# xmlyqing00/V-FloodNet

Hardware: AMD Instinct MI355X
Metric: segmented frames/sec at 480p (higher is better)
Workload: dtype f32

## Files before the change

include/vfn_hip.h:

```cpp
#ifndef VFN_HIP_H
#define VFN_HIP_H

#ifdef __cplusplus
extern "C" {
#endif

#define VFN_ABI_VERSION 12
enum { VFN_DESC_CONV = 0, VFN_DESC_STEM = 1, VFN_DESC_BANKSCAN = 2, VFN_DESC_MEMREAD = 3, VFN_DESC_BANK = 4, VFN_DESC_WGRAD = 5,
       VFN_DESC_REFRESH_FILTER = 6, VFN_DESC_REFRESH_EPILOGUE = 7, VFN_DESC_GATHER = 8 };
int vfn_abi_version(void);
int vfn_sizeof_desc(int which);

typedef struct vfn_conv_desc {
    const float* in;
    const float* w;
    const float* scale;
    const float* shift;
    const float* res;
    float* out;
    int N, H, W, Cin, in_ld;
    int Ho, Wo, Cout, cout_pad, out_ld, res_ld;
    int KH, KW, stride, pad;
    int relu_in, relu_out;
    int M;
    int ksplit;
    int split_from;
    int res_mod;
    float* partial;
    int* tile_counters;
    int w_packed;
    int in_lp;
    int out_lp_relu;
    void* out_lp;
    const float* mask;
    int mask_ld;
    int mask_after;
    int w_batch_rows;
    int k_rot;
} vfn_conv_desc;

int vfn_conv_cfg_count(void);
int vfn_conv_cfg_tile(int cfg, int* bm, int* bn);
int vfn_conv_cfg_info(int cfg, int* bm, int* bn, int* wm, int* wn, int* dma);
int vfn_conv_cfg_wk(int cfg);
int vfn_conv_cfg_tpb(int cfg);
#define VFN_CONV_SK_WS_FLOATS (16 * 1024 * 1024)
#define VFN_CONV_SK_MAX_TILES 16384
int vfn_conv_cfg_kind(int cfg);
int vfn_conv_cfg_name(int cfg, char* buf, int n);
int vfn_conv2d_nhwc_f32(const vfn_conv_desc* d, int cfg, void* stream);
int vfn_conv2d_nhwc_bf16(const vfn_conv_desc* d, int cfg, void* stream);
int vfn_conv2d_nhwc_bf16x3(const vfn_conv_desc* d, int cfg, void* stream);

int vfn_winograd_tiles(int N, int H, int W);
int vfn_winograd_input_f32(const float* x, int N, int H, int W, int C, int ld_x, int relu, float* V, int rows_pad, void* stream);
int vfn_winograd_output_f32(const float* Mb, int rows_pad, int N, int H, int W, int Cout, const float* scale, const float* shift,
                            const float* res, int res_ld, int res_mod, int relu_out, float* out, int out_ld, void* stream);
int vfn_winograd_output_masked_f32(const float* Mb, int rows_pad, int N, int H, int W, int Cout, const float* res, int res_ld,
                                   const float* mask, int mask_ld, int mask_after, float* out, int out_ld, void* stream);
int vfn_winograd_gemm_f32(const float* V, const float* U, float* Mb, int comps, int rows_pad, int C, int Cout, int cout_pad, int cfg,
                          int wgs, void* stream);
int vfn_conv1x1_persistent_f32(const vfn_conv_desc* d, int cfg, int wgs, void* stream);
int vfn_winograd_input_bf16(const float* x, int N, int H, int W, int C, int ld_x, int relu, void* V, int rows_pad, void* stream);
int vfn_winograd_gemm_bf16(const void* V, const void* U, float* Mb, int comps, int rows_pad, int C, int Cout, int cout_pad, int cfg,
                           int wgs, void* stream);
int vfn_winograd_gy_f32(const float* gy, int N, int H, int W, int C, int ld, float* Z, int rows_pad, void* stream);
int vfn_winograd_dw_f32(const float* dU, int Cout, int Cin, const float* rowscale, float* dw, int accumulate, void* stream);

typedef struct vfn_stem_desc {
    const float* frame;
    const float* mask;
    const float* w;
    const float* scale;
    const float* shift;
    float* out;
    float mean[3];
    float std[3];
    int N, cin;
    int H0, W0;
    int pad_top, pad_left;
    int Hp, Wp;
    int Ho, Wo;
} vfn_stem_desc;

int vfn_stem_conv7x7_f32(const vfn_stem_desc* d, void* stream);
int vfn_maxpool3x3s2_nhwc_f32(const float* in, float* out, int N, int H, int W, int C, void* stream);

int vfn_upsample2x_add_nhwc_f32(const float* s, const float* pm, float* out, int N, int h, int w, int C,
                                int s_bcast, void* stream);
int vfn_upsample2x_add_lp_nhwc_f32(const float* s, const float* pm, float* out, void* out_lp, int lp_relu,
                                   int N, int h, int w, int C, int s_bcast, void* stream);
int vfn_rough_uncertainty_f32(const float* p, float* p_up, float* rough, float* unc, int obj_n, int h, int w,
                              void* stream);
int vfn_local_hpass_f32(const float* r1, const float* rough, float* hs, float* hr, float* hm, int obj_n,
                        int h, int w, int C, void* stream);
int vfn_local_vpass_f32(const float* hs, const float* hr, const float* hm, float* lm,
                        float* conf, int obj_n, int h, int w, int C, void* stream);
int vfn_local_stats_f32(const float* r1, const float* rough, float* lm, float* conf, int obj_n, int h, int w, int C,
                        void* stream);
int vfn_pred2_gather_f32(const float* z, const float* bias, float* out, int N, int h, int w, int ldz, void* stream);
int vfn_final_logits_f32(const float* p_up, const float* unc, const float* conf, const float* q, float* score,
                         int obj_n, int h, int w, int pad_top, int pad_left, int H0, int W0, void* stream);

int vfn_segment_uncertainty_f32(const float* logit, int bs, int obj_n, int n, float* partial, float* out, void* stream);

int vfn_transpose_taps_f32(const float* x, int N, int H, int W, int C, int ld_x, int relu, int k, int stride, int pad, int Ho, int Wo,
                           const float* colscale, float* out, int Mpad, void* stream);

typedef struct vfn_wgrad_desc {
    const float* x;
    const float* gy;
    const float* rowscale;
    float* dw;
    float* partial;
    int N, H, W, Cin, ld_x;
    int Ho, Wo, Cout, ld_g;
    int k, stride, pad;
    int relu;
    int accumulate;
    int ksplit;
    int* tile_counters;
    int batch;
    int reserved;
    long long x_bstride, g_bstride;
} vfn_wgrad_desc;
int vfn_conv_wgrad_f32(const vfn_wgrad_desc* d, void* stream);

int vfn_stem_wgrad_scratch_floats(int C);
int vfn_stem_wgrad_f32(const float* x, const float* g, const float* rowscale, float* dw, float* partial, long long partial_floats,
                       int N, int Hp, int Wp, int C, int Ho, int Wo, int accumulate, void* stream);

typedef struct vfn_refresh_filter {
    const float* src;
    float* dst;
    const float* gamma;
    const float* var;
    float eps;
    int kind;
    int cout, cin, cin_off, cin_total, kh, kw;
    int dst_ld, dst_row0, dst_col0, cout_ld;
    int block0;
    int reserved;
} vfn_refresh_filter;
typedef struct vfn_refresh_epilogue {
    const float* gamma;
    const float* beta;
    const float* mean;
    const float* var;
    float* scale;
    float* shift;
    float eps;
    int C;
} vfn_refresh_epilogue;
int vfn_refresh_elems_per_block(void);
int vfn_refresh_filters_f32(const vfn_refresh_filter* table_dev, int n, int total_blocks, void* stream);
int vfn_refresh_epilogues_f32(const vfn_refresh_epilogue* table_dev, int n, void* stream);
typedef struct vfn_gather_entry {
    const float* src;
    long long dst_offset;
    long long stride[4];
    int shape[4];
    int block0;
    int reserved;
} vfn_gather_entry;
int vfn_gather_strided_f32(const vfn_gather_entry* table_dev, int n, int total_blocks, float* dst, void* stream);
int vfn_dilate2_f32(const float* g, float* out, int N, int Ho, int Wo, int H, int W, int C, void* stream);
int vfn_bn_param_grads_f32(const float* g, const float* y, const float* idn, const float* beta, const float* gamma, int M, int C,
                           float* partial, int nb, float* dgamma, float* dbeta, void* stream);
int vfn_bn_param_grads_acc_f32(const float* g, const float* y, const float* idn, const float* beta, const float* gamma, int M, int C,
                               float* partial, int nb, float* dgamma, float* dbeta, int accumulate, int* counter,
                               void* stream);
int vfn_maxpool3x3s2_backward_f32(const float* x, const float* g, float* gx, int N, int H, int W, int C, const float* add, int relu_mask,
                                  void* stream);
int vfn_softmax_cols_f32(const float* S, int B, int Q, int ld, float scale, float* P, void* stream);
int vfn_softmax_cols_backward_f32(const float* P, const float* dP, int B, int Q, int ld, float scale, float* dS, void* stream);
int vfn_adamw_f32(float* p, const float* g, float* m, float* v, long long n, double lr, double beta1, double beta2, double eps,
                  double weight_decay, int step, void* stream);
int vfn_colsum_f32(const float* x, int M, int C, int ld, float* partial, int nb, float* out, void* stream);
#define VFN_COLSUM_COUNTERS 64
int vfn_colsum_acc_f32(const float* x, int M, int C, int ld, float* partial, int nb, float* out, int accumulate, int* counter,
                       void* stream);
int vfn_upsample2x_add_backward_f32(const float* gm, float* gs, float* gpm, int N, int h, int w, int C, int s_bcast,
                                    void* stream);
int vfn_segment_loss_f32(const float* logit, const int* label, int bs, int obj_n, int n, float lu, float* partial, float* stats,
                         float* grad, void* stream);
int vfn_segment_uncertainty_backward_f32(const float* logit, int bs, int obj_n, int n, const float* g_unc_dev,
                                         const float* g_scores, float* partial, float* stats, float* grad, void* stream);
int vfn_tail_grad_o_f32(const float* G, const float* p_up, const float* unc, const float* conf, const float* q, float* g_o,
                        int obj_n, int h, int w, int pad_top, int pad_left, int H0, int W0, void* stream);
int vfn_tail_split_f32(const float* g_p2, const float* unc, const float* conf, const float* q, float* g_q, float* g_cf, float* g_u,
                       int obj_n, int npix, void* stream);
int vfn_local_stats_backward_f32(const float* g_lm, const float* lm, const float* g_cf, const float* g_u, const float* g_p2,
                                 const float* r1, const float* rough, const float* p_up, float* dA, float* dBv, int* amax,
                                 float* g_r1, float* g_pup, int obj_n, int h, int w, int C, void* stream);

typedef struct vfn_bankscan_desc {
    const float* q;
    const float* bank_k;
    const int* bank_len;
    const float* rowscale;
    float* part;
    long long stride_q, stride_k, stride_rs;
    float scale;
    int ldq, q_per_obj, HW, obj_n, nsplit, mode;
    int precision;
    int* work_counter;
    const void* bank_k_lp;
    float* scores;
    long long stride_scores;
} vfn_bankscan_desc;

typedef struct vfn_memread_desc {
    const float* q;
    const float* qv;
    const float* bank_k;
    const float* bank_v;
    const int* bank_len;
    const float* ml;
    float* o_part;
    int* cnt;
    float* info;
    float* out;
    long long stride_k, stride_v, stride_cnt, stride_info;
    float scale, thres;
    int ldq, ldqv, ld_out, HW, obj_n, nsplit;
    int precision;
    const void* bank_k_lp;
    const void* bank_v_lp;
    const float* scores;
    long long stride_scores;
} vfn_memread_desc;

int vfn_bank_scan(const vfn_bankscan_desc* d, void* stream);
int vfn_bank_scan_finish(const float* part, int nsplit, int HW, int obj_n, int mode, float* ml, int* idx,
                         float* corr, const float* colscale, void* stream);
int vfn_memread_apply(const vfn_memread_desc* d, void* stream);
int vfn_memread_finish(const vfn_memread_desc* d, void* stream);

#define VFN_BANK_MAX_HW 32768
typedef struct vfn_bank_desc {
    float* bank_k;
    float* bank_v;
    float* info;
    float* scratch_k;
    float* scratch_v;
    float* scratch_info;
    const int* bank_len;
    int* bank_len_rw;
    const float* bank_knorm;
    const float* bank_vnorm;
    const int* match_idx;
    const float* match_corr;
    const float* new_k;
    const float* new_knorm;
    const float* new_vnorm;
    int* app_pos;
    int* keep_dst;
    int* plan;
    int* stats;
    long long stride_k, stride_v, stride_info, stride_n, stride_new;
    double class_budget;
    float thres_close, update_rate, new_hit_init;
    int frame_idx, ld_new, voff, HW, obj_n, cap;
    int rm_class;
    int rm_request;
} vfn_bank_desc;

int vfn_bank_refresh_lp(const vfn_bank_desc* d, void* bank_k_lp, void* bank_v_lp, int all_rows, void* stream);

int vfn_row_norms(const float* x, long long stride_obj, int ld, int dim, const int* len_dev, int rows,
                  int obj_n, float* nrm, float* inv , long long stride_n, void* stream);
int vfn_bank_merge(const vfn_bank_desc* d, void* stream);
int vfn_bank_append(const vfn_bank_desc* d, void* stream);
int vfn_bank_remove(const vfn_bank_desc* d, void* stream);
int vfn_bank_refresh_norms(const vfn_bank_desc* d, float* bank_knorm, float* bank_kinv, float* bank_vnorm, void* stream);
int vfn_scatter_mean_f32(const float* src, long long src_s0, long long src_s1, const long long* index,
                         int S, float* out, long long out_s0, long long out_s1, int D, void* stream);
int vfn_scatter_mean_checked_f32(const float* src, long long src_s0, long long src_s1, const long long* index,
                                 long long index_s0, int S, float* out, long long out_s0, long long out_s1, int D,
                                 long long B, int* status, void* stream);

int vfn_resize_bicubic_f32(const float* in, float* out, int C, int Hi, int Wi, int Ho, int Wo, void* stream);
int vfn_resize_nearest_f32(const float* in, float* out, int C, int Hi, int Wi, int Ho, int Wo, void* stream);
int vfn_softmax_objects_f32(const float* score, float* prob, int obj_n, int n, void* stream);
int vfn_resize_argmax_u8(const float* prob, unsigned char* label, int obj_n, int Hi, int Wi, int Ho, int Wo,
                         void* stream);
int vfn_postprocess_pred_u8(const unsigned char* pred_host, int H, int W, unsigned char* out_host);
int vfn_postprocess_pred_device_u8(const unsigned char* pred, unsigned char* out, int* scratch, int H, int W,
                                   void* stream);

int vfn_to_tensor_u8(const unsigned char* src, float* dst, int H, int W, void* stream);
int vfn_overlay_u8(const float* frame, const unsigned char* mask, const unsigned char* palette, int* scratch,
                   unsigned char* out, int H, int W, double alpha, double cscale, void* stream);

int vfn_jpeg_entropy_decode(const unsigned char* data, long long size, short* coef, long long coef_cap,
                            unsigned short* qt, int* info);
int vfn_jpeg_idct_u8(const short* coef, const unsigned short* qt, unsigned char* plane, int blocks_per_row,
                     int block_rows, int pitch, void* stream);
int vfn_jpeg_to_tensor_f32(const unsigned char* y, const unsigned char* cb, const unsigned char* cr, int pitch_y,
                           int pitch_c, int W, int H, int hs, int vs, int ncomp, float* out_f32, unsigned char* out_u8,
                           void* stream);

int vfn_png_sizes(int H, int W, int bpp, long long* work_bytes, long long* out_bytes);
int vfn_png_deflate_u8(const unsigned char* raw, int H, int W, int bpp, void* work, unsigned char* out, int* stats,
                       void* stream);

int vfn_png_unfilter_sizes(int width, int height, int bpp, int* pitch, long long* work_bytes);
int vfn_png_unfilter_u8(const unsigned char* filtered, int width, int height, int bpp, void* work, unsigned char* raw,
                        int* status, void* stream);
int vfn_png_to_tensor_f32(const unsigned char* raw, int pitch, int width, int height, int color_type,
                          const unsigned char* palette, float* out, unsigned char* out_u8, void* stream);

int vfn_ln_stem_f32(const float* x, const float* w, const float* scale, const float* shift, float* out, int N, int H, int W, int Ho,
                    int Wo, int ld, int pad_before, void* stream);
int vfn_ln_dwconv_f32(const float* x, const float* w, const float* scale, const float* shift, float* out, int N, int H, int W, int C,
                      int ld_x, int ld_out, int k, int stride, int pad_before, int Ho, int Wo, int swish_in, void* stream);
int vfn_ln_se_gate_f32(const float* sum_px, float inv_hw, const float* w1, const float* b1, const float* w2, const float* b2,
                       float* gate, int C, int sq, int Cpad, void* stream);
int vfn_ln_scale_cols_f32(const float* w, const float* g, float* out, int rows, int K, void* stream);
int vfn_ln_add_f32(const float* a, const float* b, float* out, long long n, void* stream);
int vfn_ln_head_f32(const float* x, const float* w, float bias, float* out, long long M, int C, int ld, int prob, void* stream);

#ifdef __cplusplus
}
#endif
#endif
```

v-floodnet_amd/_lib.py:

```python
import ctypes as C
import os

import torch

_HERE = os.path.dirname(os.path.abspath(__file__))
LIB_PATH = os.environ.get('VFN_LIB_PATH') or os.path.join(_HERE, 'libvfn_hip.so')

_lib = None

c_fp = C.c_void_p


class ConvDesc(C.Structure):
    _fields_ = [('inp', c_fp), ('w', c_fp), ('scale', c_fp), ('shift', c_fp), ('res', c_fp), ('out', c_fp),
                ('N', C.c_int), ('H', C.c_int), ('W', C.c_int), ('Cin', C.c_int), ('in_ld', C.c_int),
                ('Ho', C.c_int), ('Wo', C.c_int), ('Cout', C.c_int), ('cout_pad', C.c_int),
                ('out_ld', C.c_int), ('res_ld', C.c_int),
                ('KH', C.c_int), ('KW', C.c_int), ('stride', C.c_int), ('pad', C.c_int),
                ('relu_in', C.c_int), ('relu_out', C.c_int), ('M', C.c_int), ('ksplit', C.c_int),
                ('split_from', C.c_int), ('res_mod', C.c_int), ('partial', c_fp), ('tile_counters', c_fp),
                ('w_packed', C.c_int), ('in_lp', C.c_int), ('out_lp_relu', C.c_int), ('out_lp', c_fp), ('mask', c_fp), ('mask_ld', C.c_int), ('mask_after', C.c_int), ('w_batch_rows', C.c_int), ('k_rot', C.c_int)]


class WgradDesc(C.Structure):
    _fields_ = [('x', c_fp), ('gy', c_fp), ('rowscale', c_fp), ('dw', c_fp), ('partial', c_fp),
                ('N', C.c_int), ('H', C.c_int), ('W', C.c_int), ('Cin', C.c_int), ('ld_x', C.c_int),
                ('Ho', C.c_int), ('Wo', C.c_int), ('Cout', C.c_int), ('ld_g', C.c_int),
                ('k', C.c_int), ('stride', C.c_int), ('pad', C.c_int), ('relu', C.c_int), ('accumulate', C.c_int), ('ksplit', C.c_int),
                ('tile_counters', c_fp), ('batch', C.c_int), ('reserved', C.c_int), ('x_bstride', C.c_longlong), ('g_bstride', C.c_longlong)]


class RefreshFilter(C.Structure):
    _fields_ = [('src', c_fp), ('dst', c_fp), ('gamma', c_fp), ('var', c_fp), ('eps', C.c_float), ('kind', C.c_int),
                ('cout', C.c_int), ('cin', C.c_int), ('cin_off', C.c_int), ('cin_total', C.c_int), ('kh', C.c_int), ('kw', C.c_int),
                ('dst_ld', C.c_int), ('dst_row0', C.c_int), ('dst_col0', C.c_int), ('cout_ld', C.c_int), ('block0', C.c_int),
                ('reserved', C.c_int)]


class RefreshEpilogue(C.Structure):
    _fields_ = [('gamma', c_fp), ('beta', c_fp), ('mean', c_fp), ('var', c_fp), ('scale', c_fp), ('shift', c_fp),
                ('eps', C.c_float), ('C', C.c_int)]


class GatherEntry(C.Structure):
    _fields_ = [('src', c_fp), ('dst_offset', C.c_longlong), ('stride', C.c_longlong * 4), ('shape', C.c_int * 4), ('block0', C.c_int),
                ('reserved', C.c_int)]


class StemDesc(C.Structure):
    _fields_ = [('frame', c_fp), ('mask', c_fp), ('w', c_fp), ('scale', c_fp), ('shift', c_fp), ('out', c_fp),
                ('mean', C.c_float * 3), ('std', C.c_float * 3),
                ('N', C.c_int), ('cin', C.c_int), ('H0', C.c_int), ('W0', C.c_int),
                ('pad_top', C.c_int), ('pad_left', C.c_int), ('Hp', C.c_int), ('Wp', C.c_int),
                ('Ho', C.c_int), ('Wo', C.c_int)]


class BankScanDesc(C.Structure):
    _fields_ = [('q', c_fp), ('bank_k', c_fp), ('bank_len', c_fp), ('rowscale', c_fp), ('part', c_fp),
                ('stride_q', C.c_longlong), ('stride_k', C.c_longlong), ('stride_rs', C.c_longlong),
                ('scale', C.c_float),
                ('ldq', C.c_int), ('q_per_obj', C.c_int), ('HW', C.c_int), ('obj_n', C.c_int),
                ('nsplit', C.c_int), ('mode', C.c_int), ('precision', C.c_int), ('work_counter', c_fp), ('bank_k_lp', c_fp), ('scores', c_fp), ('stride_scores', C.c_longlong)]


class MemReadDesc(C.Structure):
    _fields_ = [('q', c_fp), ('qv', c_fp), ('bank_k', c_fp), ('bank_v', c_fp), ('bank_len', c_fp), ('ml', c_fp),
                ('o_part', c_fp), ('cnt', c_fp), ('info', c_fp), ('out', c_fp),
                ('stride_k', C.c_longlong), ('stride_v', C.c_longlong), ('stride_cnt', C.c_longlong),
                ('stride_info', C.c_longlong),
                ('scale', C.c_float), ('thres', C.c_float),
                ('ldq', C.c_int), ('ldqv', C.c_int), ('ld_out', C.c_int), ('HW', C.c_int), ('obj_n', C.c_int),
                ('nsplit', C.c_int), ('precision', C.c_int), ('bank_k_lp', c_fp), ('bank_v_lp', c_fp), ('scores', c_fp), ('stride_scores', C.c_longlong)]


class BankDesc(C.Structure):
    _fields_ = [('bank_k', c_fp), ('bank_v', c_fp), ('info', c_fp),
                ('scratch_k', c_fp), ('scratch_v', c_fp), ('scratch_info', c_fp),
                ('bank_len', c_fp), ('bank_len_rw', c_fp), ('bank_knorm', c_fp), ('bank_vnorm', c_fp),
                ('match_idx', c_fp), ('match_corr', c_fp), ('new_k', c_fp), ('new_knorm', c_fp), ('new_vnorm', c_fp),
                ('app_pos', c_fp), ('keep_dst', c_fp), ('plan', c_fp), ('stats', c_fp),
                ('stride_k', C.c_longlong), ('stride_v', C.c_longlong), ('stride_info', C.c_longlong),
                ('stride_n', C.c_longlong), ('stride_new', C.c_longlong),
                ('class_budget', C.c_double),
                ('thres_close', C.c_float), ('update_rate', C.c_float), ('new_hit_init', C.c_float),
                ('frame_idx', C.c_int), ('ld_new', C.c_int), ('voff', C.c_int), ('HW', C.c_int),
                ('obj_n', C.c_int), ('cap', C.c_int), ('rm_class', C.c_int), ('rm_request', C.c_int)]


ABI_VERSION = 12
DESC_IDS = {0: ConvDesc, 1: StemDesc, 2: BankScanDesc, 3: MemReadDesc, 4: BankDesc, 5: WgradDesc, 6: RefreshFilter, 7: RefreshEpilogue, 8: GatherEntry}


def lib():
    global _lib
    if _lib is None:
        if not os.path.isfile(LIB_PATH):
            raise RuntimeError(
                f'{LIB_PATH} not found: build the HIP kernels first '
                '(python -c "import __graft_entry__ as g; g.build()" or make -C v-floodnet_amd/csrc)')
        L = C.CDLL(LIB_PATH)
        L.vfn_abi_version.restype = C.c_int
        if L.vfn_abi_version() != ABI_VERSION:
            raise RuntimeError(f'{LIB_PATH} has ABI version {L.vfn_abi_version()}, this package expects {ABI_VERSION} '
                               '(descriptor layouts differ): rebuild it (make -C v-floodnet_amd/csrc)')
        L.vfn_sizeof_desc.restype = C.c_int
        for which, cls in DESC_IDS.items():
            if L.vfn_sizeof_desc(which) != C.sizeof(cls):
                raise RuntimeError(f'{LIB_PATH}: sizeof({cls.__name__}) is {L.vfn_sizeof_desc(which)} in the library, '
                                   f'{C.sizeof(cls)} in this binding: rebuild it (make -C v-floodnet_amd/csrc)')
        _declare(L)
        _lib = L
    return _lib


def _declare(L):
    i, f, p = C.c_int, C.c_float, C.c_void_p
    L.vfn_abi_version.restype = i
    L.vfn_conv_cfg_count.restype = i
    L.vfn_conv_cfg_tile.argtypes = [i, C.POINTER(i), C.POINTER(i)]
    L.vfn_conv_cfg_info.argtypes = [i] + [C.POINTER(i)] * 5
    L.vfn_conv_cfg_wk.argtypes = [i]
    L.vfn_conv_cfg_wk.restype = i
    L.vfn_conv_cfg_tpb.argtypes = [i]
    L.vfn_conv_cfg_tpb.restype = i
    L.vfn_conv_cfg_kind.argtypes = [i]
    L.vfn_conv_cfg_name.argtypes = [i, C.c_char_p, i]
    L.vfn_conv_cfg_name.restype = i
    L.vfn_conv_cfg_kind.restype = i
    L.vfn_sizeof_desc.argtypes = [i]
    L.vfn_conv2d_nhwc_f32.argtypes = [C.POINTER(ConvDesc), i, p]
    L.vfn_conv2d_nhwc_bf16.argtypes = [C.POINTER(ConvDesc), i, p]
    L.vfn_conv2d_nhwc_bf16x3.argtypes = [C.POINTER(ConvDesc), i, p]
    L.vfn_stem_conv7x7_f32.argtypes = [C.POINTER(StemDesc), p]
    L.vfn_bank_scan.argtypes = [C.POINTER(BankScanDesc), p]
    L.vfn_memread_apply.argtypes = [C.POINTER(MemReadDesc), p]
    L.vfn_memread_finish.argtypes = [C.POINTER(MemReadDesc), p]
    L.vfn_bank_merge.argtypes = [C.POINTER(BankDesc), p]
    L.vfn_bank_append.argtypes = [C.POINTER(BankDesc), p]
    L.vfn_bank_remove.argtypes = [C.POINTER(BankDesc), p]
    L.vfn_bank_refresh_norms.argtypes = [C.POINTER(BankDesc), p, p, p, p]
    L.vfn_conv_wgrad_f32.argtypes = [C.POINTER(WgradDesc), p]
    L.vfn_bank_refresh_lp.argtypes = [C.POINTER(BankDesc), p, p, i, p]
    L.vfn_stem_wgrad_scratch_floats.argtypes = [i]
    L.vfn_stem_wgrad_scratch_floats.restype = i
    for name, args in SIGNATURES.items():
        fn = getattr(L, name)
        fn.argtypes = args
        fn.restype = i


_i, _f, _p = C.c_int, C.c_float, C.c_void_p
_ll = C.c_longlong
SIGNATURES = {
    'vfn_maxpool3x3s2_nhwc_f32': [_p, _p, _i, _i, _i, _i, _p],
    'vfn_upsample2x_add_nhwc_f32': [_p, _p, _p, _i, _i, _i, _i, _i, _p],
    'vfn_upsample2x_add_lp_nhwc_f32': [_p, _p, _p, _p, _i, _i, _i, _i, _i, _i, _p],
    'vfn_rough_uncertainty_f32': [_p, _p, _p, _p, _i, _i, _i, _p],
    'vfn_transpose_taps_f32': [_p, _i, _i, _i, _i, _i, _i, _i, _i, _i, _i, _i, _p, _p, _i, _p],
    'vfn_dilate2_f32': [_p, _p, _i, _i, _i, _i, _i, _i, _p],
    'vfn_bn_param_grads_f32': [_p, _p, _p, _p, _p, _i, _i, _p, _i, _p, _p, _p],
    'vfn_bn_param_grads_acc_f32': [_p, _p, _p, _p, _p, _i, _i, _p, _i, _p, _p, _i, _p, _p],
    'vfn_maxpool3x3s2_backward_f32': [_p, _p, _p, _i, _i, _i, _i, _p, _i, _p],
    'vfn_softmax_cols_f32': [_p, _i, _i, _i, _f, _p, _p],
    'vfn_softmax_cols_backward_f32': [_p, _p, _i, _i, _i, _f, _p, _p],
    'vfn_adamw_f32': [_p, _p, _p, _p, _ll, C.c_double, C.c_double, C.c_double, C.c_double, C.c_double, _i, _p],
    'vfn_colsum_f32': [_p, _i, _i, _i, _p, _i, _p, _p],
    'vfn_colsum_acc_f32': [_p, _i, _i, _i, _p, _i, _p, _i, _p, _p],
    'vfn_upsample2x_add_backward_f32': [_p, _p, _p, _i, _i, _i, _i, _i, _p],
    'vfn_tail_grad_o_f32': [_p, _p, _p, _p, _p, _p, _i, _i, _i, _i, _i, _i, _i, _p],
    'vfn_segment_loss_f32': [_p, _p, _i, _i, _i, _f, _p, _p, _p, _p],
    'vfn_segment_uncertainty_backward_f32': [_p, _i, _i, _i, _p, _p, _p, _p, _p, _p],
    'vfn_tail_split_f32': [_p, _p, _p, _p, _p, _p, _p, _i, _i, _p],
    'vfn_local_stats_backward_f32': [_p] * 13 + [_i, _i, _i, _i, _p],
    'vfn_local_hpass_f32': [_p, _p, _p, _p, _p, _i, _i, _i, _i, _p],
    'vfn_local_vpass_f32': [_p, _p, _p, _p, _p, _i, _i, _i, _i, _p],
    'vfn_local_stats_f32': [_p, _p, _p, _p, _i, _i, _i, _i, _p],
    'vfn_pred2_gather_f32': [_p, _p, _p, _i, _i, _i, _i, _p],
    'vfn_final_logits_f32': [_p, _p, _p, _p, _p, _i, _i, _i, _i, _i, _i, _i, _p],
    'vfn_bank_scan_finish': [_p, _i, _i, _i, _i, _p, _p, _p, _p, _p],
    'vfn_row_norms': [_p, _ll, _i, _i, _p, _i, _i, _p, _p, _ll, _p],
    'vfn_scatter_mean_f32': [_p, _ll, _ll, _p, _i, _p, _ll, _ll, _i, _p],
    'vfn_winograd_tiles': [_i, _i, _i],
    'vfn_winograd_input_f32': [_p, _i, _i, _i, _i, _i, _i, _p, _i, _p],
    'vfn_winograd_output_f32': [_p, _i, _i, _i, _i, _i, _p, _p, _p, _i, _i, _i, _p, _i, _p],
    'vfn_winograd_gy_f32': [_p, _i, _i, _i, _i, _i, _p, _i, _p],
    'vfn_winograd_gemm_f32': [_p, _p, _p, _i, _i, _i, _i, _i, _i, _i, _p],
    'vfn_conv1x1_persistent_f32': [_p, _i, _i, _p],
    'vfn_winograd_input_bf16': [_p, _i, _i, _i, _i, _i, _i, _p, _i, _p],
    'vfn_winograd_gemm_bf16': [_p, _p, _p, _i, _i, _i, _i, _i, _i, _i, _p],
    'vfn_winograd_dw_f32': [_p, _i, _i, _p, _p, _i, _p],
    'vfn_winograd_output_masked_f32': [_p, _i, _i, _i, _i, _i, _p, _i, _p, _i, _i, _p, _i, _p],
    'vfn_scatter_mean_checked_f32': [_p, _ll, _ll, _p, _ll, _i, _p, _ll, _ll, _i, _ll, _p, _p],
    'vfn_resize_bicubic_f32': [_p, _p, _i, _i, _i, _i, _i, _p],
    'vfn_resize_nearest_f32': [_p, _p, _i, _i, _i, _i, _i, _p],
    'vfn_softmax_objects_f32': [_p, _p, _i, _i, _p],
    'vfn_resize_argmax_u8': [_p, _p, _i, _i, _i, _i, _i, _p],
    'vfn_postprocess_pred_u8': [_p, _i, _i, _p],
    'vfn_postprocess_pred_device_u8': [_p, _p, _p, _i, _i, _p],
    'vfn_to_tensor_u8': [_p, _p, _i, _i, _p],
    'vfn_overlay_u8': [_p, _p, _p, _p, _p, _i, _i, C.c_double, C.c_double, _p],
    'vfn_segment_uncertainty_f32': [_p, _i, _i, _i, _p, _p, _p],
    'vfn_jpeg_entropy_decode': [_p, _ll, _p, _ll, _p, _p],
    'vfn_jpeg_idct_u8': [_p, _p, _p, _i, _i, _i, _p],
    'vfn_jpeg_to_tensor_f32': [_p, _p, _p, _i, _i, _i, _i, _i, _i, _i, _p, _p, _p],
    'vfn_png_sizes': [_i, _i, _i, C.POINTER(_ll), C.POINTER(_ll)],
    'vfn_png_deflate_u8': [_p, _i, _i, _i, _p, _p, _p, _p],
    'vfn_png_unfilter_sizes': [_i, _i, _i, C.POINTER(_i), C.POINTER(_ll)],
    'vfn_png_unfilter_u8': [_p, _i, _i, _i, _p, _p, _p, _p],
    'vfn_png_to_tensor_f32': [_p, _i, _i, _i, _i, _p, _p, _p, _p],
    'vfn_refresh_elems_per_block': [],
    'vfn_refresh_filters_f32': [_p, _i, _i, _p],
    'vfn_refresh_epilogues_f32': [_p, _i, _p],
    'vfn_gather_strided_f32': [_p, _i, _i, _p, _p],
    'vfn_ln_stem_f32': [_p, _p, _p, _p, _p, _i, _i, _i, _i, _i, _i, _i, _p],
    'vfn_ln_dwconv_f32': [_p, _p, _p, _p, _p, _i, _i, _i, _i, _i, _i, _i, _i, _i, _i, _i, _i, _p],
    'vfn_ln_se_gate_f32': [_p, _f, _p, _p, _p, _p, _p, _i, _i, _i, _p],
    'vfn_ln_scale_cols_f32': [_p, _p, _p, _i, _i, _p],
    'vfn_ln_add_f32': [_p, _p, _p, _ll, _p],
    'vfn_ln_head_f32': [_p, _p, _f, _p, _ll, _i, _i, _i, _p],
    'vfn_stem_wgrad_f32': [_p, _p, _p, _p, _p, _ll, _i, _i, _i, _i, _i, _i, _i, _p],
}
ALL_SYMBOLS = sorted(list(SIGNATURES) + [
    'vfn_abi_version', 'vfn_sizeof_desc', 'vfn_conv_cfg_count', 'vfn_conv_cfg_tile', 'vfn_conv_cfg_info', 'vfn_conv_cfg_wk', 'vfn_conv_cfg_tpb', 'vfn_conv_cfg_kind', 'vfn_conv_cfg_name', 'vfn_conv2d_nhwc_f32', 'vfn_conv2d_nhwc_bf16', 'vfn_conv2d_nhwc_bf16x3',
    'vfn_stem_conv7x7_f32',
    'vfn_bank_scan', 'vfn_memread_apply', 'vfn_memread_finish', 'vfn_bank_merge', 'vfn_bank_append', 'vfn_bank_remove', 'vfn_bank_refresh_norms', 'vfn_bank_refresh_lp', 'vfn_conv_wgrad_f32',
    'vfn_stem_wgrad_scratch_floats'])


def check(status, what):
    if status != 0:
        raise RuntimeError(f'HIP kernel launcher {what} failed with status {status}')


def ptr(t):
    if t is None:
        return None
    return C.c_void_p(t.data_ptr())


_raw_stream = getattr(torch._C, '_cuda_getCurrentRawStream', None)


def stream():
    if _raw_stream is not None:
        return C.c_void_p(_raw_stream(torch.cuda.current_device()))
    return C.c_void_p(torch.cuda.current_stream().cuda_stream)


def require_gpu(t, what='tensor'):
    if not t.is_cuda:
        raise RuntimeError(f'{what} must live on the GPU: the V-FloodNet hot path has no CPU fallback')


PROBES = []


def independent_stream(device, beside=(), tries=12, priority=0):
    device = torch.device(device)
    cur = torch.cuda.current_stream(device)
    others = [cur] + [s_ for s_ in beside if s_ is not None]
    big, small = torch.zeros(16 * 1024 * 1024, device=device), torch.zeros(16, device=device)

    def overlaps(cand, ref):
        torch.cuda.synchronize(device)
        ref_end, cand_end = torch.cuda.Event(), torch.cuda.Event()
        with torch.cuda.stream(ref):
            for _ in range(64):
                big.add_(1.0)
            ref_end.record()
        with torch.cuda.stream(cand):
            small.add_(1.0)
            cand_end.record()
        cand_end.synchronize()
        ok = not ref_end.query()
        torch.cuda.synchronize(device)
        return ok

    cand = None
    for n_ in range(tries):
        cand = torch.cuda.Stream(device=device, priority=priority)
        if all(overlaps(cand, o_) for o_ in others):
            PROBES.append((True, n_ + 1))
            return cand
    PROBES.append((False, tries))
    import warnings
    warnings.warn('vfloodnet_amd: no stream with a hardware queue of its own found; side-stream work will run in order with the frame loop')
    return cand
```

v-floodnet_amd/csrc/abi.hip:

```cpp
#include "common.h"
#include "../../include/vfn_hip.h"
extern "C" int vfn_abi_version(void) { return VFN_ABI_VERSION; }

extern "C" int vfn_sizeof_desc(int which) {
    switch (which) {
        case VFN_DESC_CONV: return (int)sizeof(vfn_conv_desc);
        case VFN_DESC_STEM: return (int)sizeof(vfn_stem_desc);
        case VFN_DESC_BANKSCAN: return (int)sizeof(vfn_bankscan_desc);
        case VFN_DESC_MEMREAD: return (int)sizeof(vfn_memread_desc);
        case VFN_DESC_BANK: return (int)sizeof(vfn_bank_desc);
        case VFN_DESC_WGRAD: return (int)sizeof(vfn_wgrad_desc);
        case VFN_DESC_REFRESH_FILTER: return (int)sizeof(vfn_refresh_filter);
        case VFN_DESC_REFRESH_EPILOGUE: return (int)sizeof(vfn_refresh_epilogue);
        case VFN_DESC_GATHER: return (int)sizeof(vfn_gather_entry);
    }
    return -1;
}
```

v-floodnet_amd/csrc/bank.hip:

```cpp
#include "common.h"
#include "../../include/vfn_hip.h"

namespace {

constexpr int DK = 128, DV = 512;

__device__ __forceinline__ float block_reduce_sum(float v, float* red) {
    v = wave_sum(v);
    const int lane = threadIdx.x & 63, w = threadIdx.x >> 6;
    __syncthreads();
    if (lane == 0) red[w] = v;
    __syncthreads();
    float t = 0.f;
    for (int i = 0; i < (int)(blockDim.x >> 6); ++i) t += red[i];
    return t;
}
__device__ __forceinline__ float block_reduce_min(float v, float* red) {
    v = wave_min(v);
    const int lane = threadIdx.x & 63, w = threadIdx.x >> 6;
    __syncthreads();
    if (lane == 0) red[w] = v;
    __syncthreads();
    float t = INFINITY;
    for (int i = 0; i < (int)(blockDim.x >> 6); ++i) t = fminf(t, red[i]);
    return t;
}
__device__ __forceinline__ int block_reduce_sum_i(int v, int* red) {
    v = wave_sum_i(v);
    const int lane = threadIdx.x & 63, w = threadIdx.x >> 6;
    __syncthreads();
    if (lane == 0) red[w] = v;
    __syncthreads();
    int t = 0;
    for (int i = 0; i < (int)(blockDim.x >> 6); ++i) t += red[i];
    return t;
}

__device__ __forceinline__ int block_excl_scan(int flag, int* red, int* total) {
    const int lane = threadIdx.x & 63, w = threadIdx.x >> 6;
    const unsigned long long m = __ballot(flag);
    const int within = __popcll(m & ((1ull << lane) - 1ull));
    __syncthreads();
    if (lane == 0) red[w] = __popcll(m);
    __syncthreads();
    int base = 0, tot = 0;
    for (int i = 0; i < (int)(blockDim.x >> 6); ++i) { if (i < w) base += red[i]; tot += red[i]; }
    *total = tot;
    return base + within;
}

__global__ void row_norms_kernel(const float* __restrict__ x, long long stride_obj, int ld, int dim,
                                 const int* __restrict__ len_dev, int rows_fixed,
                                 float* __restrict__ nrm, float* __restrict__ inv, long long stride_n) {
    const int obj = blockIdx.y;
    const int rows = len_dev ? len_dev[obj] : rows_fixed;
    const int lane = threadIdx.x & 63;
    const int wpb = blockDim.x >> 6;
    for (int r = blockIdx.x * wpb + (threadIdx.x >> 6); r < rows; r += gridDim.x * wpb) {
        const float* src = x + (size_t)obj * stride_obj + (size_t)r * ld;
        float s = 0.f;
        for (int d = lane * 4; d < dim; d += 256) {
            const f32x4 v = *reinterpret_cast<const f32x4*>(src + d);
            s += v.x * v.x + v.y * v.y + v.z * v.z + v.w * v.w;
        }
        s = wave_sum(s);
        if (lane == 0) {
            const float n = sqrtf(s);
            nrm[(size_t)obj * stride_n + r] = n;
            if (inv) inv[(size_t)obj * stride_n + r] = 1.f / fmaxf(n, 1e-12f);
        }
    }
}

__global__ __launch_bounds__(256)
void bank_merge_kernel(const vfn_bank_desc p) {
    extern __shared__ __attribute__((aligned(16))) char smem[];
    __shared__ int s_any;
    const int obj = blockIdx.y, hw = blockIdx.x, tid = threadIdx.x;
    const int* idx = p.match_idx + (size_t)obj * p.HW;
    const float* corr = p.match_corr + (size_t)obj * p.HW;
    if (!(corr[hw] > p.thres_close)) return;
    const int tgt = idx[hw];
    if (tid == 0) s_any = 0;
    __syncthreads();
    int found = 0;
    for (int j = tid; j < hw; j += 256) found |= (idx[j] == tgt && corr[j] > p.thres_close);
    if (found) s_any = 1;
    __syncthreads();
    if (s_any) return;
    unsigned* s_bits = reinterpret_cast<unsigned*>(smem);
    const int nwords = (p.HW + 31) >> 5;
    for (int w = tid; w < nwords; w += 256) s_bits[w] = 0u;
    __syncthreads();
    for (int j = hw + tid; j < p.HW; j += 256)
        if (idx[j] == tgt && corr[j] > p.thres_close) atomicOr(&s_bits[j >> 5], 1u << (j & 31));
    __syncthreads();

    const float* nk = p.new_k + (size_t)obj * p.stride_new;
    const float* nkn = p.new_knorm + (size_t)obj * p.HW;
    const float* nvn = p.new_vnorm + (size_t)obj * p.HW;
    float ak = 0.f, av0 = 0.f, av1 = 0.f;
    int cnt = 0;
    for (int w = hw >> 5; w < nwords; ++w) {
        unsigned bits = s_bits[w];
        while (bits) {
            const int j = (w << 5) + __ffs(bits) - 1;
            bits &= bits - 1;
            const float* row = nk + (size_t)j * p.ld_new;
            const float dk = fmaxf(nkn[j], 1e-12f), dv = fmaxf(nvn[j], 1e-12f);
            if (tid < DK) ak += row[tid] / dk;
            av0 += row[p.voff + tid] / dv;
            av1 += row[p.voff + 256 + tid] / dv;
            ++cnt;
        }
    }
    const float c = (float)(cnt < 1 ? 1 : cnt);
    const float r = p.update_rate;
    float* K = p.bank_k + (size_t)obj * p.stride_k + (size_t)tgt * DK;
    float* V = p.bank_v + (size_t)obj * p.stride_v + (size_t)tgt * DV;
    const float magk = p.bank_knorm[(size_t)obj * p.stride_n + tgt];
    const float magv = p.bank_vnorm[(size_t)obj * p.stride_n + tgt];
    const float dk = fmaxf(magk, 1e-12f), dv = fmaxf(magv, 1e-12f);
    if (tid < DK) K[tid] = magk * ((1.f - r) * (K[tid] / dk) + r * (ak / c));
    V[tid] = magv * ((1.f - r) * (V[tid] / dv) + r * (av0 / c));
    V[256 + tid] = magv * ((1.f - r) * (V[256 + tid] / dv) + r * (av1 / c));
}

__global__ __launch_bounds__(1024)
void bank_plan_kernel(const vfn_bank_desc p) {
    __shared__ float redf[16];
    __shared__ int redi[16];
    __shared__ int s_carry;
    const int obj = blockIdx.x, tid = threadIdx.x;
    const float* corr = p.match_corr + (size_t)obj * p.HW;
    int* pos = p.app_pos + (size_t)obj * p.HW;
    int* plan = p.plan + obj * 4;
    const int B = p.bank_len[obj];
    const bool remove_only = p.rm_class >= 0;
    if (remove_only && obj != p.rm_class) {
        if (tid == 0) { plan[0] = 0; plan[1] = 0; plan[2] = B; plan[3] = 0; }
        return;
    }

    int carry = 0;
    for (int base = 0; base < (remove_only ? 0 : p.HW); base += 1024) {
        const int j = base + tid;
        const int f = (j < p.HW) && (corr[j] <= p.thres_close);
        int tot;
        const int off = block_excl_scan(f, redi, &tot);
        if (j < p.HW) pos[j] = f ? carry + off : -1;
        carry += tot;
        __syncthreads();
    }
    const int n_app = remove_only ? p.rm_request : carry;

    int evict = 0, kept = B;
    if (remove_only || (double)p.class_budget < (double)B + (double)n_app) {
        evict = 1;
        const float* info = p.info + (size_t)obj * p.stride_info;
        int* dst = p.keep_dst + (size_t)obj * p.stride_n;
        float mn = INFINITY;
        int has_nan = 0;
        for (int b = tid; b < B; b += 1024) {
            const float l = info[(size_t)b * 2 + 1] / ((float)p.frame_idx - info[(size_t)b * 2]);
            has_nan |= (l != l);
            mn = fminf(mn, l);
        }
        mn = block_reduce_min(mn, redf);
        has_nan = block_reduce_sum_i(has_nan, redi);
        if (has_nan || (B > 0 && !(fabsf(mn) < INFINITY))) {
            if (tid == 0) { plan[0] = 0; plan[1] = 0; plan[2] = B; plan[3] = 0; p.stats[obj * 4 + 3] = has_nan ? -1 : -2; }
            return;
        }
        int thr = (int)mn + 1;
        for (int it = 0; it < 100000; ++it) {
            int cnt = 0;
            float mn2 = INFINITY;
            for (int b = tid; b < B; b += 1024) {
                const float l = info[(size_t)b * 2 + 1] / ((float)p.frame_idx - info[(size_t)b * 2]);
                if (l > (float)thr) { ++cnt; mn2 = fminf(mn2, l); }
            }
            kept = block_reduce_sum_i(cnt, redi);
            const double balance = ((double)p.class_budget - (double)kept) - (double)n_app;
            if (balance >= 0.0 || kept == 0) break;
            mn2 = block_reduce_min(mn2, redf);
            thr = (int)mn2 + 1;
        }
        int c2 = 0;
        for (int base = 0; base < B; base += 1024) {
            const int b = base + tid;
            int f = 0;
            if (b < B) {
                const float l = info[(size_t)b * 2 + 1] / ((float)p.frame_idx - info[(size_t)b * 2]);
                f = l > (float)thr;
            }
            int tot;
            const int off = block_excl_scan(f, redi, &tot);
            if (b < B) dst[b] = f ? c2 + off : -1;
            c2 += tot;
            __syncthreads();
        }
        kept = c2;
    }
    if (tid == 0) {
        plan[0] = remove_only ? 0 : n_app; plan[1] = evict; plan[2] = kept; plan[3] = B - kept;
        (void)s_carry;
    }
}

__global__ void bank_compact_kernel(const vfn_bank_desc p, int phase) {
    const int obj = blockIdx.y;
    const int* plan = p.plan + obj * 4;
    if (!plan[1]) return;
    const int B = p.bank_len[obj];
    const int* dst = p.keep_dst + (size_t)obj * p.stride_n;
    float* K = p.bank_k + (size_t)obj * p.stride_k;
    float* V = p.bank_v + (size_t)obj * p.stride_v;
    float* I = p.info + (size_t)obj * p.stride_info;
    float* Ks = p.scratch_k + (size_t)obj * p.stride_k;
    float* Vs = p.scratch_v + (size_t)obj * p.stride_v;
    float* Is = p.scratch_info + (size_t)obj * p.stride_info;
    const int lane = threadIdx.x & 63, wpb = blockDim.x >> 6;
    for (int b = blockIdx.x * wpb + (threadIdx.x >> 6); b < B; b += gridDim.x * wpb) {
        const int d = dst[b];
        if (d < 0 || d == b) continue;
        const float* sk = phase == 0 ? K + (size_t)b * DK : Ks + (size_t)d * DK;
        const float* sv = phase == 0 ? V + (size_t)b * DV : Vs + (size_t)d * DV;
        const float* si = phase == 0 ? I + (size_t)b * 2 : Is + (size_t)d * 2;
        float* dk = phase == 0 ? Ks + (size_t)d * DK : K + (size_t)d * DK;
        float* dv = phase == 0 ? Vs + (size_t)d * DV : V + (size_t)d * DV;
        float* di = phase == 0 ? Is + (size_t)d * 2 : I + (size_t)d * 2;
        if (lane < 32) *reinterpret_cast<f32x4*>(dk + lane * 4) = *reinterpret_cast<const f32x4*>(sk + lane * 4);
        *reinterpret_cast<f32x4*>(dv + lane * 4) = *reinterpret_cast<const f32x4*>(sv + lane * 4);
        *reinterpret_cast<f32x4*>(dv + 256 + lane * 4) = *reinterpret_cast<const f32x4*>(sv + 256 + lane * 4);
        if (lane == 0) { di[0] = si[0]; di[1] = si[1]; }
    }
}

__global__ void bank_append_kernel(const vfn_bank_desc p) {
    const int obj = blockIdx.y;
    const int* plan = p.plan + obj * 4;
    const int base = plan[2];
    const int* pos = p.app_pos + (size_t)obj * p.HW;
    float* K = p.bank_k + (size_t)obj * p.stride_k;
    float* V = p.bank_v + (size_t)obj * p.stride_v;
    float* I = p.info + (size_t)obj * p.stride_info;
    const float* nk = p.new_k + (size_t)obj * p.stride_new;
    const int lane = threadIdx.x & 63, wpb = blockDim.x >> 6;
    for (int j = blockIdx.x * wpb + (threadIdx.x >> 6); j < p.HW; j += gridDim.x * wpb) {
        const int q = pos[j];
        if (q < 0) continue;
        const int row = base + q;
        if (row >= p.cap) continue;
        const float* src = nk + (size_t)j * p.ld_new;
        if (lane < 32) *reinterpret_cast<f32x4*>(K + (size_t)row * DK + lane * 4) = *reinterpret_cast<const f32x4*>(src + lane * 4);
        *reinterpret_cast<f32x4*>(V + (size_t)row * DV + lane * 4) = *reinterpret_cast<const f32x4*>(src + p.voff + lane * 4);
        *reinterpret_cast<f32x4*>(V + (size_t)row * DV + 256 + lane * 4) = *reinterpret_cast<const f32x4*>(src + p.voff + 256 + lane * 4);
        if (lane == 0) { I[(size_t)row * 2] = (float)p.frame_idx; I[(size_t)row * 2 + 1] = p.new_hit_init; }
    }
}

__global__ void bank_finalize_kernel(const vfn_bank_desc p) {
    const int obj = blockIdx.y;
    const int* plan = p.plan + obj * 4;
    int newlen = plan[2] + plan[0];
    if (newlen > p.cap) newlen = p.cap;
    float* I = p.info + (size_t)obj * p.stride_info;
    if (p.rm_class < 0)
        for (int b = blockIdx.x * blockDim.x + threadIdx.x; b < newlen; b += gridDim.x * blockDim.x)
            I[(size_t)b * 2 + 1] = fminf(fmaxf(I[(size_t)b * 2 + 1], 0.f), 1e5f);
    if (blockIdx.x == 0 && threadIdx.x == 0) {
        int* st = p.stats + obj * 4;
        st[0] = newlen;
        if (newlen > st[1]) st[1] = newlen;
        st[2] += plan[3];
        if (st[3] >= 0 && p.rm_class < 0) st[3] = plan[0];
    }
}

__global__ void bank_commit_len_kernel(const vfn_bank_desc p) {
    const int obj = threadIdx.x;
    if (obj < p.obj_n) p.bank_len_rw[obj] = p.stats[obj * 4];
}

__global__ void bank_refresh_norms_kernel(const vfn_bank_desc p, float* __restrict__ knorm, float* __restrict__ kinv,
                                          float* __restrict__ vnorm) {
    const int obj = blockIdx.y;
    const int* plan = p.plan + obj * 4;
    const bool all = plan[1] != 0;
    const int newlen = p.stats[obj * 4];
    const int base = plan[2];
    const int items = all ? newlen : p.HW;
    const int* idx = p.match_idx + (size_t)obj * p.HW;
    const float* corr = p.match_corr + (size_t)obj * p.HW;
    const int* pos = p.app_pos + (size_t)obj * p.HW;
    const float* K = p.bank_k + (size_t)obj * p.stride_k;
    const float* V = p.bank_v + (size_t)obj * p.stride_v;
    const int lane = threadIdx.x & 63, wpb = blockDim.x >> 6;
    for (int it = blockIdx.x * wpb + (threadIdx.x >> 6); it < items; it += gridDim.x * wpb) {
        int row = it;
        if (!all) row = (corr[it] > p.thres_close) ? idx[it] : base + pos[it];
        if (row < 0 || row >= newlen) continue;
        float sk = 0.f, sv = 0.f;
        for (int d = lane * 4; d < DK; d += 256) {
            const f32x4 v = *reinterpret_cast<const f32x4*>(K + (size_t)row * DK + d);
            sk += v.x * v.x + v.y * v.y + v.z * v.z + v.w * v.w;
        }
        for (int d = lane * 4; d < DV; d += 256) {
            const f32x4 v = *reinterpret_cast<const f32x4*>(V + (size_t)row * DV + d);
            sv += v.x * v.x + v.y * v.y + v.z * v.z + v.w * v.w;
        }
        sk = wave_sum(sk);
        sv = wave_sum(sv);
        if (lane == 0) {
            const float nk = sqrtf(sk);
            knorm[(size_t)obj * p.stride_n + row] = nk;
            kinv[(size_t)obj * p.stride_n + row] = 1.f / fmaxf(nk, 1e-12f);
            vnorm[(size_t)obj * p.stride_n + row] = sqrtf(sv);
        }
    }
}

typedef __bf16 bf16x4_t __attribute__((ext_vector_type(4)));
typedef __bf16 bf16x2_t __attribute__((ext_vector_type(2)));
typedef __bf16 bf16x8_t __attribute__((ext_vector_type(8)));
__global__ void bank_refresh_lp_kernel(const vfn_bank_desc p, char* __restrict__ klp, char* __restrict__ vlp, int all_rows) {
    const int obj = blockIdx.y;
    bool all = all_rows != 0;
    int newlen, base = 0;
    if (all) newlen = p.bank_len[obj];
    else {
        const int* plan = p.plan + obj * 4;
        all = plan[1] != 0;
        newlen = p.stats[obj * 4];
        base = plan[2];
    }
    const int* idx = p.match_idx + (size_t)obj * p.HW;
    const float* corr = p.match_corr + (size_t)obj * p.HW;
    const int* pos = p.app_pos + (size_t)obj * p.HW;
    const float* K = p.bank_k + (size_t)obj * p.stride_k;
    const float* V = p.bank_v + (size_t)obj * p.stride_v;
    char* KL = klp + (size_t)obj * p.stride_k * 4;
    char* VL = vlp + (size_t)obj * p.stride_v * 4;
    const int lane = threadIdx.x & 63, wpb = blockDim.x >> 6;
    auto split_key_row = [&](int row) {
        const float2 v = *reinterpret_cast<const float2*>(K + (size_t)row * DK + 2 * lane);
        bf16x2_t h, l;
        h[0] = (__bf16)v.x; h[1] = (__bf16)v.y;
        l[0] = (__bf16)(v.x - (float)h[0]); l[1] = (__bf16)(v.y - (float)h[1]);
        char* dst = KL + (size_t)row * (DK * 4);
        *reinterpret_cast<bf16x2_t*>(dst + 4 * lane) = h;
        *reinterpret_cast<bf16x2_t*>(dst + DK * 2 + 4 * lane) = l;
    };
    if (all) {
        const int nblk = (newlen + 7) >> 3;
        for (int blk = blockIdx.x * wpb + (threadIdx.x >> 6); blk < nblk; blk += gridDim.x * wpb) {
#pragma unroll
            for (int r = 0; r < 8; ++r)
                if (blk * 8 + r < newlen) split_key_row(blk * 8 + r);
            char* dst = VL + (size_t)blk * (8 * DV * 4);
            for (int c = lane; c < DV; c += 64) {
                bf16x8_t h, l;
#pragma unroll
                for (int r = 0; r < 8; ++r) {
                    const int row = blk * 8 + r;
                    const float x = row < newlen ? V[(size_t)row * DV + c] : 0.f;
                    h[r] = (__bf16)x;
                    l[r] = (__bf16)(x - (float)h[r]);
                }
                *reinterpret_cast<bf16x8_t*>(dst + c * 16) = h;
                *reinterpret_cast<bf16x8_t*>(dst + DV * 16 + c * 16) = l;
            }
        }
        return;
    }
    for (int it = blockIdx.x * wpb + (threadIdx.x >> 6); it < p.HW; it += gridDim.x * wpb) {
        const int row = (corr[it] > p.thres_close) ? idx[it] : base + pos[it];
        if (row < 0 || row >= newlen) continue;
        split_key_row(row);
        char* dst = VL + (size_t)(row >> 3) * (8 * DV * 4) + (row & 7) * 2;
        for (int c = lane; c < DV; c += 64) {
            const float x = V[(size_t)row * DV + c];
            const __bf16 h = (__bf16)x;
            *reinterpret_cast<__bf16*>(dst + c * 16) = h;
            *reinterpret_cast<__bf16*>(dst + DV * 16 + c * 16) = (__bf16)(x - (float)h);
        }
    }
}

__global__ __launch_bounds__(256)
void scatter_mean_kernel(const float* __restrict__ src, long long src_s0, long long src_s1,
                         const long long* __restrict__ index, long long index_s0, int S, float* __restrict__ out,
                         long long out_s0, long long out_s1, int D, long long B, int* __restrict__ status) {
    __shared__ int s_any;
    const int s = blockIdx.x, tid = threadIdx.x;
    const long long tgt = index[s];
    if (status) {
        if (index_s0 != 0) {
            int bad = 0;
            for (int d = tid; d < D; d += 256) bad |= (index[d * index_s0 + s] != tgt);
            if (bad) atomicOr(status, 2);
        }
        if (tgt < 0 || tgt >= B) {
            if (tid == 0) atomicOr(status, 1);
            return;
        }
    }
    if (tid == 0) s_any = 0;
    __syncthreads();
    int found = 0;
    for (int j = tid; j < s; j += 256) found |= (index[j] == tgt);
    if (found) s_any = 1;
    __syncthreads();
    if (s_any) return;
    for (int d = tid; d < D; d += 256) {
        float acc = out[d * out_s0 + tgt * out_s1];
        int cnt = 0;
        for (int j = s; j < S; ++j)
            if (index[j] == tgt) { acc += src[d * src_s0 + j * src_s1]; ++cnt; }
        out[d * out_s0 + tgt * out_s1] = acc / (float)(cnt < 1 ? 1 : cnt);
    }
}

}

extern "C" int vfn_row_norms(const float* x, long long stride_obj, int ld, int dim, const int* len_dev, int rows,
                             int obj_n, float* nrm, float* inv, long long stride_n, void* stream) {
    if (!x || !nrm || dim % 4 || ld % 4 || obj_n < 1) return VFN_ERR_ARG;
    const int blocks = len_dev ? 1024 : (cdiv(rows, 4) < 1024 ? (cdiv(rows, 4) > 0 ? cdiv(rows, 4) : 1) : 1024);
    hipLaunchKernelGGL(row_norms_kernel, dim3(blocks, obj_n), dim3(256), 0, (hipStream_t)stream,
                       x, stride_obj, ld, dim, len_dev, rows, nrm, inv, stride_n);
    return vfn_check_launch();
}

static int bank_desc_ok(const vfn_bank_desc* d) {
    return d && d->bank_k && d->bank_v && d->info && d->bank_len && d->HW > 0 && d->HW <= VFN_BANK_MAX_HW && d->obj_n > 0;
}

extern "C" int vfn_bank_merge(const vfn_bank_desc* d, void* stream) {
    if (!bank_desc_ok(d) || d->rm_class >= 0) return VFN_ERR_ARG;
    if (!d->match_idx || !d->match_corr || !d->new_k || !d->new_knorm || !d->new_vnorm || !d->bank_knorm || !d->bank_vnorm)
        return VFN_ERR_ARG;
    hipLaunchKernelGGL(bank_merge_kernel, dim3(d->HW, d->obj_n), dim3(256), (size_t)((d->HW + 31) / 32) * 4, (hipStream_t)stream, *d);
    return vfn_check_launch();
}

extern "C" int vfn_bank_append(const vfn_bank_desc* d, void* stream) {
    if (!bank_desc_ok(d) || d->rm_class >= 0) return VFN_ERR_ARG;
    if (!d->match_corr || !d->app_pos || !d->plan || !d->keep_dst || !d->new_k || !d->stats || !d->bank_len_rw ||
        !d->scratch_k || !d->scratch_v || !d->scratch_info)
        return VFN_ERR_ARG;
    hipStream_t s = (hipStream_t)stream;
    hipLaunchKernelGGL(bank_plan_kernel, dim3(d->obj_n), dim3(1024), 0, s, *d);
    hipLaunchKernelGGL(bank_compact_kernel, dim3(1024, d->obj_n), dim3(256), 0, s, *d, 0);
    hipLaunchKernelGGL(bank_compact_kernel, dim3(1024, d->obj_n), dim3(256), 0, s, *d, 1);
    hipLaunchKernelGGL(bank_append_kernel, dim3(cdiv(d->HW, 4), d->obj_n), dim3(256), 0, s, *d);
    hipLaunchKernelGGL(bank_finalize_kernel, dim3(256, d->obj_n), dim3(256), 0, s, *d);
    hipLaunchKernelGGL(bank_commit_len_kernel, dim3(1), dim3(64), 0, s, *d);
    return vfn_check_launch();
}

extern "C" int vfn_bank_remove(const vfn_bank_desc* d, void* stream) {
    if (!bank_desc_ok(d) || d->rm_class < 0 || d->rm_class >= d->obj_n || d->rm_request < 0) return VFN_ERR_ARG;
    if (!d->app_pos || !d->plan || !d->keep_dst || !d->stats || !d->bank_len_rw || !d->scratch_k || !d->scratch_v ||
        !d->scratch_info || !d->match_corr)
        return VFN_ERR_ARG;
    hipStream_t s = (hipStream_t)stream;
    hipLaunchKernelGGL(bank_plan_kernel, dim3(d->obj_n), dim3(1024), 0, s, *d);
    hipLaunchKernelGGL(bank_compact_kernel, dim3(1024, d->obj_n), dim3(256), 0, s, *d, 0);
    hipLaunchKernelGGL(bank_compact_kernel, dim3(1024, d->obj_n), dim3(256), 0, s, *d, 1);
    hipLaunchKernelGGL(bank_finalize_kernel, dim3(256, d->obj_n), dim3(256), 0, s, *d);
    hipLaunchKernelGGL(bank_commit_len_kernel, dim3(1), dim3(64), 0, s, *d);
    return vfn_check_launch();
}

extern "C" int vfn_scatter_mean_f32(const float* src, long long src_s0, long long src_s1, const long long* index,
                                    int S, float* out, long long out_s0, long long out_s1, int D, void* stream) {
    if (!src || !index || !out || S < 0 || D < 1) return VFN_ERR_ARG;
    if (S == 0) return VFN_OK;
    hipLaunchKernelGGL(scatter_mean_kernel, dim3(S), dim3(256), 0, (hipStream_t)stream,
                       src, src_s0, src_s1, index, 0LL, S, out, out_s0, out_s1, D, 0LL, (int*)nullptr);
    return vfn_check_launch();
}

extern "C" int vfn_scatter_mean_checked_f32(const float* src, long long src_s0, long long src_s1, const long long* index,
                                            long long index_s0, int S, float* out, long long out_s0, long long out_s1, int D,
                                            long long B, int* status, void* stream) {
    if (!src || !index || !out || !status || S < 0 || D < 1 || B < 1) return VFN_ERR_ARG;
    if (S == 0) return VFN_OK;
    hipLaunchKernelGGL(scatter_mean_kernel, dim3(S), dim3(256), 0, (hipStream_t)stream,
                       src, src_s0, src_s1, index, index_s0, S, out, out_s0, out_s1, D, B, status);
    return vfn_check_launch();
}

extern "C" int vfn_bank_refresh_norms(const vfn_bank_desc* d, float* bank_knorm, float* bank_kinv, float* bank_vnorm,
                                      void* stream) {
    if (!bank_desc_ok(d) || !d->plan || !d->stats || !d->match_idx || !d->match_corr || !d->app_pos) return VFN_ERR_ARG;
    if (!bank_knorm || !bank_kinv || !bank_vnorm) return VFN_ERR_ARG;
    hipLaunchKernelGGL(bank_refresh_norms_kernel, dim3(1024, d->obj_n), dim3(256), 0, (hipStream_t)stream, *d,
                       bank_knorm, bank_kinv, bank_vnorm);
    return vfn_check_launch();
}

extern "C" int vfn_bank_refresh_lp(const vfn_bank_desc* d, void* bank_k_lp, void* bank_v_lp, int all_rows, void* stream) {
    if (!bank_desc_ok(d) || !bank_k_lp || !bank_v_lp) return VFN_ERR_ARG;
    if (!all_rows && (!d->plan || !d->stats || !d->match_idx || !d->match_corr || !d->app_pos)) return VFN_ERR_ARG;
    hipLaunchKernelGGL(bank_refresh_lp_kernel, dim3(all_rows ? 4096 : 1024, d->obj_n), dim3(256), 0, (hipStream_t)stream, *d,
                       (char*)bank_k_lp, (char*)bank_v_lp, all_rows);
    return vfn_check_launch();
}
```

v-floodnet_amd/csrc/memory_read.hip:

```cpp
#include "common.h"
#include "../../include/vfn_hip.h"
#include <type_traits>
#include <cstdlib>

namespace {

constexpr int DK = 128, DV = 512;
constexpr int CH = 64;

__device__ __forceinline__ int swz(int row, int chunk) { return row * DK + ((chunk ^ (row & 15)) << 2); }

__device__ __forceinline__ int swz64(int row, int chunk) { return row * CH + ((chunk ^ (row & 15)) << 2); }

struct ChunkRegs { f32x4 v[8]; };
__device__ __forceinline__ void chunk_load(ChunkRegs& R, const float* src, int valid, int tid) {
    const int c = tid & 31;
#pragma unroll
    for (int j = 0; j < 8; ++j) {
        const int r = (tid >> 5) + 8 * j;
        const int rr = r < valid ? r : 0;
        R.v[j] = *reinterpret_cast<const f32x4*>(src + (size_t)rr * DK + c * 4);
        if (r >= valid) R.v[j] = f32x4{0.f, 0.f, 0.f, 0.f};
    }
}
__device__ __forceinline__ void chunk_store(const ChunkRegs& R, float* dst, int tid) {
    const int c = tid & 31;
#pragma unroll
    for (int j = 0; j < 8; ++j) {
        const int r = (tid >> 5) + 8 * j;
        *reinterpret_cast<f32x4*>(dst + swz(r, c)) = R.v[j];
    }
}

__device__ __forceinline__ void chunk_load_async(float* sK, const float* src, int valid, int wave, int lane) {
#pragma unroll
    for (int j = 0; j < 8; ++j) {
        const int r = (wave * 8 + j) * 2 + (lane >> 5);
        const int pc = lane & 31;
        const int rr = min(r, valid - 1);
        const float* g = src + (size_t)rr * DK + ((pc ^ (r & 15)) << 2);
        __builtin_amdgcn_global_load_lds(g, sK + (wave * 8 + j) * 2 * DK, 16, 0, 0);
    }
}

__device__ __forceinline__ void stage_rows(float* dst, const float* src, size_t ld, int rows, int valid, int tid) {
    const int c = tid & 31;
    for (int r = tid >> 5; r < rows; r += 8) {
        f32x4 v = {0.f, 0.f, 0.f, 0.f};
        if (r < valid) v = *reinterpret_cast<const f32x4*>(src + (size_t)r * ld + c * 4);
        *reinterpret_cast<f32x4*>(dst + swz(r, c)) = v;
    }
}

__device__ __forceinline__ void score_tile(const float* sK, const float* sQ, int wr, int wq, int li, int lh, f32x16& acc) {
#pragma unroll
    for (int r = 0; r < 16; ++r) acc[r] = 0.f;
    const int ra = wr * 32 + li, rq = wq * 32 + li;
    f32x4 a[2], b[2];
    a[0] = *reinterpret_cast<const f32x4*>(sK + swz(ra, lh));
    b[0] = *reinterpret_cast<const f32x4*>(sQ + swz(rq, lh));
#pragma unroll
    for (int kk = 0; kk < 16; ++kk) {
        const int cur = kk & 1;
        if (kk + 1 < 16) {
            a[cur ^ 1] = *reinterpret_cast<const f32x4*>(sK + swz(ra, 2 * (kk + 1) + lh));
            b[cur ^ 1] = *reinterpret_cast<const f32x4*>(sQ + swz(rq, 2 * (kk + 1) + lh));
        }
#pragma unroll
        for (int t = 0; t < 4; ++t)
            acc = __builtin_amdgcn_mfma_f32_32x32x2f32(a[cur][t], b[cur][t], acc, 0, 0, 0);
    }
}

typedef __attribute__((ext_vector_type(2))) float f32x2;
typedef unsigned u32x4 __attribute__((ext_vector_type(4)));
typedef unsigned u32x2 __attribute__((ext_vector_type(2)));
typedef __attribute__((ext_vector_type(4))) __bf16 bf16x4;
typedef __attribute__((ext_vector_type(8))) __bf16 bf16x8;

__device__ __forceinline__ bf16x8 cvt8(const f32x4& a, const f32x4& b) {
    bf16x8 r;
#pragma unroll
    for (int e = 0; e < 4; ++e) { r[e] = (__bf16)a[e]; r[4 + e] = (__bf16)b[e]; }
    return r;
}
__device__ __forceinline__ void split8(const f32x4& a, const f32x4& b, bf16x8& h, bf16x8& l) {
#pragma unroll
    for (int e = 0; e < 4; ++e) {
        const __bf16 x = (__bf16)a[e], y = (__bf16)b[e];
        h[e] = x; h[4 + e] = y;
        l[e] = (__bf16)(a[e] - (float)x); l[4 + e] = (__bf16)(b[e] - (float)y);
    }
}
__device__ __forceinline__ int swzk(int row, int half, int chunk) { return row * 512 + half * 256 + ((chunk ^ (row & 15)) << 4); }
__device__ __forceinline__ int swzq(int row, int chunk) { return row * 256 + ((chunk ^ (row & 15)) << 4); }

template <int NT, bool X3>
__device__ __forceinline__ void convert_chunk_inplace(float* sK, int tid) {
    constexpr int TPR = NT / CH;
    constexpr int F4 = 32 / TPR;
    const int r = tid / TPR, part = tid % TPR;
    f32x4 v[F4];
#pragma unroll
    for (int j = 0; j < F4; ++j) v[j] = *reinterpret_cast<const f32x4*>(sK + swz(r, part * F4 + j));
    __syncthreads();
    char* base = reinterpret_cast<char*>(sK);
#pragma unroll
    for (int j = 0; j < F4; j += 2) {
        bf16x8 h, l;
        split8(v[j], v[j + 1], h, l);
        const int chunk = (part * F4 + j) >> 1;
        *reinterpret_cast<bf16x8*>(base + swzk(r, 0, chunk)) = h;
        if constexpr (X3) *reinterpret_cast<bf16x8*>(base + swzk(r, 1, chunk)) = l;
    }
    __syncthreads();
}

template <bool X3>
__device__ __forceinline__ void mfma_lp(f32x16& acc, const bf16x8& ah, const bf16x8& al, const bf16x8& bh, const bf16x8& bl) {
    if constexpr (X3) {
        acc = __builtin_amdgcn_mfma_f32_32x32x16_bf16(al, bh, acc, 0, 0, 0);
        acc = __builtin_amdgcn_mfma_f32_32x32x16_bf16(ah, bl, acc, 0, 0, 0);
    }
    acc = __builtin_amdgcn_mfma_f32_32x32x16_bf16(ah, bh, acc, 0, 0, 0);
}

__device__ __forceinline__ float fast_exp(float x) { return __expf(x); }

__device__ __forceinline__ void chunk_range(int B, int nsplit, int split, int& c_lo, int& c_hi) {
    const int nchunks = (B + CH - 1) / CH;
    const int per = (nchunks + nsplit - 1) / nsplit;
    c_lo = split * per;
    c_hi = min(nchunks, c_lo + per);
}

constexpr int QTS = 128;

#ifdef VFN_CENSUS
__device__ unsigned long long vfn_census_buf[4096 * 4];
#endif

template <int MODE, int PREC = 0>
__global__ __launch_bounds__(256, 2)
void bank_scan_kernel(const vfn_bankscan_desc p) {
#ifdef VFN_CENSUS
    const unsigned long long census_t0 = __builtin_amdgcn_s_memrealtime();
#endif
    extern __shared__ __attribute__((aligned(16))) char smem[];
    float* sKb = reinterpret_cast<float*>(smem);
    __shared__ int s_item;

    const int tid = threadIdx.x, lane = tid & 63, wave = tid >> 6;
    const int li = lane & 31, lh = lane >> 5;
    const int qtiles = (p.HW + QTS - 1) / QTS;
    const int total = p.nsplit * qtiles * p.obj_n;
  for (;;) {
    if (tid == 0) s_item = atomicAdd(p.work_counter, 1);
    __syncthreads();
    const int item = s_item;
    __syncthreads();
    if (item >= total) break;
    const int obj = item % p.obj_n;
    const int qt = (item / p.obj_n) % qtiles;
    const int split = item / (p.obj_n * qtiles);
    const int q0 = qt * QTS + wave * 32;
    const int B = p.bank_len[obj];
    const bool lp_image = PREC != 0 && p.bank_k_lp != nullptr;
    const float* K = (lp_image ? reinterpret_cast<const float*>(p.bank_k_lp) : p.bank_k) + (size_t)obj * p.stride_k;
    const float* Q = p.q + (size_t)(p.q_per_obj ? obj : 0) * p.stride_q;

    int c_lo, c_hi;
    chunk_range(B, p.nsplit, split, c_lo, c_hi);
    if (c_lo < c_hi) chunk_load_async(sKb, K + (size_t)c_lo * CH * DK, min(CH, B - c_lo * CH), wave, lane);

    f32x4 qf[PREC == 0 ? 16 : 1];
    bf16x8 qh[PREC == 0 ? 1 : 8], ql[PREC == 2 ? 8 : 1];
    {
        const int q = min(q0 + li, p.HW - 1);
        if constexpr (PREC == 0) {
            const float* qrow = Q + (size_t)q * p.ldq + 4 * lh;
#pragma unroll
            for (int kk = 0; kk < 16; ++kk) qf[kk] = *reinterpret_cast<const f32x4*>(qrow + 8 * kk);
        } else {
            const float* qrow = Q + (size_t)q * p.ldq + 8 * lh;
#pragma unroll
            for (int g = 0; g < 8; ++g) {
                const f32x4 x0 = *reinterpret_cast<const f32x4*>(qrow + 16 * g);
                const f32x4 x1 = *reinterpret_cast<const f32x4*>(qrow + 16 * g + 4);
                if constexpr (PREC == 2) split8(x0, x1, qh[g], ql[g]);
                else qh[g] = cvt8(x0, x1);
            }
        }
    }

    float run_m = -INFINITY, run_l = 0.f;
    int run_i = 0x7fffffff;
    __syncthreads();

    for (int c = c_lo; c < c_hi; ++c) {
        const int b0 = c * CH;
        const float* sK = sKb + ((c - c_lo) & 1) * CH * DK;
#ifndef VFN_ABLATE_KLOAD
        if (c + 1 < c_hi)
            chunk_load_async(sKb + ((c + 1 - c_lo) & 1) * CH * DK, K + (size_t)(b0 + CH) * DK, min(CH, B - b0 - CH), wave, lane);
#endif
        f32x4 scv[MODE == 1 ? 2 : 1][MODE == 1 ? 4 : 1];
        if constexpr (MODE == 1) {
            const float* rs = p.rowscale + (size_t)obj * p.stride_rs;
#pragma unroll
            for (int i = 0; i < 2; ++i)
#pragma unroll
                for (int g = 0; g < 4; ++g) scv[i][g] = *reinterpret_cast<const f32x4*>(rs + b0 + 32 * i + 4 * lh + 8 * g);
        }
        f32x16 acc[2];
#pragma unroll
        for (int i = 0; i < 2; ++i)
#pragma unroll
            for (int r = 0; r < 16; ++r) acc[i][r] = 0.f;
        if constexpr (PREC == 0) {
            f32x4 a[2][2];
            a[0][0] = *reinterpret_cast<const f32x4*>(sK + swz(li, lh));
            a[0][1] = *reinterpret_cast<const f32x4*>(sK + swz(32 + li, lh));
#pragma unroll
            for (int kk = 0; kk < 16; ++kk) {
                const int cur = kk & 1;
                if (kk + 1 < 16) {
                    a[cur ^ 1][0] = *reinterpret_cast<const f32x4*>(sK + swz(li, 2 * (kk + 1) + lh));
                    a[cur ^ 1][1] = *reinterpret_cast<const f32x4*>(sK + swz(32 + li, 2 * (kk + 1) + lh));
                }
#pragma unroll
                for (int t = 0; t < 4; ++t) {
                    acc[0] = __builtin_amdgcn_mfma_f32_32x32x2f32(a[cur][0][t], qf[kk][t], acc[0], 0, 0, 0);
                    acc[1] = __builtin_amdgcn_mfma_f32_32x32x2f32(a[cur][1][t], qf[kk][t], acc[1], 0, 0, 0);
                }
            }
        } else if (PREC == 2 || lp_image) {
            if (!lp_image) convert_chunk_inplace<256, true>(const_cast<float*>(sK), tid);
            const char* kb = reinterpret_cast<const char*>(sK);
#pragma unroll
            for (int g = 0; g < 8; ++g) {
#pragma unroll
                for (int i = 0; i < 2; ++i) {
                    const bf16x8 ah = *reinterpret_cast<const bf16x8*>(kb + swzk(32 * i + li, 0, 2 * g + lh));
                    bf16x8 al = ah;
                    if constexpr (PREC == 2) al = *reinterpret_cast<const bf16x8*>(kb + swzk(32 * i + li, 1, 2 * g + lh));
                    mfma_lp<PREC == 2>(acc[i], ah, al, qh[g], ql[PREC == 2 ? g : 0]);
                }
            }
        } else {
#pragma unroll
            for (int g = 0; g < 8; ++g) {
#pragma unroll
                for (int i = 0; i < 2; ++i) {
                    const f32x4 x0 = *reinterpret_cast<const f32x4*>(sK + swz(32 * i + li, 4 * g + 2 * lh));
                    const f32x4 x1 = *reinterpret_cast<const f32x4*>(sK + swz(32 * i + li, 4 * g + 2 * lh + 1));
                    const bf16x8 ah = cvt8(x0, x1);
                    mfma_lp<false>(acc[i], ah, ah, qh[g], ql[0]);
                }
            }
        }
        if (MODE == 0 && p.scores) {
            float* tile = p.scores + (size_t)obj * p.stride_scores + ((size_t)c * qtiles + qt) * (CH * QTS);
#pragma unroll
            for (int i = 0; i < 2; ++i)
#pragma unroll
                for (int g = 0; g < 4; ++g) {
                    const f32x4 v = {acc[i][4 * g], acc[i][4 * g + 1], acc[i][4 * g + 2], acc[i][4 * g + 3]};
                    __builtin_nontemporal_store(v, reinterpret_cast<f32x4*>(tile + ((((i * 4 + g) * 2 + lh) * QTS) + wave * 32 + li) * 4));
                }
        }
#ifdef VFN_ABLATE_SOFTMAX
        if (true) { run_m = fmaxf(run_m, acc[0][0] + acc[1][5]); } else
#endif
        if (MODE == 0) {
            if (b0 + CH <= B) {
                float mx = acc[0][0];
#pragma unroll
                for (int i = 0; i < 2; ++i)
#pragma unroll
                    for (int r = 0; r < 16; ++r) mx = fmaxf(mx, acc[i][r]);
                const float mn = fmaxf(run_m, mx * p.scale);
                float sum = 0.f;
#pragma unroll
                for (int i = 0; i < 2; ++i)
#pragma unroll
                    for (int r = 0; r < 16; ++r) sum += fast_exp(acc[i][r] * p.scale - mn);
                run_l = run_l * expf(run_m - mn) + sum;
                run_m = mn;
            } else {
                float mx = -INFINITY;
#pragma unroll
                for (int i = 0; i < 2; ++i)
#pragma unroll
                    for (int r = 0; r < 16; ++r) {
                        const int row = b0 + 32 * i + 4 * lh + (r & 3) + 8 * (r >> 2);
                        const float s_ = acc[i][r] * p.scale;
                        acc[i][r] = s_;
                        if (row < B) mx = fmaxf(mx, s_);
                    }
                const float mn = fmaxf(run_m, mx);
                if (mn > -INFINITY) {
                    float sum = 0.f;
#pragma unroll
                    for (int i = 0; i < 2; ++i)
#pragma unroll
                        for (int r = 0; r < 16; ++r) {
                            const int row = b0 + 32 * i + 4 * lh + (r & 3) + 8 * (r >> 2);
                            if (row < B) sum += fast_exp(acc[i][r] - mn);
                        }
                    run_l = run_l * expf(run_m - mn) + sum;
                    run_m = mn;
                }
            }
        } else {
#pragma unroll
            for (int i = 0; i < 2; ++i)
#pragma unroll
                for (int g = 0; g < 4; ++g) {
                    const int row0 = b0 + 32 * i + 4 * lh + 8 * g;
                    const f32x4 sc = scv[MODE == 1 ? i : 0][MODE == 1 ? g : 0];
#pragma unroll
                    for (int j = 0; j < 4; ++j) {
                        const int row = row0 + j;
                        if (row < B) {
                            const float s_ = acc[i][4 * g + j] * sc[j];
                            if (s_ > run_m) { run_m = s_; run_i = row; }
                        }
                    }
                }
        }
        __syncthreads();
    }

    {
        const float om = __shfl_xor(run_m, 32, 64);
        if (MODE == 0) {
            const float ol = __shfl_xor(run_l, 32, 64);
            const float mn = fmaxf(run_m, om);
            float l = 0.f;
            if (mn > -INFINITY) l = run_l * expf(run_m - mn) + ol * expf(om - mn);
            run_m = mn; run_l = l;
        } else {
            const int oi = __shfl_xor(run_i, 32, 64);
            if (om > run_m || (om == run_m && oi < run_i)) { run_m = om; run_i = oi; }
        }
    }
#ifdef VFN_CENSUS
    if (threadIdx.x == 0) {
        const int lin = blockIdx.y * gridDim.x + blockIdx.x;
        if (lin < 4096) {
            unsigned hw_id, xcc;
            asm volatile("s_getreg_b32 %0, hwreg(HW_REG_HW_ID)" : "=s"(hw_id));
            asm volatile("s_getreg_b32 %0, hwreg(HW_REG_XCC_ID)" : "=s"(xcc));
            vfn_census_buf[lin * 4] = census_t0; vfn_census_buf[lin * 4 + 1] = __builtin_amdgcn_s_memrealtime();
            vfn_census_buf[lin * 4 + 2] = hw_id; vfn_census_buf[lin * 4 + 3] = xcc;
        }
    }
#endif
    const int q = q0 + li;
    if (lh == 0 && q < p.HW) {
        float* dst = p.part + (((size_t)obj * p.nsplit + split) * p.HW + q) * 2;
        dst[0] = run_m;
        dst[1] = (MODE == 0) ? run_l : __int_as_float(run_i);
    }
  }
}

constexpr size_t SCAN_PIPE_LDS = 2 * (size_t)CH * DK * 2 + 2 * CH * sizeof(float);
constexpr unsigned SCAN_PIPE_SC0 = 2 * CH * DK * 2;

template <int MODE>
__global__ __launch_bounds__(256, 2)
void bank_scan_pipe_kernel(const vfn_bankscan_desc p) {
    extern __shared__ __attribute__((aligned(16))) char smem[];
    __shared__ int s_item;

    const int tid = threadIdx.x, lane = tid & 63, wave = tid >> 6;
    const int li = lane & 31, lh = lane >> 5;
    const int qtiles = (p.HW + QTS - 1) / QTS;
    const int total = p.nsplit * qtiles * p.obj_n;
    const int krow = tid >> 2, kc4 = (tid & 3) * 4;
    const unsigned klane_off = (unsigned)krow * 512u + (unsigned)kc4 * 16u;
  for (;;) {
    if (tid == 0) s_item = atomicAdd(p.work_counter, 1);
    __syncthreads();
    const int item = s_item;
    __syncthreads();
    if (item >= total) break;
    const int obj = item % p.obj_n;
    const int qt = (item / p.obj_n) % qtiles;
    const int split = item / (p.obj_n * qtiles);
    const int q0 = qt * QTS + wave * 32;
    const int B = p.bank_len[obj];
    const char* Kimg = reinterpret_cast<const char*>(p.bank_k_lp) + (size_t)obj * p.stride_k * 4;
    const float* Q = p.q + (size_t)(p.q_per_obj ? obj : 0) * p.stride_q;

    int c_lo, c_hi;
    chunk_range(B, p.nsplit, split, c_lo, c_hi);

    u32x4 kst[2][4];
    f32x4 sst[2];
    const float* rs = MODE == 1 ? p.rowscale + (size_t)obj * p.stride_rs : nullptr;
    auto load_k = [&](int c, auto SET_) {
        constexpr int set = decltype(SET_)::value;
        const int b0 = c * CH;
        const __amdgpu_buffer_rsrc_t r = __builtin_amdgcn_make_buffer_rsrc(const_cast<char*>(Kimg + (size_t)b0 * 512), 0, min(CH, B - b0) * 512, 0x00020000);
#pragma unroll
        for (int j = 0; j < 4; ++j) kst[set][j] = __builtin_amdgcn_raw_buffer_load_b128(r, klane_off, 16 * j, 0);
        if constexpr (MODE == 1) { if (tid < 16) sst[set] = *reinterpret_cast<const f32x4*>(rs + b0 + 4 * tid); }
    };
    auto store_k = [&](int buf, auto SET_) {
        constexpr int set = decltype(SET_)::value;
        char* d = smem + buf * (CH * DK * 2);
#pragma unroll
        for (int j = 0; j < 4; ++j) *reinterpret_cast<u32x4*>(d + swzq(krow, kc4 + j)) = kst[set][j];
        if constexpr (MODE == 1) { if (tid < 16) *reinterpret_cast<f32x4*>(smem + SCAN_PIPE_SC0 + buf * (CH * 4) + tid * 16) = sst[set]; }
    };
    using Z0 = std::integral_constant<int, 0>; using Z1 = std::integral_constant<int, 1>;
    if (c_lo < c_hi) load_k(c_lo, Z0{});
    if (c_lo + 1 < c_hi) load_k(c_lo + 1, Z1{});

    bf16x8 qh[8];
    {
        const int q = min(q0 + li, p.HW - 1);
        const float* qrow = Q + (size_t)q * p.ldq + 8 * lh;
#pragma unroll
        for (int g = 0; g < 8; ++g) {
            const f32x4 x0 = *reinterpret_cast<const f32x4*>(qrow + 16 * g);
            const f32x4 x1 = *reinterpret_cast<const f32x4*>(qrow + 16 * g + 4);
            qh[g] = cvt8(x0, x1);
        }
    }

    float run_m = -INFINITY, run_l = 0.f;
    int run_i = 0x7fffffff;
    if (c_lo < c_hi) store_k(0, Z0{});
    __syncthreads();

    auto body = [&](auto PAR_, int c) {
        constexpr int PAR = decltype(PAR_)::value;
        const int b0 = c * CH;
        const char* kb = smem + PAR * (CH * DK * 2);
        if (c + 2 < c_hi) load_k(c + 2, PAR_);
        f32x4 scv[MODE == 1 ? 2 : 1][MODE == 1 ? 4 : 1];
        if constexpr (MODE == 1) {
            const float* sS = reinterpret_cast<const float*>(smem + SCAN_PIPE_SC0 + PAR * (CH * 4));
#pragma unroll
            for (int i = 0; i < 2; ++i)
#pragma unroll
                for (int g = 0; g < 4; ++g) scv[i][g] = *reinterpret_cast<const f32x4*>(sS + 32 * i + 4 * lh + 8 * g);
        }
        f32x16 acc[2];
#pragma unroll
        for (int i = 0; i < 2; ++i)
#pragma unroll
            for (int r = 0; r < 16; ++r) acc[i][r] = 0.f;
#pragma unroll
        for (int g = 0; g < 8; ++g) {
#pragma unroll
            for (int i = 0; i < 2; ++i) {
                const bf16x8 ah = *reinterpret_cast<const bf16x8*>(kb + swzq(32 * i + li, 2 * g + lh));
                acc[i] = __builtin_amdgcn_mfma_f32_32x32x16_bf16(ah, qh[g], acc[i], 0, 0, 0);
            }
        }
        if (MODE == 0) {
            if (b0 + CH <= B) {
                float mx = acc[0][0];
#pragma unroll
                for (int i = 0; i < 2; ++i)
#pragma unroll
                    for (int r = 0; r < 16; ++r) mx = fmaxf(mx, acc[i][r]);
                const float mn = fmaxf(run_m, mx * p.scale);
                float sum = 0.f;
#pragma unroll
                for (int i = 0; i < 2; ++i)
#pragma unroll
                    for (int r = 0; r < 16; ++r) sum += fast_exp(acc[i][r] * p.scale - mn);
                run_l = run_l * expf(run_m - mn) + sum;
                run_m = mn;
            } else {
                float mx = -INFINITY;
#pragma unroll
                for (int i = 0; i < 2; ++i)
#pragma unroll
                    for (int r = 0; r < 16; ++r) {
                        const int row = b0 + 32 * i + 4 * lh + (r & 3) + 8 * (r >> 2);
                        const float s_ = acc[i][r] * p.scale;
                        acc[i][r] = s_;
                        if (row < B) mx = fmaxf(mx, s_);
                    }
                const float mn = fmaxf(run_m, mx);
                if (mn > -INFINITY) {
                    float sum = 0.f;
#pragma unroll
                    for (int i = 0; i < 2; ++i)
#pragma unroll
                        for (int r = 0; r < 16; ++r) {
                            const int row = b0 + 32 * i + 4 * lh + (r & 3) + 8 * (r >> 2);
                            if (row < B) sum += fast_exp(acc[i][r] - mn);
                        }
                    run_l = run_l * expf(run_m - mn) + sum;
                    run_m = mn;
                }
            }
        } else {
#pragma unroll
            for (int i = 0; i < 2; ++i)
#pragma unroll
                for (int g = 0; g < 4; ++g) {
                    const int row0 = b0 + 32 * i + 4 * lh + 8 * g;
                    const f32x4 sc = scv[MODE == 1 ? i : 0][MODE == 1 ? g : 0];
#pragma unroll
                    for (int j = 0; j < 4; ++j) {
                        const int row = row0 + j;
                        if (row < B) {
                            const float s_ = acc[i][4 * g + j] * sc[j];
                            if (s_ > run_m) { run_m = s_; run_i = row; }
                        }
                    }
                }
        }
        if (c + 1 < c_hi) store_k(PAR ^ 1, std::integral_constant<int, PAR ^ 1>{});
        __syncthreads();
    };
    for (int c = c_lo; c < c_hi; c += 2) {
        body(std::integral_constant<int, 0>{}, c);
        if (c + 1 < c_hi) body(std::integral_constant<int, 1>{}, c + 1);
    }

    {
        const float om = __shfl_xor(run_m, 32, 64);
        if (MODE == 0) {
            const float ol = __shfl_xor(run_l, 32, 64);
            const float mn = fmaxf(run_m, om);
            float l = 0.f;
            if (mn > -INFINITY) l = run_l * expf(run_m - mn) + ol * expf(om - mn);
            run_m = mn; run_l = l;
        } else {
            const int oi = __shfl_xor(run_i, 32, 64);
            if (om > run_m || (om == run_m && oi < run_i)) { run_m = om; run_i = oi; }
        }
    }
    const int q = q0 + li;
    if (lh == 0 && q < p.HW) {
        float* dst = p.part + (((size_t)obj * p.nsplit + split) * p.HW + q) * 2;
        dst[0] = run_m;
        dst[1] = (MODE == 0) ? run_l : __int_as_float(run_i);
    }
  }
}

template <int MODE>
__global__ void bank_scan_finish_kernel(const float* __restrict__ part, int nsplit, int HW, int obj_n,
                                        float* __restrict__ ml, int* __restrict__ idx, float* __restrict__ corr,
                                        const float* __restrict__ colscale) {
    const int t = blockIdx.x * blockDim.x + threadIdx.x;
    const int i = min(t >> 3, obj_n * HW - 1), j = t & 7;
    const bool live = (t >> 3) < obj_n * HW;
    const int obj = i / HW, q = i - obj * HW;
    float m = -INFINITY, x = (MODE == 0) ? 0.f : __int_as_float(0x7fffffff);
    auto fold = [&](float om, float ox) {
        if (MODE == 0) {
            const float mn = fmaxf(m, om);
            if (mn > -INFINITY) x = x * expf(m - mn) + ox * expf(om - mn);
            m = mn;
        } else {
            const int i0 = __float_as_int(x), i1 = __float_as_int(ox);
            if (om > m || (om == m && i1 < i0)) { m = om; x = ox; }
        }
    };
    for (int s = j; s < nsplit; s += 8) {
        const float* src = part + (((size_t)obj * nsplit + s) * HW + q) * 2;
        fold(src[0], src[1]);
    }
    const int base = (threadIdx.x & 63) & ~7;
#pragma unroll
    for (int o = 1; o < 8; ++o) {
        const float om = __shfl(m, base + o, 64), ox = __shfl(x, base + o, 64);
        if (j == 0) fold(om, ox);
    }
    if (j != 0 || !live) return;
    if (MODE == 0) { ml[(size_t)i * 2] = m; ml[(size_t)i * 2 + 1] = x; }
    else { idx[i] = __float_as_int(x); corr[i] = m * colscale[i]; }
}

__device__ __forceinline__ int softmax_hits(f32x16& acc, float scale, float qm, float qinv, float thres, int nvalid, int rloc) {
    int cnt = 0;
#ifdef VFN_ABLATE_SOFTMAX
    for (int r = 0; r < 16; ++r) acc[r] *= qinv;
    return cnt;
#endif
    const float sm = -qm;
    if (nvalid >= CH) {
#pragma unroll
        for (int r = 0; r < 16; ++r) acc[r] = fast_exp(fmaf(acc[r], scale, sm)) * qinv;
    } else {
#pragma unroll
        for (int r = 0; r < 16; ++r) {
            const int rr = rloc + (r & 3) + 8 * (r >> 2);
            const float pv = fast_exp(fmaf(acc[r], scale, sm)) * qinv;
            acc[r] = rr < nvalid ? pv : 0.f;
        }
    }
#pragma unroll
    for (int r = 0; r < 16; ++r) {
        const unsigned long long hit = __ballot(acc[r] > thres);
        const int rlo = (r & 3) + 8 * (r >> 2);
        const int c_lo = __popcll(hit & 0xffffffffull), c_hi = __popcll(hit >> 32);
        asm volatile("v_writelane_b32 %0, %1, %2" : "+v"(cnt) : "s"(c_lo), "n"(rlo));
        asm volatile("v_writelane_b32 %0, %1, %2" : "+v"(cnt) : "s"(c_hi), "n"(rlo + 4));
    }
    return cnt;
}

__device__ int vfn_apply_linear_order = 0;
__device__ __forceinline__ void apply_item(const vfn_memread_desc& p, int& split, int& qt, int& obj) {
    const int qtiles = (int)gridDim.x / p.nsplit;
    if (vfn_apply_linear_order) { split = blockIdx.x % p.nsplit; qt = blockIdx.x / p.nsplit; obj = blockIdx.y; return; }
    const int total = (int)(gridDim.x * gridDim.y);
    const int id = (int)(blockIdx.y * gridDim.x + blockIdx.x);
    const int q = total >> 3, r = total & 7;
    const int xcd = id & 7, slot = id >> 3;
    const int L = (xcd < r ? xcd * (q + 1) : r * (q + 1) + (xcd - r) * q) + slot;
    const int pair = L / qtiles;
    qt = L - pair * qtiles;
    obj = pair / p.nsplit;
    split = pair - obj * p.nsplit;
}

__device__ __forceinline__ int swzp(int row, int chunk) { return row * 128 + ((chunk ^ ((row >> 1) & 7)) << 4); }

constexpr int QTW = 128;

__device__ __forceinline__ void chunk_load_async8(float* sK, const float* src, int valid, int wave, int lane) {
#pragma unroll
    for (int j = 0; j < 4; ++j) {
        const int r = (wave * 4 + j) * 2 + (lane >> 5);
        const int pc = lane & 31;
        const int rr = min(r, valid - 1);
        const float* g = src + (size_t)rr * DK + ((pc ^ (r & 15)) << 2);
        __builtin_amdgcn_global_load_lds(g, sK + (wave * 4 + j) * 2 * DK, 16, 0, 0);
    }
}

template <bool X3>
__global__ __launch_bounds__(512, 1)
void memread_apply_lpw_kernel(const vfn_memread_desc p) {
    extern __shared__ __attribute__((aligned(16))) char smem[];
    char* sQh = smem;
    char* sQl = sQh + QTW * DK * 2;
    float* sK = reinterpret_cast<float*>(sQh + (X3 ? 2 : 1) * QTW * DK * 2);
    char* sPh = reinterpret_cast<char*>(sK + CH * DK);
    char* sPl = sPh + QTW * CH * 2;

    const int tid = threadIdx.x, lane = tid & 63, wave = tid >> 6;
    const int li = lane & 31, lh = lane >> 5;
    const int wr = wave >> 2, wq = wave & 3;
    int split, qt, obj;
    apply_item(p, split, qt, obj);
    const int q0 = qt * QTW;
    const int B = p.bank_len[obj];
    const float* K = p.bank_k + (size_t)obj * p.stride_k;
    const float* V = p.bank_v + (size_t)obj * p.stride_v;

    {
        const int c = tid & 31;
        for (int r = tid >> 5; r < QTW; r += 16) {
            f32x4 v = {0.f, 0.f, 0.f, 0.f};
            if (q0 + r < p.HW) v = *reinterpret_cast<const f32x4*>(p.q + (size_t)(q0 + r) * p.ldq + c * 4);
            bf16x4 h, l;
#pragma unroll
            for (int e = 0; e < 4; ++e) { h[e] = (__bf16)v[e]; l[e] = (__bf16)(v[e] - (float)h[e]); }
            const int off = swzq(r, c >> 1) + (c & 1) * 8;
            *reinterpret_cast<bf16x4*>(sQh + off) = h;
            if constexpr (X3) *reinterpret_cast<bf16x4*>(sQl + off) = l;
        }
    }

    int c_lo, c_hi;
    chunk_range(B, p.nsplit, split, c_lo, c_hi);

    f32x16 o[4][2];
#pragma unroll
    for (int a = 0; a < 4; ++a)
#pragma unroll
        for (int b = 0; b < 2; ++b)
#pragma unroll
            for (int r = 0; r < 16; ++r) o[a][b][r] = 0.f;

    const float* vcol = V + wave * 64 + li * 2;
    const unsigned vlane_off = (unsigned)((8 * lh) * DV + wave * 64 + li * 2) * 4u;

    if (c_lo < c_hi) chunk_load_async8(sK, K + (size_t)c_lo * CH * DK, min(CH, B - c_lo * CH), wave, lane);
    __syncthreads();

    const int qcol = wq * 32 + li;
    const bool qok = (q0 + qcol) < p.HW;
    float qm = 1e30f, qinv = 0.f;
    if (qok) {
        qm = p.ml[((size_t)obj * p.HW + q0 + qcol) * 2];
        qinv = 1.f / p.ml[((size_t)obj * p.HW + q0 + qcol) * 2 + 1];
    }

    for (int c = c_lo; c < c_hi; ++c) {
        const int b0 = c * CH;
        const bool more = c + 1 < c_hi;

        f32x2 raw[8];
        const __amdgpu_buffer_rsrc_t vrsrc = __builtin_amdgcn_make_buffer_rsrc(
            const_cast<float*>(V + (size_t)b0 * DV), 0, min(CH, B - b0) * DV * 4, 0x00020000);
        auto load_raw = [&](int st) {
#pragma unroll
            for (int j = 0; j < 8; ++j)
                raw[j] = __builtin_bit_cast(f32x2, __builtin_amdgcn_raw_buffer_load_b64(vrsrc, vlane_off + (unsigned)((16 * st + j) * DV * 4), 0, 0));
        };
        load_raw(0);

        f32x16 acc;
#pragma unroll
        for (int r = 0; r < 16; ++r) acc[r] = 0.f;
        {
            const int ra = wr * 32 + li, rq = wq * 32 + li;
#pragma unroll
            for (int g = 0; g < 8; ++g) {
                const f32x4 x0 = *reinterpret_cast<const f32x4*>(sK + swz(ra, 4 * g + 2 * lh));
                const f32x4 x1 = *reinterpret_cast<const f32x4*>(sK + swz(ra, 4 * g + 2 * lh + 1));
                const bf16x8 bh = *reinterpret_cast<const bf16x8*>(sQh + swzq(rq, 2 * g + lh));
                bf16x8 bl = bh;
                if constexpr (X3) bl = *reinterpret_cast<const bf16x8*>(sQl + swzq(rq, 2 * g + lh));
                bf16x8 ah, al;
                if constexpr (X3) split8(x0, x1, ah, al);
                else { ah = cvt8(x0, x1); al = ah; }
                mfma_lp<X3>(acc, ah, al, bh, bl);
            }
        }

        const int rloc = wr * 32 + 4 * lh;
        const int mycnt = softmax_hits(acc, p.scale, qm, qinv, p.thres, B - b0, rloc);
#pragma unroll
        for (int g = 0; g < 4; ++g) {
            const int brow = rloc + 8 * g;
            bf16x4 h, l;
#pragma unroll
            for (int e = 0; e < 4; ++e) { h[e] = (__bf16)acc[4 * g + e]; l[e] = (__bf16)(acc[4 * g + e] - (float)h[e]); }
            const int off = swzp(qcol, brow >> 3) + ((brow >> 2) & 1) * 8;
            *reinterpret_cast<bf16x4*>(sPh + off) = h;
            if constexpr (X3) *reinterpret_cast<bf16x4*>(sPl + off) = l;
        }
        if (p.cnt && lh == 0 && mycnt > 0) {
            const int row = b0 + wr * 32 + li;
            if (row < B) atomicAdd(p.cnt + (size_t)obj * p.stride_cnt + row, mycnt);
        }
        __syncthreads();
        if (more) chunk_load_async8(sK, K + (size_t)(b0 + CH) * DK, min(CH, B - b0 - CH), wave, lane);

#pragma unroll
        for (int st = 0; st < CH / 16; ++st) {
            bf16x8 vh[2], vl[2];
#pragma unroll
            for (int tc = 0; tc < 2; ++tc)
#pragma unroll
                for (int j = 0; j < 8; ++j) {
                    const float x = raw[j][tc];
                    const __bf16 hx = (__bf16)x;
                    vh[tc][j] = hx;
                    if constexpr (X3) vl[tc][j] = (__bf16)(x - (float)hx); else vl[tc][j] = hx;
                }
            if (st + 1 < CH / 16) load_raw(st + 1);
#pragma unroll
            for (int tq = 0; tq < 4; ++tq) {
                const bf16x8 ph = *reinterpret_cast<const bf16x8*>(sPh + swzp(tq * 32 + li, 2 * st + lh));
                bf16x8 pl = ph;
                if constexpr (X3) pl = *reinterpret_cast<const bf16x8*>(sPl + swzp(tq * 32 + li, 2 * st + lh));
#pragma unroll
                for (int tc = 0; tc < 2; ++tc) mfma_lp<X3>(o[tq][tc], ph, pl, vh[tc], vl[tc]);
            }
        }
        __syncthreads();
    }

    float* dst = p.o_part + ((size_t)obj * p.nsplit + split) * p.HW * DV;
#pragma unroll
    for (int tq = 0; tq < 4; ++tq)
#pragma unroll
        for (int r = 0; r < 16; ++r) {
            const int q = q0 + tq * 32 + (r & 3) + 8 * (r >> 2) + 4 * lh;
            if (q < p.HW) {
                const f32x2 v = {o[tq][0][r], o[tq][1][r]};
                *reinterpret_cast<f32x2*>(dst + (size_t)q * DV + wave * 64 + li * 2) = v;
            }
        }
}


constexpr unsigned VBLK = 8 * DV * 4;

template <bool X3>
__global__ __launch_bounds__(512, 1)
void memread_apply_shw_kernel(const vfn_memread_desc p) {
    extern __shared__ __attribute__((aligned(16))) char smem[];
    char* sQh = smem;
    char* sQl = sQh + QTW * DK * 2;
    float* sK = reinterpret_cast<float*>(sQh + (X3 ? 2 : 1) * QTW * DK * 2);
    char* sPh = reinterpret_cast<char*>(sK + CH * DK);
    char* sPl = sPh + QTW * CH * 2;

    const int tid = threadIdx.x, lane = tid & 63, wave = tid >> 6;
    const int li = lane & 31, lh = lane >> 5;
    const int wr = wave >> 2, wq = wave & 3;
    const int qhalf = wave >> 2, cq = wave & 3;
    int split, qt, obj;
    apply_item(p, split, qt, obj);
    const int q0 = qt * QTW;
    const int B = p.bank_len[obj];
    const float* K = reinterpret_cast<const float*>(p.bank_k_lp) + (size_t)obj * p.stride_k;
    const char* V = reinterpret_cast<const char*>(p.bank_v_lp) + (size_t)obj * p.stride_v * 4;

    {
        const int c = tid & 31;
        for (int r = tid >> 5; r < QTW; r += 16) {
            f32x4 v = {0.f, 0.f, 0.f, 0.f};
            if (q0 + r < p.HW) v = *reinterpret_cast<const f32x4*>(p.q + (size_t)(q0 + r) * p.ldq + c * 4);
            bf16x4 h, l;
#pragma unroll
            for (int e = 0; e < 4; ++e) { h[e] = (__bf16)v[e]; l[e] = (__bf16)(v[e] - (float)h[e]); }
            const int off = swzq(r, c >> 1) + (c & 1) * 8;
            *reinterpret_cast<bf16x4*>(sQh + off) = h;
            if constexpr (X3) *reinterpret_cast<bf16x4*>(sQl + off) = l;
        }
    }

    int c_lo, c_hi;
    chunk_range(B, p.nsplit, split, c_lo, c_hi);

    f32x16 o[2][4];
#pragma unroll
    for (int a = 0; a < 2; ++a)
#pragma unroll
        for (int b = 0; b < 4; ++b)
#pragma unroll
            for (int r = 0; r < 16; ++r) o[a][b][r] = 0.f;

    const unsigned vlane_off = (unsigned)lh * VBLK + (unsigned)(cq * 128 + li) * 16u;

    if (c_lo < c_hi) chunk_load_async8(sK, K + (size_t)c_lo * CH * DK, min(CH, B - c_lo * CH), wave, lane);
    __syncthreads();

    const int qcol = wq * 32 + li;
    const bool qok = (q0 + qcol) < p.HW;
    float qm = 1e30f, qinv = 0.f;
    if (qok) {
        qm = p.ml[((size_t)obj * p.HW + q0 + qcol) * 2];
        qinv = 1.f / p.ml[((size_t)obj * p.HW + q0 + qcol) * 2 + 1];
    }

    for (int c = c_lo; c < c_hi; ++c) {
        const int b0 = c * CH;
        const bool more = c + 1 < c_hi;
        const int live = min(CH, B - b0);
        const __amdgpu_buffer_rsrc_t vrsrc = __builtin_amdgcn_make_buffer_rsrc(
            const_cast<char*>(V + (size_t)(b0 >> 3) * VBLK), 0, ((live + 7) >> 3) * VBLK, 0x00020000);

        constexpr int NSLOT = X3 ? 2 : 3;
        u32x4 vop[NSLOT][8];
        auto load_v = [&](int st, u32x4 (&dst)[8]) {
#pragma unroll
            for (int tc = 0; tc < 4; ++tc) {
#ifdef VFN_ABLATE_V
                dst[2 * tc] = u32x4{(unsigned)lane, (unsigned)st, 0x3f803f80u, 0x3f803f80u};
                dst[2 * tc + 1] = u32x4{0x3f803f80u, (unsigned)tc, 0u, 0u};
#else
                dst[2 * tc] = __builtin_amdgcn_raw_buffer_load_b128(vrsrc, vlane_off, 2 * st * VBLK + tc * 512, 0);
                if constexpr (X3) dst[2 * tc + 1] = __builtin_amdgcn_raw_buffer_load_b128(vrsrc, vlane_off, 2 * st * VBLK + DV * 16 + tc * 512, 0);
#endif
            }
        };
        if constexpr (X3) load_v(0, vop[0]);
        else {
#pragma unroll
            for (int st = 0; st < 3; ++st) load_v(st, vop[st]);
        }

        f32x16 acc;
#pragma unroll
        for (int r = 0; r < 16; ++r) acc[r] = 0.f;
        {
            const int ra = wr * 32 + li, rq = wq * 32 + li;
            const char* kb = reinterpret_cast<const char*>(sK);
#pragma unroll
            for (int g = 0; g < 8; ++g) {
                const bf16x8 ah = *reinterpret_cast<const bf16x8*>(kb + swzk(ra, 0, 2 * g + lh));
                bf16x8 al = ah;
                if constexpr (X3) al = *reinterpret_cast<const bf16x8*>(kb + swzk(ra, 1, 2 * g + lh));
                const bf16x8 bh = *reinterpret_cast<const bf16x8*>(sQh + swzq(rq, 2 * g + lh));
                bf16x8 bl = bh;
                if constexpr (X3) bl = *reinterpret_cast<const bf16x8*>(sQl + swzq(rq, 2 * g + lh));
                mfma_lp<X3>(acc, ah, al, bh, bl);
            }
        }

        const int rloc = wr * 32 + 4 * lh;
        const int mycnt = softmax_hits(acc, p.scale, qm, qinv, p.thres, B - b0, rloc);
#pragma unroll
        for (int g = 0; g < 4; ++g) {
            const int brow = rloc + 8 * g;
            bf16x4 h, l;
#pragma unroll
            for (int e = 0; e < 4; ++e) { h[e] = (__bf16)acc[4 * g + e]; l[e] = (__bf16)(acc[4 * g + e] - (float)h[e]); }
            const int off = swzp(qcol, brow >> 3) + ((brow >> 2) & 1) * 8;
            *reinterpret_cast<bf16x4*>(sPh + off) = h;
            if constexpr (X3) *reinterpret_cast<bf16x4*>(sPl + off) = l;
        }
        if (p.cnt && lh == 0 && mycnt > 0) {
            const int row = b0 + wr * 32 + li;
            if (row < B) atomicAdd(p.cnt + (size_t)obj * p.stride_cnt + row, mycnt);
        }
        __syncthreads();
        if (more) chunk_load_async8(sK, K + (size_t)(b0 + CH) * DK, min(CH, B - b0 - CH), wave, lane);

#pragma unroll
        for (int st = 0; st < CH / 16; ++st) {
            if constexpr (X3) { if (st + 1 < CH / 16) load_v(st + 1, vop[(st + 1) & 1]); }
            const u32x4 (&vv)[8] = vop[X3 ? (st & 1) : st % 3];
#pragma unroll
            for (int tq = 0; tq < 2; ++tq) {
                const int prow = qhalf * 64 + tq * 32 + li;
                const bf16x8 ph = *reinterpret_cast<const bf16x8*>(sPh + swzp(prow, 2 * st + lh));
                bf16x8 pl = ph;
                if constexpr (X3) pl = *reinterpret_cast<const bf16x8*>(sPl + swzp(prow, 2 * st + lh));
#pragma unroll
                for (int tc = 0; tc < 4; ++tc) {
                    const bf16x8 vh = __builtin_bit_cast(bf16x8, vv[2 * tc]);
                    const bf16x8 vl = X3 ? __builtin_bit_cast(bf16x8, vv[2 * tc + 1]) : vh;
                    mfma_lp<X3>(o[tq][tc], ph, pl, vh, vl);
                }
            }
            if constexpr (!X3) {
                if (st == 0) { __builtin_amdgcn_sched_barrier(0); load_v(3, vop[0]); }
            }
        }
        __syncthreads();
    }

    float* dst = p.o_part + ((size_t)obj * p.nsplit + split) * p.HW * DV;
#pragma unroll
    for (int tq = 0; tq < 2; ++tq)
#pragma unroll
        for (int r = 0; r < 16; ++r) {
            const int q = q0 + qhalf * 64 + tq * 32 + (r & 3) + 8 * (r >> 2) + 4 * lh;
            if (q < p.HW) {
#pragma unroll
                for (int tc = 0; tc < 4; ++tc) dst[(size_t)q * DV + cq * 128 + tc * 32 + li] = o[tq][tc][r];
            }
        }
}

constexpr size_t APPLY_PIPE_LDS = (size_t)QTW * DK * 2 + 2 * (size_t)CH * DK * 2 + 2 * (size_t)QTW * CH * 2;
constexpr unsigned PIPE_K0 = QTW * DK * 2;
constexpr unsigned PIPE_P0 = PIPE_K0 + 2 * CH * DK * 2;
constexpr unsigned PIPE_KB = CH * DK * 2, PIPE_PB = QTW * CH * 2;

__global__ __launch_bounds__(512, 1)
void memread_apply_pipe_kernel(const vfn_memread_desc p) {
    extern __shared__ __attribute__((aligned(16))) char smem[];
    char* sQh = smem;

    const int tid = threadIdx.x, lane = tid & 63, wave = tid >> 6;
    const int li = lane & 31, lh = lane >> 5;
    const int wr = wave >> 2, wq = wave & 3;
#ifdef PIPE_2X4
    constexpr int TQN = 2, TCN = 4;
    const int qbase = (wave >> 2) * 64, cbase = (wave & 3) * 128;
#else
    constexpr int TQN = 4, TCN = 2;
    const int qbase = 0, cbase = wave * 64;
#endif
    int split, qt, obj;
    apply_item(p, split, qt, obj);
    const int q0 = qt * QTW;
    const int B = p.bank_len[obj];
    const char* Kimg = reinterpret_cast<const char*>(p.bank_k_lp) + (size_t)obj * p.stride_k * 4;
    const char* V = reinterpret_cast<const char*>(p.bank_v_lp) + (size_t)obj * p.stride_v * 4;

    {
        const int c = tid & 31;
        for (int r = tid >> 5; r < QTW; r += 16) {
            f32x4 v = {0.f, 0.f, 0.f, 0.f};
            if (q0 + r < p.HW) v = *reinterpret_cast<const f32x4*>(p.q + (size_t)(q0 + r) * p.ldq + c * 4);
            const bf16x4 h = {(__bf16)v[0], (__bf16)v[1], (__bf16)v[2], (__bf16)v[3]};
            *reinterpret_cast<bf16x4*>(sQh + swzq(r, c >> 1) + (c & 1) * 8) = h;
        }
    }

    int c_lo, c_hi;
    chunk_range(B, p.nsplit, split, c_lo, c_hi);
    const int n = c_hi - c_lo;

    f32x16 o[TQN][TCN];
#pragma unroll
    for (int a = 0; a < TQN; ++a)
#pragma unroll
        for (int b = 0; b < TCN; ++b)
#pragma unroll
            for (int r = 0; r < 16; ++r) o[a][b][r] = 0.f;

    const int qcol = wq * 32 + li;
    const bool qok = (q0 + qcol) < p.HW;
    float qm = 1e30f, qinv = 0.f;
    if (qok) {
        qm = p.ml[((size_t)obj * p.HW + q0 + qcol) * 2];
        qinv = 1.f / p.ml[((size_t)obj * p.HW + q0 + qcol) * 2 + 1];
    }
    const float sm = -qm;
    const int rloc = wr * 32 + 4 * lh;

    if (n > 0) {
        const unsigned vlane_off = (unsigned)lh * VBLK + (unsigned)(cbase + li) * 16u;
        const int krow = tid >> 3, kc2 = (tid & 7) * 2;
        const unsigned klane_off = (unsigned)krow * 512u + (unsigned)kc2 * 16u;
        unsigned bK = PIPE_K0 + (unsigned)swzq(wr * 32 + li, lh);
        unsigned bQ = (unsigned)swzq(wq * 32 + li, lh);
        unsigned bR = PIPE_P0 + (unsigned)swzp(qbase + li, lh);
        unsigned bW = PIPE_P0 + (unsigned)swzp(qcol, 4 * wr) + 8u * lh;
        unsigned bS = PIPE_K0 + (unsigned)swzq(krow, kc2);
        const unsigned bS1 = (unsigned)(swzq(krow, kc2 + 1) - swzq(krow, kc2));
        auto lds = [&](unsigned a) { return smem + a; };
        u32x4 vop[4][TCN];
        u32x4 kreg[2];
        f32x16 acc;
        int mycnt = 0;

        auto vres = [&](int c) {
            const int b0 = c * CH;
            return __builtin_amdgcn_make_buffer_rsrc(const_cast<char*>(V + (size_t)(b0 >> 3) * VBLK), 0, ((min(CH, B - b0) + 7) >> 3) * (int)VBLK, 0x00020000);
        };
        auto kres = [&](int c) {
            const int b0 = c * CH;
            return __builtin_amdgcn_make_buffer_rsrc(const_cast<char*>(Kimg + (size_t)b0 * 512), 0, min(CH, B - b0) * 512, 0x00020000);
        };
        auto load_v = [&](const __amdgpu_buffer_rsrc_t& r, int st, auto SLOT_) {
            constexpr int slot = decltype(SLOT_)::value;
#ifdef PIPE_ABLATE_V
            for (int tc = 0; tc < TCN; ++tc) vop[slot][tc] = u32x4{0x3f803f80u + (unsigned)st, 0x3f803f80u, 0x3f803f80u + (unsigned)tc, 0x3f803f80u};
#else
#pragma unroll
            for (int tc = 0; tc < TCN; ++tc) vop[slot][tc] = __builtin_amdgcn_raw_buffer_load_b128(r, vlane_off, 2 * st * (int)VBLK + tc * 512, 0);
#endif
        };
        auto load_k = [&](int c) {
            const __amdgpu_buffer_rsrc_t r = kres(c);
            kreg[0] = __builtin_amdgcn_raw_buffer_load_b128(r, klane_off, 0, 0);
            kreg[1] = __builtin_amdgcn_raw_buffer_load_b128(r, klane_off, 16, 0);
        };
        auto store_k = [&](int buf) {
            const unsigned a = bS + buf * PIPE_KB;
            *reinterpret_cast<u32x4*>(lds(a)) = kreg[0];
            *reinterpret_cast<u32x4*>(lds(a + bS1)) = kreg[1];
        };
        auto score = [&](int buf) {
            const unsigned ak = bK + buf * PIPE_KB;
#pragma unroll
            for (int r = 0; r < 16; ++r) acc[r] = 0.f;
            bf16x8 fa[2], fb[2];
            fa[0] = *reinterpret_cast<const bf16x8*>(lds(ak));
            fb[0] = *reinterpret_cast<const bf16x8*>(lds(bQ));
#pragma unroll
            for (int g = 0; g < 8; ++g) {
                if (g + 1 < 8) {
                    fa[(g + 1) & 1] = *reinterpret_cast<const bf16x8*>(lds(ak ^ (32u * (g + 1))));
                    fb[(g + 1) & 1] = *reinterpret_cast<const bf16x8*>(lds(bQ ^ (32u * (g + 1))));
                }
                acc = __builtin_amdgcn_mfma_f32_32x32x16_bf16(fa[g & 1], fb[g & 1], acc, 0, 0, 0);
                __builtin_amdgcn_sched_group_barrier(0x100, 2, 0);
                __builtin_amdgcn_sched_group_barrier(0x8, 1, 0);
            }
        };
        auto softmax_quarter = [&](auto G_, int pbuf) {
            constexpr int g = decltype(G_)::value;
            float pv[4];
#pragma unroll
            for (int e = 0; e < 4; ++e) pv[e] = fast_exp(fmaf(acc[4 * g + e], p.scale, sm)) * qinv;
#ifndef PIPE_NO_HITS
#pragma unroll
            for (int e = 0; e < 4; ++e) {
                const unsigned long long hit = __ballot(pv[e] > p.thres);
                const int h_lo = __popcll(hit & 0xffffffffull), h_hi = __popcll(hit >> 32);
                asm volatile("v_writelane_b32 %0, %1, %2" : "+v"(mycnt) : "s"(h_lo), "n"(e + 8 * g));
                asm volatile("v_writelane_b32 %0, %1, %2" : "+v"(mycnt) : "s"(h_hi), "n"(e + 8 * g + 4));
            }
#endif
            const bf16x4 h = {(__bf16)pv[0], (__bf16)pv[1], (__bf16)pv[2], (__bf16)pv[3]};
            *reinterpret_cast<bf16x4*>(lds((bW + pbuf * PIPE_PB) ^ (16u * g))) = h;
        };
        auto zero_dead_rows = [&](int pbuf, int nvalid) {
#pragma unroll
            for (int g = 0; g < 4; ++g)
#pragma unroll
                for (int e = 0; e < 4; ++e)
                    if (rloc + 8 * g + e >= nvalid) *reinterpret_cast<unsigned short*>(lds(((bW + pbuf * PIPE_PB) ^ (16u * g)) + e * 2)) = 0;
        };
        auto add_hits = [&](int c) {
            if (p.cnt && lh == 0 && mycnt > 0) {
                const int row = c * CH + wr * 32 + li;
                if (row < B) atomicAdd(p.cnt + (size_t)obj * p.stride_cnt + row, mycnt);
            }
            mycnt = 0;
        };
        auto pv_step = [&](auto ST_, auto SLOT_, int pbuf) {
            constexpr int st = decltype(ST_)::value, slot = decltype(SLOT_)::value;
            const unsigned ar = (bR + pbuf * PIPE_PB) ^ (32u * st);
#pragma unroll
            for (int tq = 0; tq < TQN; ++tq) {
                const bf16x8 ph = *reinterpret_cast<const bf16x8*>(lds(ar + tq * 4096));
#ifdef PIPE_SETPRIO
                __builtin_amdgcn_s_setprio(1);
#endif
#pragma unroll
                for (int tc = 0; tc < TCN; ++tc)
                    o[tq][tc] = __builtin_amdgcn_mfma_f32_32x32x16_bf16(ph, __builtin_bit_cast(bf16x8, vop[slot][tc]), o[tq][tc], 0, 0, 0);
#ifdef PIPE_SETPRIO
                __builtin_amdgcn_s_setprio(0);
#endif
            }
        };
        using I0 = std::integral_constant<int, 0>; using I1 = std::integral_constant<int, 1>;
        using I2 = std::integral_constant<int, 2>; using I3 = std::integral_constant<int, 3>;
        auto opaque = [&]() {
            asm volatile("" : "+v"(bK), "+v"(bQ), "+v"(bR), "+v"(bW), "+v"(bS));
        };

        {
            const __amdgpu_buffer_rsrc_t vr = vres(c_lo);
            load_k(c_lo);
            load_v(vr, 0, I0{}); load_v(vr, 1, I1{}); load_v(vr, 2, I2{}); load_v(vr, 3, I3{});
            store_k(0);
            if (n > 1) load_k(c_lo + 1);
            __syncthreads();
            score(0);
            softmax_quarter(I0{}, 0); softmax_quarter(I1{}, 0); softmax_quarter(I2{}, 0); softmax_quarter(I3{}, 0);
            if (B - c_lo * CH < CH) zero_dead_rows(0, B - c_lo * CH);
            add_hits(c_lo);
            if (n > 1) store_k(1);
            __syncthreads();
        }

        auto iter = [&](auto NEXT_, auto KNEXT_, int i) {
            constexpr bool NEXT = decltype(NEXT_)::value, KNEXT = decltype(KNEXT_)::value;
            const int c = c_lo + i;
            const int pc = i & 1, pn = pc ^ 1;
            opaque();
            if constexpr (KNEXT) load_k(c + 2);
            const __amdgpu_buffer_rsrc_t vr1 = vres(NEXT ? c + 1 : c);
#ifdef PIPE_NO_SCHEDBAR
#define PIPE_SB()
#else
#define PIPE_SB() __builtin_amdgcn_sched_barrier(0)
#endif
#ifdef PIPE_SCORE_LATE
            pv_step(I0{}, I0{}, pc);
            if constexpr (NEXT) { load_v(vr1, 0, I0{}); score(pn); }
            PIPE_SB();
            pv_step(I1{}, I1{}, pc);
            if constexpr (NEXT) { load_v(vr1, 1, I1{}); softmax_quarter(I0{}, pn); }
            PIPE_SB();
            pv_step(I2{}, I2{}, pc);
            if constexpr (NEXT) { load_v(vr1, 2, I2{}); softmax_quarter(I1{}, pn); }
            PIPE_SB();
            pv_step(I3{}, I3{}, pc);
            if constexpr (NEXT) { load_v(vr1, 3, I3{}); softmax_quarter(I2{}, pn); softmax_quarter(I3{}, pn); }
#else
            if constexpr (NEXT) score(pn);
            pv_step(I0{}, I0{}, pc);
            if constexpr (NEXT) { load_v(vr1, 0, I0{}); softmax_quarter(I0{}, pn); }
            PIPE_SB();
            pv_step(I1{}, I1{}, pc);
            if constexpr (NEXT) { load_v(vr1, 1, I1{}); softmax_quarter(I1{}, pn); }
            PIPE_SB();
            pv_step(I2{}, I2{}, pc);
            if constexpr (NEXT) { load_v(vr1, 2, I2{}); softmax_quarter(I2{}, pn); }
            PIPE_SB();
            pv_step(I3{}, I3{}, pc);
            if constexpr (NEXT) { load_v(vr1, 3, I3{}); softmax_quarter(I3{}, pn); }
#endif
            if constexpr (NEXT) {
                if (B - (c + 1) * CH < CH) zero_dead_rows(pn, B - (c + 1) * CH);
                add_hits(c + 1);
            }
            if constexpr (KNEXT) store_k(pc);
            __syncthreads();
        };
        const std::true_type T{};
        const std::false_type F{};
        int i = 0;
        for (; i + 2 < n; ++i) iter(T, T, i);
        if (i + 1 < n) { iter(T, F, i); ++i; }
        iter(F, F, i);
    }

    float* dst = p.o_part + ((size_t)obj * p.nsplit + split) * p.HW * DV;
#pragma unroll
    for (int tq = 0; tq < TQN; ++tq)
#pragma unroll
        for (int r = 0; r < 16; ++r) {
            const int q = q0 + qbase + tq * 32 + (r & 3) + 8 * (r >> 2) + 4 * lh;
            if (q < p.HW) {
#pragma unroll
                for (int tc = 0; tc < TCN; ++tc) dst[(size_t)q * DV + cbase + tc * 32 + li] = o[tq][tc][r];
            }
        }
}

#ifdef VFN_CENSUS
#define PH_DECL unsigned long long ph_t = __builtin_amdgcn_s_memtime(), ph_acc[5] = {0, 0, 0, 0, 0}
#define PH_MARK(k) do { const unsigned long long t_ = __builtin_amdgcn_s_memtime(); ph_acc[k] += t_ - ph_t; ph_t = t_; } while (0)
#else
#define PH_DECL
#define PH_MARK(k)
#endif
__global__ __launch_bounds__(512, 1)
void memread_apply_wide_kernel(const vfn_memread_desc p) {
    extern __shared__ __attribute__((aligned(16))) char smem[];
    float* sQ = reinterpret_cast<float*>(smem);
    float* sK = sQ + QTW * DK;
    float* sP = sK + CH * DK;

    const int tid = threadIdx.x, lane = tid & 63, wave = tid >> 6;
    const int li = lane & 31, lh = lane >> 5;
    const int wr = wave >> 2, wq = wave & 3;
    int split, qt, obj;
    apply_item(p, split, qt, obj);
    const int q0 = qt * QTW;
    const int B = p.bank_len[obj];
    const float* K = p.bank_k + (size_t)obj * p.stride_k;
    const float* V = p.bank_v + (size_t)obj * p.stride_v;

    {
        const int c = tid & 31;
        for (int r = tid >> 5; r < QTW; r += 16) {
            f32x4 v = {0.f, 0.f, 0.f, 0.f};
            if (q0 + r < p.HW) v = *reinterpret_cast<const f32x4*>(p.q + (size_t)(q0 + r) * p.ldq + c * 4);
            *reinterpret_cast<f32x4*>(sQ + swz(r, c)) = v;
        }
    }

    int c_lo, c_hi;
    chunk_range(B, p.nsplit, split, c_lo, c_hi);

    f32x16 o[4][2];
#pragma unroll
    for (int a = 0; a < 4; ++a)
#pragma unroll
        for (int b = 0; b < 2; ++b)
#pragma unroll
            for (int r = 0; r < 16; ++r) o[a][b][r] = 0.f;

    const float* vcol = V + wave * 64 + li * 2;
    const unsigned vlane_off = (unsigned)((4 * lh) * DV + wave * 64 + li * 2) * 4u;

    if (c_lo < c_hi) chunk_load_async8(sK, K + (size_t)c_lo * CH * DK, min(CH, B - c_lo * CH), wave, lane);
    __syncthreads();

    const int qcol = wq * 32 + li;
    const bool qok = (q0 + qcol) < p.HW;
    float qm = 1e30f, qinv = 0.f;
    if (qok) {
        qm = p.ml[((size_t)obj * p.HW + q0 + qcol) * 2];
        qinv = 1.f / p.ml[((size_t)obj * p.HW + q0 + qcol) * 2 + 1];
    }

    PH_DECL;
    for (int c = c_lo; c < c_hi; ++c) {
        const int b0 = c * CH;
        const bool more = c + 1 < c_hi;

        f32x16 acc;
        score_tile(sK, sQ, wr, wq, li, lh, acc);
        PH_MARK(0);

        const int rloc = wr * 32 + 4 * lh;
        const int mycnt = softmax_hits(acc, p.scale, qm, qinv, p.thres, B - b0, rloc);
#pragma unroll
        for (int g = 0; g < 4; ++g) {
            const int brow = rloc + 8 * g;
            const f32x4 v = {acc[4 * g], acc[4 * g + 1], acc[4 * g + 2], acc[4 * g + 3]};
            *reinterpret_cast<f32x4*>(sP + swz64(qcol, brow >> 2)) = v;
        }
        if (p.cnt && lh == 0 && mycnt > 0) {
            const int row = b0 + wr * 32 + li;
            if (row < B) atomicAdd(p.cnt + (size_t)obj * p.stride_cnt + row, mycnt);
        }
        PH_MARK(1);
        __syncthreads();
        PH_MARK(2);
        if (more) chunk_load_async8(sK, K + (size_t)(b0 + CH) * DK, min(CH, B - b0 - CH), wave, lane);

        f32x2 vb[3][4];
        const __amdgpu_buffer_rsrc_t vrsrc = __builtin_amdgcn_make_buffer_rsrc(
            const_cast<float*>(V + (size_t)b0 * DV), 0, min(CH, B - b0) * DV * 4, 0x00020000);
        auto load_v = [&](int kk, int slot) {
#pragma unroll
            for (int t = 0; t < 4; ++t)
                vb[slot][t] = __builtin_bit_cast(f32x2, __builtin_amdgcn_raw_buffer_load_b64(vrsrc, vlane_off + (unsigned)((8 * kk + t) * DV * 4), 0, 0));
        };
        load_v(0, 0);
        load_v(1, 1);
        __builtin_amdgcn_sched_barrier(0);
#pragma unroll
        for (int kk = 0; kk < CH / 8; ++kk) {
            const int cur = kk % 3;
            if (kk + 2 < CH / 8) load_v(kk + 2, (kk + 2) % 3);
            __builtin_amdgcn_sched_barrier(0);
            const int lc = 2 * kk + lh;
            f32x4 a[4];
#pragma unroll
            for (int tq = 0; tq < 4; ++tq) a[tq] = *reinterpret_cast<const f32x4*>(sP + swz64(tq * 32 + li, lc));
#pragma unroll
            for (int t = 0; t < 4; ++t)
#pragma unroll
                for (int tq = 0; tq < 4; ++tq) {
                    o[tq][0] = __builtin_amdgcn_mfma_f32_32x32x2f32(a[tq][t], vb[cur][t][0], o[tq][0], 0, 0, 0);
                    o[tq][1] = __builtin_amdgcn_mfma_f32_32x32x2f32(a[tq][t], vb[cur][t][1], o[tq][1], 0, 0, 0);
                }
        }
        PH_MARK(3);
        __syncthreads();
        PH_MARK(4);
    }
#ifdef VFN_CENSUS
    if ((threadIdx.x & 63) == 0) {
        const int lin = (blockIdx.y * gridDim.x + blockIdx.x) * 8 + (threadIdx.x >> 6);
        if (lin < 2048) {
            for (int k = 0; k < 5; ++k) vfn_census_buf[lin * 8 + k] = ph_acc[k];
            vfn_census_buf[lin * 8 + 5] = c_hi - c_lo;
        }
    }
#endif

    float* dst = p.o_part + ((size_t)obj * p.nsplit + split) * p.HW * DV;
#pragma unroll
    for (int tq = 0; tq < 4; ++tq)
#pragma unroll
        for (int r = 0; r < 16; ++r) {
            const int q = q0 + tq * 32 + (r & 3) + 8 * (r >> 2) + 4 * lh;
            if (q < p.HW) {
                const f32x2 v = {o[tq][0][r], o[tq][1][r]};
                *reinterpret_cast<f32x2*>(dst + (size_t)q * DV + wave * 64 + li * 2) = v;
            }
        }
}

__global__ __launch_bounds__(512, 1)
void memread_apply_ss_kernel(const vfn_memread_desc p) {
    extern __shared__ __attribute__((aligned(16))) char smem[];
    float* sP = reinterpret_cast<float*>(smem);

    const int tid = threadIdx.x, lane = tid & 63, wave = tid >> 6;
    const int li = lane & 31, lh = lane >> 5;
    const int wr = wave >> 2, wq = wave & 3;
    int split, qt, obj;
    apply_item(p, split, qt, obj);
    const int q0 = qt * QTW;
    const int qtiles = (p.HW + QTW - 1) / QTW;
    const int B = p.bank_len[obj];
    const float* V = p.bank_v + (size_t)obj * p.stride_v;
    const float* S = p.scores + (size_t)obj * p.stride_scores;

    int c_lo, c_hi;
    chunk_range(B, p.nsplit, split, c_lo, c_hi);

    f32x16 o[4][2];
#pragma unroll
    for (int a = 0; a < 4; ++a)
#pragma unroll
        for (int b = 0; b < 2; ++b)
#pragma unroll
            for (int r = 0; r < 16; ++r) o[a][b][r] = 0.f;

    const float* vcol = V + wave * 64 + li * 2;
    const unsigned vlane_off = (unsigned)((4 * lh) * DV + wave * 64 + li * 2) * 4u;
    const unsigned slane_off = (unsigned)(((wr * 4) * 2 + lh) * QTW + wq * 32 + li) * 16u;
    f32x4 sv[4];
    auto load_scores = [&](int c) {
        const char* tile = reinterpret_cast<const char*>(S + ((size_t)c * qtiles + qt) * (CH * QTW));
#pragma unroll
        for (int g = 0; g < 4; ++g) sv[g] = __builtin_nontemporal_load(reinterpret_cast<const f32x4*>(tile + slane_off + g * (2 * QTW * 16)));
    };
    const int qcol = wq * 32 + li;
    const bool qok = (q0 + qcol) < p.HW;
    float qm = 1e30f, qinv = 0.f;
    if (qok) {
        qm = p.ml[((size_t)obj * p.HW + q0 + qcol) * 2];
        qinv = 1.f / p.ml[((size_t)obj * p.HW + q0 + qcol) * 2 + 1];
    }
    const int rloc = wr * 32 + 4 * lh;
    auto softmax_to = [&](int c, float* sPb) {
        f32x16 acc;
#pragma unroll
        for (int r = 0; r < 16; ++r) acc[r] = sv[r >> 2][r & 3];
        const int b0 = c * CH;
        const int mycnt = softmax_hits(acc, p.scale, qm, qinv, p.thres, B - b0, rloc);
#pragma unroll
        for (int g = 0; g < 4; ++g) {
            const int brow = rloc + 8 * g;
            const f32x4 v = {acc[4 * g], acc[4 * g + 1], acc[4 * g + 2], acc[4 * g + 3]};
            *reinterpret_cast<f32x4*>(sPb + swz64(qcol, brow >> 2)) = v;
        }
        if (p.cnt && lh == 0 && mycnt > 0) {
            const int row = b0 + wr * 32 + li;
            if (row < B) atomicAdd(p.cnt + (size_t)obj * p.stride_cnt + row, mycnt);
        }
    };

    f32x2 vb[4][4];
    auto chunk_rsrc = [&](int c) {
        const int rows = c < c_hi ? min(CH, B - c * CH) : 0;
        return __builtin_amdgcn_make_buffer_rsrc(const_cast<float*>(V + (size_t)min(c, max(c_hi - 1, 0)) * CH * DV), 0, rows * DV * 4, 0x00020000);
    };
    auto load_v = [&](const __amdgpu_buffer_rsrc_t& rs, int kk, int slot) {
#pragma unroll
        for (int t = 0; t < 4; ++t)
            vb[slot][t] = __builtin_bit_cast(f32x2, __builtin_amdgcn_raw_buffer_load_b64(rs, vlane_off + (unsigned)((8 * kk + t) * DV * 4), 0, 0));
    };
    if (c_lo < c_hi) {
        const __amdgpu_buffer_rsrc_t rs0 = chunk_rsrc(c_lo);
        load_v(rs0, 0, 0);
        load_v(rs0, 1, 1);
        load_scores(c_lo);
        softmax_to(c_lo, sP);
        if (c_lo + 1 < c_hi) load_scores(c_lo + 1);
    }
    __syncthreads();

    for (int c = c_lo; c < c_hi; ++c) {
        const int b0 = c * CH;
        const int buf = (c - c_lo) & 1;
        const float* sPc = sP + buf * (QTW * CH);
        float* sPn = sP + (buf ^ 1) * (QTW * CH);
        const bool nxt = c + 1 < c_hi;

        const __amdgpu_buffer_rsrc_t vrsrc = chunk_rsrc(c), vrsrc_n = chunk_rsrc(c + 1);
        f32x4 a[2][4];
#pragma unroll
        for (int tq = 0; tq < 4; ++tq) a[0][tq] = *reinterpret_cast<const f32x4*>(sPc + swz64(tq * 32 + li, lh));
        __builtin_amdgcn_sched_barrier(0);
#pragma unroll
        for (int kk = 0; kk < CH / 8; ++kk) {
            const int cur = kk % 4;
            if (kk + 2 < CH / 8) load_v(vrsrc, kk + 2, (kk + 2) % 4);
            else load_v(vrsrc_n, kk + 2 - CH / 8, (kk + 2) % 4);
            if (kk + 1 < CH / 8) {
#pragma unroll
                for (int tq = 0; tq < 4; ++tq)
                    a[(kk + 1) & 1][tq] = *reinterpret_cast<const f32x4*>(sPc + swz64(tq * 32 + li, 2 * (kk + 1) + lh));
            }
            __builtin_amdgcn_sched_barrier(0);
#pragma unroll
            for (int t = 0; t < 4; ++t)
#pragma unroll
                for (int tq = 0; tq < 4; ++tq) {
                    o[tq][0] = __builtin_amdgcn_mfma_f32_32x32x2f32(a[kk & 1][tq][t], vb[cur][t][0], o[tq][0], 0, 0, 0);
                    o[tq][1] = __builtin_amdgcn_mfma_f32_32x32x2f32(a[kk & 1][tq][t], vb[cur][t][1], o[tq][1], 0, 0, 0);
                }
            if (kk == 2 && nxt) {
                softmax_to(c + 1, sPn);
                if (c + 2 < c_hi) load_scores(c + 2);
            }
        }
        __syncthreads();
    }

    float* dst = p.o_part + ((size_t)obj * p.nsplit + split) * p.HW * DV;
#pragma unroll
    for (int tq = 0; tq < 4; ++tq)
#pragma unroll
        for (int r = 0; r < 16; ++r) {
            const int q = q0 + tq * 32 + (r & 3) + 8 * (r >> 2) + 4 * lh;
            if (q < p.HW) {
                const f32x2 v = {o[tq][0][r], o[tq][1][r]};
                *reinterpret_cast<f32x2*>(dst + (size_t)q * DV + wave * 64 + li * 2) = v;
            }
        }
}

__global__ void memread_finish_kernel(const vfn_memread_desc p) {
    const int obj = blockIdx.y;
    const size_t total = (size_t)p.HW * (DV / 4);
    for (size_t i = blockIdx.x * (size_t)blockDim.x + threadIdx.x; i < total; i += (size_t)gridDim.x * blockDim.x) {
        const int c4 = i % (DV / 4);
        const int q = i / (DV / 4);
        f32x4 s = {0.f, 0.f, 0.f, 0.f};
        for (int sp = 0; sp < p.nsplit; ++sp)
            s += *reinterpret_cast<const f32x4*>(p.o_part + (((size_t)obj * p.nsplit + sp) * p.HW + q) * DV + c4 * 4);
        float* o = p.out + ((size_t)obj * p.HW + q) * p.ld_out;
        *reinterpret_cast<f32x4*>(o + c4 * 4) = s;
        if (p.qv) *reinterpret_cast<f32x4*>(o + DV + c4 * 4) = *reinterpret_cast<const f32x4*>(p.qv + (size_t)q * p.ldqv + c4 * 4);
    }
    if (p.cnt) {
        const int B = p.bank_len[obj];
        int* cnt = p.cnt + (size_t)obj * p.stride_cnt;
        float* info = p.info + (size_t)obj * p.stride_info;
        for (int b = blockIdx.x * blockDim.x + threadIdx.x; b < B; b += gridDim.x * blockDim.x) {
            info[(size_t)b * 2 + 1] += logf((float)cnt[b] + 1.f);
            cnt[b] = 0;
        }
    }
}

constexpr size_t SCAN_LDS = (size_t)(2 * CH * DK) * sizeof(float);

bool scores_fit(long long stride_scores, long long stride_k, int HW) {
    const long long cap = stride_k / DK;
    return stride_scores >= ((cap + CH - 1) / CH) * (long long)((HW + 127) / 128) * 8192;
}

template <typename K>
void allow_lds(K kern, size_t bytes) {
    hipFuncSetAttribute(reinterpret_cast<const void*>(kern), hipFuncAttributeMaxDynamicSharedMemorySize, (int)bytes);
}

}

extern "C" int vfn_bank_scan(const vfn_bankscan_desc* d, void* stream) {
    if (!d || !d->q || !d->bank_k || !d->bank_len || !d->part) return VFN_ERR_ARG;
    if (d->nsplit < 1 || d->HW < 1 || d->obj_n < 1 || d->ldq % 4) return VFN_ERR_ARG;
    if (d->mode == 1 && (!d->rowscale || d->stride_rs % 4)) return VFN_ERR_ARG;
    if (d->precision < 0 || d->precision > 2) return VFN_ERR_ARG;
    if (d->scores && (d->mode != 0 || !scores_fit(d->stride_scores, d->stride_k, d->HW))) return VFN_ERR_ARG;
    static bool once = false;
    if (!once) {
        allow_lds(bank_scan_kernel<0, 0>, SCAN_LDS); allow_lds(bank_scan_kernel<1, 0>, SCAN_LDS);
        allow_lds(bank_scan_kernel<0, 1>, SCAN_LDS); allow_lds(bank_scan_kernel<1, 1>, SCAN_LDS);
        allow_lds(bank_scan_kernel<0, 2>, SCAN_LDS); allow_lds(bank_scan_kernel<1, 2>, SCAN_LDS);
        once = true;
    }
    if (!d->work_counter) return VFN_ERR_ARG;
    const int items = cdiv(d->HW, QTS) * d->nsplit * d->obj_n;
    const dim3 grid(items < 512 ? items : 512);
    hipStream_t s = (hipStream_t)stream;
    if (hipMemsetAsync(d->work_counter, 0, sizeof(int), s) != hipSuccess) return VFN_ERR_LAUNCH;
    if (d->precision == 1 && d->bank_k_lp) {
        const char* ep = getenv("VFN_SCAN_PIPE");
        if (!(ep && atoi(ep) == 0)) {
            static int wgs = 0;
            if (!wgs) { const char* ew = getenv("VFN_SCAN_WGS"); wgs = ew ? atoi(ew) : 768; if (wgs < 1) wgs = 768; }
            const dim3 gridp(items < wgs ? items : wgs);
            if (d->mode == 0) hipLaunchKernelGGL((bank_scan_pipe_kernel<0>), gridp, dim3(256), SCAN_PIPE_LDS, s, *d);
            else hipLaunchKernelGGL((bank_scan_pipe_kernel<1>), gridp, dim3(256), SCAN_PIPE_LDS, s, *d);
            return vfn_check_launch();
        }
    }
    switch (d->mode * 3 + d->precision) {
        case 0: hipLaunchKernelGGL((bank_scan_kernel<0, 0>), grid, dim3(256), SCAN_LDS, s, *d); break;
        case 1: hipLaunchKernelGGL((bank_scan_kernel<0, 1>), grid, dim3(256), SCAN_LDS, s, *d); break;
        case 2: hipLaunchKernelGGL((bank_scan_kernel<0, 2>), grid, dim3(256), SCAN_LDS, s, *d); break;
        case 3: hipLaunchKernelGGL((bank_scan_kernel<1, 0>), grid, dim3(256), SCAN_LDS, s, *d); break;
        case 4: hipLaunchKernelGGL((bank_scan_kernel<1, 1>), grid, dim3(256), SCAN_LDS, s, *d); break;
        case 5: hipLaunchKernelGGL((bank_scan_kernel<1, 2>), grid, dim3(256), SCAN_LDS, s, *d); break;
        default: return VFN_ERR_ARG;
    }
    return vfn_check_launch();
}

extern "C" int vfn_bank_scan_finish(const float* part, int nsplit, int HW, int obj_n, int mode, float* ml, int* idx,
                                    float* corr, const float* colscale, void* stream) {
    if (!part) return VFN_ERR_ARG;
    const int total = obj_n * HW;
    if (mode == 0) {
        if (!ml) return VFN_ERR_ARG;
        hipLaunchKernelGGL(bank_scan_finish_kernel<0>, dim3(cdiv(total * 8, 256)), dim3(256), 0, (hipStream_t)stream,
                           part, nsplit, HW, obj_n, ml, idx, corr, colscale);
    } else {
        if (!idx || !corr || !colscale) return VFN_ERR_ARG;
        hipLaunchKernelGGL(bank_scan_finish_kernel<1>, dim3(cdiv(total * 8, 256)), dim3(256), 0, (hipStream_t)stream,
                           part, nsplit, HW, obj_n, ml, idx, corr, colscale);
    }
    return vfn_check_launch();
}

extern "C" int vfn_memread_apply(const vfn_memread_desc* d, void* stream) {
    if (!d || !d->q || !d->bank_k || !d->bank_v || !d->bank_len || !d->ml || !d->o_part) return VFN_ERR_ARG;
    if (d->nsplit < 1 || d->ldq % 4) return VFN_ERR_ARG;
    if (d->precision < 0 || d->precision > 2) return VFN_ERR_ARG;
    if (d->scores && !scores_fit(d->stride_scores, d->stride_k, d->HW)) return VFN_ERR_ARG;
    {
        static bool once_x = false;
        if (!once_x) {
            const char* e = getenv("VFN_APPLY_XCD");
            const int lin = (e && atoi(e) == 0) ? 1 : 0;
            if (lin && hipMemcpyToSymbol(HIP_SYMBOL(vfn_apply_linear_order), &lin, sizeof(int)) != hipSuccess) return VFN_ERR_LAUNCH;
            once_x = true;
        }
    }
    if (d->precision == 0) {
        static bool once_f = false;
        constexpr size_t LDS_WF = (size_t)(QTW * DK + CH * DK + QTW * CH) * sizeof(float);
        if (!once_f) { allow_lds(memread_apply_wide_kernel, LDS_WF); once_f = true; }
        const dim3 gridw(cdiv(d->HW, QTW) * d->nsplit, d->obj_n);
        if (d->scores) hipLaunchKernelGGL(memread_apply_ss_kernel, gridw, dim3(512), (size_t)2 * QTW * CH * sizeof(float), (hipStream_t)stream, *d);
        else hipLaunchKernelGGL(memread_apply_wide_kernel, gridw, dim3(512), LDS_WF, (hipStream_t)stream, *d);
        return vfn_check_launch();
    }
    {
        static bool once_w = false;
        constexpr size_t LDS_W1 = (size_t)QTW * DK * 2 + (size_t)CH * DK * 4 + 2 * (size_t)QTW * CH * 2;
        constexpr size_t LDS_W2 = LDS_W1 + (size_t)QTW * DK * 2;
        if (!once_w) { allow_lds(memread_apply_lpw_kernel<false>, LDS_W1); allow_lds(memread_apply_lpw_kernel<true>, LDS_W2); once_w = true; }
        const dim3 gridw(cdiv(d->HW, QTW) * d->nsplit, d->obj_n);
        static int img_bf16 = 1;
        if (d->bank_k_lp && d->bank_v_lp && (d->precision == 2 || img_bf16)) {
            static bool once_s = false;
            if (!once_s) {
                allow_lds(memread_apply_shw_kernel<true>, LDS_W2);
                allow_lds(memread_apply_shw_kernel<false>, LDS_W1);
                const char* e = getenv("VFN_APPLY_IMG_BF16");
                if (e) img_bf16 = atoi(e);
                once_s = true;
            }
            static bool once_p = false;
            if (!once_p) { allow_lds(memread_apply_pipe_kernel, APPLY_PIPE_LDS); once_p = true; }
            const char* ep = getenv("VFN_APPLY_PIPE");
            const bool pipe = !(ep && atoi(ep) == 0);
            if (d->precision == 2) hipLaunchKernelGGL(memread_apply_shw_kernel<true>, gridw, dim3(512), LDS_W2, (hipStream_t)stream, *d);
            else if (img_bf16 && pipe) hipLaunchKernelGGL(memread_apply_pipe_kernel, gridw, dim3(512), APPLY_PIPE_LDS, (hipStream_t)stream, *d);
            else if (img_bf16) hipLaunchKernelGGL(memread_apply_shw_kernel<false>, gridw, dim3(512), LDS_W1, (hipStream_t)stream, *d);
            if (d->precision == 2 || img_bf16) return vfn_check_launch();
        }
        if (d->precision == 1) hipLaunchKernelGGL(memread_apply_lpw_kernel<false>, gridw, dim3(512), LDS_W1, (hipStream_t)stream, *d);
        else hipLaunchKernelGGL(memread_apply_lpw_kernel<true>, gridw, dim3(512), LDS_W2, (hipStream_t)stream, *d);
        return vfn_check_launch();
    }
}

extern "C" int vfn_memread_finish(const vfn_memread_desc* d, void* stream) {
    if (!d || !d->o_part || !d->out || !d->bank_len) return VFN_ERR_ARG;
    if (d->cnt && !d->info) return VFN_ERR_ARG;
    if (d->ld_out % 4 || d->ldqv % 4) return VFN_ERR_ARG;
    const dim3 grid(1024, d->obj_n);
    hipLaunchKernelGGL(memread_finish_kernel, grid, dim3(256), 0, (hipStream_t)stream, *d);
    return vfn_check_launch();
}

#ifdef VFN_CENSUS
extern "C" int vfn_debug_census(unsigned long long* host_out) {
    return hipMemcpyFromSymbol(host_out, HIP_SYMBOL(vfn_census_buf), sizeof(unsigned long long) * 4096 * 4) == hipSuccess ? 0 : 1;
}
#endif
```

v-floodnet_amd/feature_bank.py:

```python
import numpy as np
import torch

from . import _lib, ops
from ._lib import ptr, stream, check, BankDesc, BankScanDesc

DK, DV = 128, 512
MAX_SPLIT = 20
MAX_SPLIT_SCAN = 256
QT, QT_SCAN, CH = 64, 128, 64
MAX_HW = 32768


def pick_scan_slices(hw, obj_n, b_upper, target_items=1536, min_chunks=8):
    nchunks = max(1, (b_upper + CH - 1) // CH)
    qtiles = (hw + QT_SCAN - 1) // QT_SCAN
    import os
    if os.environ.get('VFN_NSPLIT_SCAN'):
        return max(1, min(int(os.environ['VFN_NSPLIT_SCAN']), nchunks, MAX_SPLIT_SCAN))
    want = max(1, target_items // (qtiles * obj_n))
    return max(1, min(want, nchunks // min_chunks if nchunks >= min_chunks else 1, MAX_SPLIT_SCAN))


def pick_nsplit(hw, obj_n, b_upper, qt=QT, max_split=MAX_SPLIT):
    nchunks = max(1, (b_upper + CH - 1) // CH)
    qtiles = (hw + qt - 1) // qt
    import os
    env = 'VFN_NSPLIT' if qt == QT else 'VFN_NSPLIT_SCAN'
    if os.environ.get(env):
        return min(int(os.environ[env]), nchunks, max_split)
    best, best_eff = 1, -1.0
    for s in range(1, max(1, min(nchunks // 3, max_split)) + 1):
        blocks = qtiles * obj_n * s
        eff = blocks / (((blocks + 255) // 256) * 256)
        if eff >= best_eff:
            best, best_eff = s, eff
    return best


class FeatureBank:
    def __init__(self, obj_n, memory_budget, device, update_rate=0.1, thres_close=0.95, precision=None):
        self.obj_n = obj_n
        self.update_rate = update_rate
        self.thres_close = thres_close
        self.device = torch.device(device)
        import os
        self.precision = precision or os.environ.get('VFN_PRECISION', 'fp32')
        if self.precision not in ops.MODES:
            raise ValueError(f'precision must be one of {sorted(ops.MODES)}, got {self.precision!r}')

        self._graph_kv = None
        self.peak_n = np.zeros(obj_n)
        self.replace_n = np.zeros(obj_n)

        self.class_budget = memory_budget // obj_n
        if obj_n == 2:
            self.class_budget = 0.8 * self.class_budget

        self._cap = 0
        self._hw = 0
        self._len_host = None
        self._len_upper = None
        self._n_updates = 0
        self._hist = {}
        self._dirty = False
        self._kbuf = self._vbuf = self._ibuf = None
        self._scratch = None
        self._norms_valid = self._lp_valid = False
        self._klp = self._vlp = None

    def _require_gpu(self):
        if self.device.type != 'cuda':
            raise RuntimeError('FeatureBank lives in GPU memory (HIP kernels only, no CPU fallback); '
                               f'got device {self.device}')
        _lib.lib()

    def _alloc(self, hw, n_init):
        self._require_gpu()
        dev = self.device
        o = self.obj_n
        cap = (int(max(self.class_budget, n_init)) + 2 * hw + 2 * CH + 63) // 64 * 64
        self._cap, self._hw = cap, hw
        self._kbuf = torch.empty(o, cap, DK, device=dev)
        self._vbuf = torch.empty(o, cap, DV, device=dev)
        self._ibuf = torch.zeros(o, cap, 2, device=dev)
        self._len_dev = torch.zeros(o, dtype=torch.int32, device=dev)
        self._stats = torch.zeros(o, 4, dtype=torch.int32, device=dev)
        self._knorm = torch.empty(o, cap, device=dev)
        self._vnorm = torch.empty(o, cap, device=dev)
        self._kinv = torch.empty(o, cap, device=dev)
        self._cnt = torch.zeros(o, cap, dtype=torch.int32, device=dev)
        self._keep_dst = torch.empty(o, cap, dtype=torch.int32, device=dev)
        self._plan = torch.zeros(o, 4, dtype=torch.int32, device=dev)
        self._new = torch.empty(o, hw, DK + DV, device=dev)
        self._nknorm = torch.empty(o, hw, device=dev)
        self._nvnorm = torch.empty(o, hw, device=dev)
        self._nkinv = torch.empty(o, hw, device=dev)
        self._midx = torch.empty(o, hw, dtype=torch.int32, device=dev)
        self._mcorr = torch.empty(o, hw, device=dev)
        self._app_pos = torch.empty(o, hw, dtype=torch.int32, device=dev)
        self._part = torch.empty(o, MAX_SPLIT_SCAN, hw, 2, device=dev)
        self._work = torch.zeros(4, dtype=torch.int32, device=dev)
        self._stats_pinned = torch.zeros(o, 4, dtype=torch.int32).pin_memory()
        self._scratch = None
        self._klp = self._vlp = None
        self._norms_valid = self._lp_valid = False

    def _ensure_scratch(self):
        if self._scratch is None:
            self._scratch = (torch.empty_like(self._kbuf), torch.empty_like(self._vbuf), torch.empty_like(self._ibuf))
        return self._scratch

    def _bank_desc(self):
        o, cap = self.obj_n, self._cap
        bd = BankDesc()
        bd.bank_k, bd.bank_v, bd.info = ptr(self._kbuf), ptr(self._vbuf), ptr(self._ibuf)
        bd.bank_len, bd.bank_len_rw = ptr(self._len_dev), ptr(self._len_dev)
        bd.stride_k, bd.stride_v, bd.stride_info, bd.stride_n = cap * DK, cap * DV, cap * 2, cap
        bd.HW, bd.obj_n, bd.cap = self._hw, o, cap
        return bd

    def lp_image(self):
        import os
        if os.environ.get('VFN_LP_IMAGE', '1') == '0' or self._kbuf is None:
            return None, None
        if self._klp is None:
            o, cap = self.obj_n, self._cap
            self._klp = torch.zeros(o * cap * DK * 2 + CH * DK * 2, dtype=torch.int16, device=self.device)
            self._vlp = torch.zeros(o * cap * DV * 2 + CH * DV * 2, dtype=torch.int16, device=self.device)
            self._lp_valid = False
        if not self._lp_valid:
            bd = self._bank_desc()
            check(_lib.lib().vfn_bank_refresh_lp(_lib.C.byref(bd), ptr(self._klp), ptr(self._vlp), 1, stream()),
                  'vfn_bank_refresh_lp')
            self._lp_valid = True
        return self._klp, self._vlp

    def _sync_len(self):
        if self._dirty:
            self._stats_pinned.copy_(self._stats, non_blocking=True)
            torch.cuda.current_stream().synchronize()
            self.absorb_stats(self._stats_pinned)
        return self._len_host

    def absorb_stats(self, stats_host, in_flight=0):
        st = stats_host.numpy()
        self._len_host = [int(st[i, 0]) for i in range(self.obj_n)]
        self._len_upper = [min(n + in_flight * self._hw, self._cap) for n in self._len_host]
        self._hist[self._n_updates - in_flight] = list(self._len_host)
        for k in [k for k in self._hist if k < self._n_updates - 2]:
            del self._hist[k]
        for i in range(self.obj_n):
            self.peak_n[i] = max(self.peak_n[i], float(st[i, 1]))
            self.replace_n[i] = float(st[i, 2])
        self._dirty = in_flight > 0
        for i in range(self.obj_n):
            if st[i, 3] < 0:
                code = int(st[i, 3])
                self._stats[i, 3] = 0
                if code == -1:
                    raise ValueError('cannot convert float NaN to integer (FeatureBank.remove: an entry born at '
                                     f'frame_idx with no hits, object {i})')
                raise OverflowError(f'cannot convert float infinity to integer (FeatureBank.remove, object {i})')

    def stats_device(self):
        return self._stats

    def len_upper(self):
        u = self._n_updates
        if u == 0 and 0 in self._hist:
            return max(self._hist[0])
        prev = self._hist.get(u - 1)
        if prev is not None:
            return min(max(prev) + self._hw, self._cap)
        return max(self._len_upper)

    @property
    def keys(self):
        if self._kbuf is None:
            return None
        n = self._sync_len()
        self._norms_valid = self._lp_valid = False
        return [self._kbuf[i, :n[i]].t() for i in range(self.obj_n)]

    @keys.setter
    def keys(self, value):
        if value is None:
            self._kbuf = None
            return
        raise AttributeError('assign through init_bank()/append(): the bank lives in pre-allocated device slabs')

    @property
    def values(self):
        if self._vbuf is None:
            return None
        n = self._sync_len()
        self._norms_valid = self._lp_valid = False
        return [self._vbuf[i, :n[i]].t() for i in range(self.obj_n)]

    @values.setter
    def values(self, value):
        if value is None:
            self._vbuf = None
            return
        raise AttributeError('assign through init_bank()/append(): the bank lives in pre-allocated device slabs')

    @property
    def info(self):
        if self._ibuf is None:
            return [None for _ in range(self.obj_n)]
        n = self._sync_len()
        return [self._ibuf[i, :n[i]] for i in range(self.obj_n)]

    @torch.no_grad()
    def _write_columns(self, keys, values, start, frame_idx, hit_init):
        for i in range(self.obj_n):
            n = keys[i].shape[1]
            s = start[i]
            self._kbuf[i, s:s + n].copy_(keys[i].t())
            self._vbuf[i, s:s + n].copy_(values[i].t())
            self._ibuf[i, s:s + n, 0] = float(frame_idx)
            self._ibuf[i, s:s + n, 1] = float(hit_init)

    def init_bank(self, keys, values, frame_idx=0):
        self._require_gpu()
        hw = keys[0].shape[1]
        n_init = max(k.shape[1] for k in keys)
        self._alloc(hw, n_init)
        self._write_columns(keys, values, [0] * self.obj_n, frame_idx, 0.0)
        lens = [int(k.shape[1]) for k in keys]
        self._set_lengths(lens)
        self._graph_kv = (list(keys), list(values)) if any(getattr(t_, 'requires_grad', False) for t_ in list(keys) + list(values)) else None

    def _set_lengths(self, lens):
        self._len_host = list(lens)
        self._len_upper = list(lens)
        self._n_updates = 0
        self._hist = {0: list(lens)}
        for i in range(self.obj_n):
            self.peak_n[i] = max(self.peak_n[i], lens[i])
        st = torch.zeros(self.obj_n, 4, dtype=torch.int32, pin_memory=True)
        for i in range(self.obj_n):
            st[i, 0] = lens[i]
            st[i, 1] = int(self.peak_n[i])
            st[i, 2] = int(self.replace_n[i])
        self._stats.copy_(st, non_blocking=True)
        ln = torch.empty(len(lens), dtype=torch.int32, pin_memory=True)
        for i, v in enumerate(lens):
            ln[i] = v
        self._len_dev.copy_(ln, non_blocking=True)
        self._dirty = False

    def append(self, keys, values, frame_idx=0):
        if self._kbuf is None:
            return self.init_bank(keys, values, frame_idx)
        lens = self._sync_len()
        need = max(lens[i] + keys[i].shape[1] for i in range(self.obj_n))
        if need > self._cap:
            self._grow(need)
        self._write_columns(keys, values, lens, frame_idx, 20.0)
        self._graph_kv = None
        self._norms_valid = self._lp_valid = False
        self._set_lengths([lens[i] + int(keys[i].shape[1]) for i in range(self.obj_n)])

    def _grow(self, need):
        cap = (int(need * 1.5) + self._hw + 63) // 64 * 64
        lens = self._len_host
        for name in ('_kbuf', '_vbuf', '_ibuf', '_knorm', '_vnorm', '_kinv', '_cnt', '_keep_dst'):
            old = getattr(self, name)
            new = torch.zeros(old.shape[0], cap, *old.shape[2:], dtype=old.dtype, device=old.device)
            new[:, :self._cap] = old
            setattr(self, name, new)
        self._cap = cap
        self._scratch = None
        self._klp = self._vlp = None
        self._lp_valid = False
        del lens

    def _stage_new(self, prev_key, prev_value):
        hw = prev_key[0].shape[1]
        k0 = prev_key[0]
        ld = DK + DV
        ok = k0.is_cuda and k0.dtype == torch.float32 and k0.stride() == (1, ld) and hw == self._hw
        if ok:
            base = k0.data_ptr()
            for i in range(self.obj_n):
                k, v = prev_key[i], prev_value[i]
                if (k.stride() != (1, ld) or v.stride() != (1, ld) or k.shape != (DK, hw) or v.shape != (DV, hw)
                        or k.data_ptr() != base + i * hw * ld * 4 or v.data_ptr() != k.data_ptr() + DK * 4):
                    ok = False
                    break
        if ok:
            return k0, ld
        for i in range(self.obj_n):
            self._new[i, :, :DK].copy_(prev_key[i].t())
            self._new[i, :, DK:].copy_(prev_value[i].t())
        return self._new, ld

    def update(self, prev_key, prev_value, frame_idx, update_rate=-1):
        self._require_gpu()
        self._graph_kv = None
        if update_rate == -1:
            update_rate = self.update_rate
        hw = prev_key[0].shape[1]
        if hw != self._hw:
            raise RuntimeError(f'feature count changed ({hw} vs {self._hw}): one bank serves one frame size')
        if hw > MAX_HW:
            raise RuntimeError(f'{hw} features per frame exceed the bank kernels\' limit of {MAX_HW} (VFN_BANK_MAX_HW)')
        L = _lib.lib()
        o, cap = self.obj_n, self._cap
        new, ld = self._stage_new(prev_key, prev_value)
        s = stream()

        if not self._norms_valid:
            ops.row_norms(self._kbuf, cap * DK, DK, DK, self._len_dev, 0, o, self._knorm, self._kinv, cap)
            ops.row_norms(self._vbuf, cap * DV, DV, DV, self._len_dev, 0, o, self._vnorm, None, cap)
        ops.row_norms(new, hw * ld, ld, DK, None, hw, o, self._nknorm, self._nkinv, hw)
        check(L.vfn_row_norms(_lib.C.c_void_p(new.data_ptr() + DK * 4), hw * ld, ld, DV, None, hw, o,
                              ptr(self._nvnorm), None, hw, s), 'vfn_row_norms')

        b_up = self.len_upper()
        nsplit = pick_scan_slices(hw, o, b_up)
        d = BankScanDesc()
        d.q, d.bank_k, d.bank_len, d.rowscale, d.part = ptr(new), ptr(self._kbuf), ptr(self._len_dev), ptr(self._kinv), ptr(self._part)
        d.stride_q, d.stride_k, d.stride_rs = hw * ld, cap * DK, cap
        d.scale = 1.0
        d.ldq, d.q_per_obj, d.HW, d.obj_n, d.nsplit, d.mode = ld, 1, hw, o, nsplit, 1
        d.precision = ops.MODES[self.precision]
        d.work_counter = ptr(self._work)
        if d.precision:
            klp, _ = self.lp_image()
            d.bank_k_lp = ptr(klp) if klp is not None else None
        check(L.vfn_bank_scan(_lib.C.byref(d), s), 'vfn_bank_scan')
        check(L.vfn_bank_scan_finish(ptr(self._part), nsplit, hw, o, 1, None, ptr(self._midx), ptr(self._mcorr),
                                     ptr(self._nkinv), s), 'vfn_bank_scan_finish')

        may_evict = self.class_budget < b_up + hw
        if may_evict:
            sk, sv, si = self._ensure_scratch()
        else:
            sk, sv, si = self._kbuf, self._vbuf, self._ibuf
        bd = BankDesc()
        bd.bank_k, bd.bank_v, bd.info = ptr(self._kbuf), ptr(self._vbuf), ptr(self._ibuf)
        bd.scratch_k, bd.scratch_v, bd.scratch_info = ptr(sk), ptr(sv), ptr(si)
        bd.bank_len, bd.bank_len_rw = ptr(self._len_dev), ptr(self._len_dev)
        bd.bank_knorm, bd.bank_vnorm = ptr(self._knorm), ptr(self._vnorm)
        bd.match_idx, bd.match_corr = ptr(self._midx), ptr(self._mcorr)
        bd.new_k, bd.new_knorm, bd.new_vnorm = ptr(new), ptr(self._nknorm), ptr(self._nvnorm)
        bd.app_pos, bd.keep_dst, bd.plan, bd.stats = ptr(self._app_pos), ptr(self._keep_dst), ptr(self._plan), ptr(self._stats)
        bd.stride_k, bd.stride_v, bd.stride_info, bd.stride_n, bd.stride_new = cap * DK, cap * DV, cap * 2, cap, hw * ld
        bd.class_budget = float(self.class_budget)
        bd.thres_close, bd.update_rate, bd.new_hit_init = float(self.thres_close), float(update_rate), 0.0
        bd.frame_idx, bd.ld_new, bd.voff, bd.HW, bd.obj_n, bd.cap = int(frame_idx), ld, DK, hw, o, cap
        bd.rm_class, bd.rm_request = -1, 0
        check(L.vfn_bank_merge(_lib.C.byref(bd), s), 'vfn_bank_merge')
        check(L.vfn_bank_append(_lib.C.byref(bd), s), 'vfn_bank_append')
        check(L.vfn_bank_refresh_norms(_lib.C.byref(bd), ptr(self._knorm), ptr(self._kinv), ptr(self._vnorm), s),
              'vfn_bank_refresh_norms')
        self._norms_valid = True
        if self._klp is not None and self._lp_valid:
            check(L.vfn_bank_refresh_lp(_lib.C.byref(bd), ptr(self._klp), ptr(self._vlp), 0, s), 'vfn_bank_refresh_lp')

        self._dirty = True
        self._len_upper = [min(n + hw, cap) for n in self._len_upper]
        self._n_updates += 1

    def remove(self, class_idx, request_n, frame_idx):
        self._require_gpu()
        self._graph_kv = None
        L = _lib.lib()
        o, cap, hw = self.obj_n, self._cap, self._hw
        self._sync_len()
        sk, sv, si = self._ensure_scratch()
        bd = BankDesc()
        bd.bank_k, bd.bank_v, bd.info = ptr(self._kbuf), ptr(self._vbuf), ptr(self._ibuf)
        bd.scratch_k, bd.scratch_v, bd.scratch_info = ptr(sk), ptr(sv), ptr(si)
        bd.bank_len, bd.bank_len_rw = ptr(self._len_dev), ptr(self._len_dev)
        bd.match_corr = ptr(self._mcorr)
        bd.app_pos, bd.keep_dst, bd.plan, bd.stats = ptr(self._app_pos), ptr(self._keep_dst), ptr(self._plan), ptr(self._stats)
        bd.stride_k, bd.stride_v, bd.stride_info, bd.stride_n, bd.stride_new = cap * DK, cap * DV, cap * 2, cap, 0
        bd.class_budget = float(self.class_budget)
        bd.thres_close, bd.update_rate, bd.new_hit_init = float(self.thres_close), float(self.update_rate), 0.0
        bd.frame_idx, bd.ld_new, bd.voff, bd.HW, bd.obj_n, bd.cap = int(frame_idx), DK + DV, DK, hw, o, cap
        bd.rm_class, bd.rm_request = int(class_idx), int(request_n)
        check(L.vfn_bank_remove(_lib.C.byref(bd), stream()), 'vfn_bank_remove')
        self._norms_valid = self._lp_valid = False
        self._dirty = True
        n = self._sync_len()
        return (self.class_budget - n[class_idx]) - request_n

    def state_dict(self, device='cpu'):
        if self._kbuf is None:
            raise RuntimeError('FeatureBank.state_dict: the bank is empty (init_bank first)')
        n = self._sync_len()
        dev = torch.device(device)
        take = lambda t: t.detach().to(dev, copy=True)
        return dict(version=1, obj_n=self.obj_n, hw=self._hw, dk=DK, dv=DV, class_budget=float(self.class_budget),
                    update_rate=float(self.update_rate), thres_close=float(self.thres_close), precision=self.precision,
                    lens=[int(x) for x in n], n_updates=int(self._n_updates),
                    hist={int(k): [int(x) for x in v] for k, v in self._hist.items()},
                    peak_n=[float(x) for x in self.peak_n], replace_n=[float(x) for x in self.replace_n],
                    keys=[take(self._kbuf[i, :n[i]]) for i in range(self.obj_n)],
                    values=[take(self._vbuf[i, :n[i]]) for i in range(self.obj_n)],
                    info=[take(self._ibuf[i, :n[i]]) for i in range(self.obj_n)])

    @torch.no_grad()
    def load_state_dict(self, sd):
        if sd.get('version') != 1:
            raise ValueError(f'FeatureBank.load_state_dict: unknown snapshot version {sd.get("version")!r}')
        if sd['obj_n'] != self.obj_n or sd['dk'] != DK or sd['dv'] != DV:
            raise ValueError(f'FeatureBank.load_state_dict: snapshot of {sd["obj_n"]} objects with {sd["dk"]} / {sd["dv"]} channels, '
                             f'bank of {self.obj_n} with {DK} / {DV}')
        lens = [int(x) for x in sd['lens']]
        for i in range(self.obj_n):
            k, v, inf = sd['keys'][i], sd['values'][i], sd['info'][i]
            if tuple(k.shape) != (lens[i], DK) or tuple(v.shape) != (lens[i], DV) or tuple(inf.shape) != (lens[i], 2):
                raise ValueError(f'FeatureBank.load_state_dict: object {i}: entries {tuple(k.shape)} / {tuple(v.shape)} / '
                                 f'{tuple(inf.shape)} do not match the recorded length {lens[i]}')
        self._alloc(int(sd['hw']), max(lens))
        for i in range(self.obj_n):
            self._kbuf[i, :lens[i]].copy_(sd['keys'][i])
            self._vbuf[i, :lens[i]].copy_(sd['values'][i])
            self._ibuf[i, :lens[i]].copy_(sd['info'][i])
        self.peak_n = np.maximum(self.peak_n, np.asarray(sd['peak_n'], dtype=np.float64))
        self.replace_n = np.asarray(sd['replace_n'], dtype=np.float64).copy()
        self._set_lengths(lens)
        self._n_updates = int(sd['n_updates'])
        self._hist = {int(k): [int(x) for x in v] for k, v in sd['hist'].items()}
        self._graph_kv = None

    def print_peak_mem(self):
        self._sync_len()
        ur = self.peak_n / self.class_budget
        rr = self.replace_n / self.class_budget
        print(f'Obj num: {self.obj_n}.', f'Budget / obj: {self.class_budget}.', f'UR: {ur}.', f'Replace: {rr}.')
```

Baseline: 152.5.

## Certify fp32 bank matches with a bf16x3 scan and exact fp32 fallback

For fp32 banks, the nearest-key match in the bank update now runs through a split-bf16 MFMA scan that tracks both the best and second-best score per column. A certify kernel accepts a match when the gap exceeds an error bound and recomputes its correlation exactly in fp32. Uncertain columns are collected in a list and rescanned in fp32 through a gather variant of the scan kernel. The change also adds a keys-only low-precision image refresh so the value image need not be maintained, at the cost of extra kernels and buffers plus atomics for the uncertain list.

```diff
diff --git a/include/vfn_hip.h b/include/vfn_hip.h
--- a/include/vfn_hip.h
+++ b/include/vfn_hip.h
@@ -5,9 +5,9 @@
 extern "C" {
 #endif
 
-#define VFN_ABI_VERSION 12
+#define VFN_ABI_VERSION 13
 enum { VFN_DESC_CONV = 0, VFN_DESC_STEM = 1, VFN_DESC_BANKSCAN = 2, VFN_DESC_MEMREAD = 3, VFN_DESC_BANK = 4, VFN_DESC_WGRAD = 5,
-       VFN_DESC_REFRESH_FILTER = 6, VFN_DESC_REFRESH_EPILOGUE = 7, VFN_DESC_GATHER = 8 };
+       VFN_DESC_REFRESH_FILTER = 6, VFN_DESC_REFRESH_EPILOGUE = 7, VFN_DESC_GATHER = 8, VFN_DESC_BANKMATCH = 9 };
 int vfn_abi_version(void);
 int vfn_sizeof_desc(int which);
 
@@ -235,6 +235,29 @@
 int vfn_bank_scan_finish(const float* part, int nsplit, int HW, int obj_n, int mode, float* ml, int* idx,
                          float* corr, const float* colscale, void* stream);
 int vfn_memread_apply(const vfn_memread_desc* d, void* stream);
+
+typedef struct vfn_bankmatch_desc {
+    const float* q;
+    const float* bank_k;
+    const void* bank_k_lp;
+    const int* bank_len;
+    const float* rowscale;
+    const float* qnorm;
+    const float* colscale;
+    float* part_x3;
+    float* part_f32;
+    int* ulist;
+    int* ucount;
+    int* utotal;
+    int* work_counter;
+    int* match_idx;
+    float* match_corr;
+    long long stride_q, stride_k, stride_rs;
+    int ldq, HW, obj_n;
+    int nsplit;
+    int nsplit_fb;
+} vfn_bankmatch_desc;
+int vfn_bank_match_certified(const vfn_bankmatch_desc* d, void* stream);
 int vfn_memread_finish(const vfn_memread_desc* d, void* stream);
 
 #define VFN_BANK_MAX_HW 32768
@@ -267,6 +290,7 @@
 } vfn_bank_desc;
 
 int vfn_bank_refresh_lp(const vfn_bank_desc* d, void* bank_k_lp, void* bank_v_lp, int all_rows, void* stream);
+int vfn_bank_refresh_lp_keys(const vfn_bank_desc* d, void* bank_k_lp, int all_rows, void* stream);
 
 int vfn_row_norms(const float* x, long long stride_obj, int ld, int dim, const int* len_dev, int rows,
                   int obj_n, float* nrm, float* inv , long long stride_n, void* stream);
diff --git a/v-floodnet_amd/_lib.py b/v-floodnet_amd/_lib.py
--- a/v-floodnet_amd/_lib.py
+++ b/v-floodnet_amd/_lib.py
@@ -71,6 +71,14 @@
                 ('scale', C.c_float), ('thres', C.c_float),
                 ('ldq', C.c_int), ('ldqv', C.c_int), ('ld_out', C.c_int), ('HW', C.c_int), ('obj_n', C.c_int),
                 ('nsplit', C.c_int), ('precision', C.c_int), ('bank_k_lp', c_fp), ('bank_v_lp', c_fp), ('scores', c_fp), ('stride_scores', C.c_longlong)]
+
+
+class BankMatchDesc(C.Structure):
+    _fields_ = [('q', c_fp), ('bank_k', c_fp), ('bank_k_lp', c_fp), ('bank_len', c_fp), ('rowscale', c_fp), ('qnorm', c_fp),
+                ('colscale', c_fp), ('part_x3', c_fp), ('part_f32', c_fp), ('ulist', c_fp), ('ucount', c_fp), ('utotal', c_fp),
+                ('work_counter', c_fp), ('match_idx', c_fp), ('match_corr', c_fp),
+                ('stride_q', C.c_longlong), ('stride_k', C.c_longlong), ('stride_rs', C.c_longlong),
+                ('ldq', C.c_int), ('HW', C.c_int), ('obj_n', C.c_int), ('nsplit', C.c_int), ('nsplit_fb', C.c_int)]
 
 
 class BankDesc(C.Structure):
@@ -87,8 +95,8 @@
                 ('obj_n', C.c_int), ('cap', C.c_int), ('rm_class', C.c_int), ('rm_request', C.c_int)]
 
 
-ABI_VERSION = 12
-DESC_IDS = {0: ConvDesc, 1: StemDesc, 2: BankScanDesc, 3: MemReadDesc, 4: BankDesc, 5: WgradDesc, 6: RefreshFilter, 7: RefreshEpilogue, 8: GatherEntry}
+ABI_VERSION = 13
+DESC_IDS = {0: ConvDesc, 1: StemDesc, 2: BankScanDesc, 3: MemReadDesc, 4: BankDesc, 5: WgradDesc, 6: RefreshFilter, 7: RefreshEpilogue, 8: GatherEntry, 9: BankMatchDesc}
 
 
 def lib():
@@ -141,6 +149,8 @@
     L.vfn_bank_refresh_norms.argtypes = [C.POINTER(BankDesc), p, p, p, p]
     L.vfn_conv_wgrad_f32.argtypes = [C.POINTER(WgradDesc), p]
     L.vfn_bank_refresh_lp.argtypes = [C.POINTER(BankDesc), p, p, i, p]
+    L.vfn_bank_refresh_lp_keys.argtypes = [C.POINTER(BankDesc), p, i, p]
+    L.vfn_bank_match_certified.argtypes = [C.POINTER(BankMatchDesc), p]
     L.vfn_stem_wgrad_scratch_floats.argtypes = [i]
     L.vfn_stem_wgrad_scratch_floats.restype = i
     for name, args in SIGNATURES.items():
@@ -224,6 +234,7 @@
     'vfn_abi_version', 'vfn_sizeof_desc', 'vfn_conv_cfg_count', 'vfn_conv_cfg_tile', 'vfn_conv_cfg_info', 'vfn_conv_cfg_wk', 'vfn_conv_cfg_tpb', 'vfn_conv_cfg_kind', 'vfn_conv_cfg_name', 'vfn_conv2d_nhwc_f32', 'vfn_conv2d_nhwc_bf16', 'vfn_conv2d_nhwc_bf16x3',
     'vfn_stem_conv7x7_f32',
     'vfn_bank_scan', 'vfn_memread_apply', 'vfn_memread_finish', 'vfn_bank_merge', 'vfn_bank_append', 'vfn_bank_remove', 'vfn_bank_refresh_norms', 'vfn_bank_refresh_lp', 'vfn_conv_wgrad_f32',
+    'vfn_bank_refresh_lp_keys', 'vfn_bank_match_certified',
     'vfn_stem_wgrad_scratch_floats'])
 
 
diff --git a/v-floodnet_amd/csrc/abi.hip b/v-floodnet_amd/csrc/abi.hip
--- a/v-floodnet_amd/csrc/abi.hip
+++ b/v-floodnet_amd/csrc/abi.hip
@@ -13,6 +13,7 @@
         case VFN_DESC_REFRESH_FILTER: return (int)sizeof(vfn_refresh_filter);
         case VFN_DESC_REFRESH_EPILOGUE: return (int)sizeof(vfn_refresh_epilogue);
         case VFN_DESC_GATHER: return (int)sizeof(vfn_gather_entry);
+        case VFN_DESC_BANKMATCH: return (int)sizeof(vfn_bankmatch_desc);
     }
     return -1;
 }
diff --git a/v-floodnet_amd/csrc/bank.hip b/v-floodnet_amd/csrc/bank.hip
--- a/v-floodnet_amd/csrc/bank.hip
+++ b/v-floodnet_amd/csrc/bank.hip
@@ -358,6 +358,7 @@
 #pragma unroll
             for (int r = 0; r < 8; ++r)
                 if (blk * 8 + r < newlen) split_key_row(blk * 8 + r);
+            if (!vlp) continue;
             char* dst = VL + (size_t)blk * (8 * DV * 4);
             for (int c = lane; c < DV; c += 64) {
                 bf16x8_t h, l;
@@ -378,6 +379,7 @@
         const int row = (corr[it] > p.thres_close) ? idx[it] : base + pos[it];
         if (row < 0 || row >= newlen) continue;
         split_key_row(row);
+        if (!vlp) continue;
         char* dst = VL + (size_t)(row >> 3) * (8 * DV * 4) + (row & 7) * 2;
         for (int c = lane; c < DV; c += 64) {
             const float x = V[(size_t)row * DV + c];
@@ -502,6 +504,14 @@
     return vfn_check_launch();
 }
 
+extern "C" int vfn_bank_refresh_lp_keys(const vfn_bank_desc* d, void* bank_k_lp, int all_rows, void* stream) {
+    if (!bank_desc_ok(d) || !bank_k_lp) return VFN_ERR_ARG;
+    if (!all_rows && (!d->plan || !d->stats || !d->match_idx || !d->match_corr || !d->app_pos)) return VFN_ERR_ARG;
+    hipLaunchKernelGGL(bank_refresh_lp_kernel, dim3(all_rows ? 4096 : 1024, d->obj_n), dim3(256), 0, (hipStream_t)stream, *d,
+                       (char*)bank_k_lp, (char*)nullptr, all_rows);
+    return vfn_check_launch();
+}
+
 extern "C" int vfn_bank_refresh_lp(const vfn_bank_desc* d, void* bank_k_lp, void* bank_v_lp, int all_rows, void* stream) {
     if (!bank_desc_ok(d) || !bank_k_lp || !bank_v_lp) return VFN_ERR_ARG;
     if (!all_rows && (!d->plan || !d->stats || !d->match_idx || !d->match_corr || !d->app_pos)) return VFN_ERR_ARG;
diff --git a/v-floodnet_amd/csrc/memory_read.hip b/v-floodnet_amd/csrc/memory_read.hip
--- a/v-floodnet_amd/csrc/memory_read.hip
+++ b/v-floodnet_amd/csrc/memory_read.hip
@@ -140,9 +140,11 @@
 __device__ unsigned long long vfn_census_buf[4096 * 4];
 #endif
 
-template <int MODE, int PREC = 0>
+struct scan_gather { const int* list; const int* count; };
+
+template <int MODE, int PREC = 0, bool GATHER = false>
 __global__ __launch_bounds__(256, 2)
-void bank_scan_kernel(const vfn_bankscan_desc p) {
+void bank_scan_kernel(const vfn_bankscan_desc p, const scan_gather gather) {
 #ifdef VFN_CENSUS
     const unsigned long long census_t0 = __builtin_amdgcn_s_memrealtime();
 #endif
@@ -153,17 +155,35 @@
     const int tid = threadIdx.x, lane = tid & 63, wave = tid >> 6;
     const int li = lane & 31, lh = lane >> 5;
     const int qtiles = (p.HW + QTS - 1) / QTS;
-    const int total = p.nsplit * qtiles * p.obj_n;
+    int total = p.nsplit * qtiles * p.obj_n;
+    if constexpr (GATHER) {
+        total = 0;
+        for (int o = 0; o < p.obj_n; ++o) total += p.nsplit * ((gather.count[o] + QTS - 1) / QTS);
+    }
   for (;;) {
     if (tid == 0) s_item = atomicAdd(p.work_counter, 1);
     __syncthreads();
-    const int item = s_item;
+    int item = s_item;
     __syncthreads();
     if (item >= total) break;
-    const int obj = item % p.obj_n;
-    const int qt = (item / p.obj_n) % qtiles;
-    const int split = item / (p.obj_n * qtiles);
+    int obj, qt, split;
+    if constexpr (GATHER) {
+        obj = 0;
+        for (;;) {
+            const int n = p.nsplit * ((gather.count[obj] + QTS - 1) / QTS);
+            if (item < n) break;
+            item -= n; ++obj;
+        }
+        const int qtl = (gather.count[obj] + QTS - 1) / QTS;
+        qt = item % qtl;
+        split = item / qtl;
+    } else {
+        obj = item % p.obj_n;
+        qt = (item / p.obj_n) % qtiles;
+        split = item / (p.obj_n * qtiles);
+    }
     const int q0 = qt * QTS + wave * 32;
+    const int ncol = GATHER ? gather.count[obj] : p.HW;
     const int B = p.bank_len[obj];
     const bool lp_image = PREC != 0 && p.bank_k_lp != nullptr;
     const float* K = (lp_image ? reinterpret_cast<const float*>(p.bank_k_lp) : p.bank_k) + (size_t)obj * p.stride_k;
@@ -176,7 +196,8 @@
     f32x4 qf[PREC == 0 ? 16 : 1];
     bf16x8 qh[PREC == 0 ? 1 : 8], ql[PREC == 2 ? 8 : 1];
     {
-        const int q = min(q0 + li, p.HW - 1);
+        int q = min(q0 + li, ncol - 1);
+        if constexpr (GATHER) q = gather.list[(size_t)obj * p.HW + q];
         if constexpr (PREC == 0) {
             const float* qrow = Q + (size_t)q * p.ldq + 4 * lh;
 #pragma unroll
@@ -195,6 +216,8 @@
 
     float run_m = -INFINITY, run_l = 0.f;
     int run_i = 0x7fffffff;
+    float run_2 = -INFINITY;
+    bool sick = false;
     __syncthreads();
 
     for (int c = c_lo; c < c_hi; ++c) {
@@ -204,13 +227,15 @@
         if (c + 1 < c_hi)
             chunk_load_async(sKb + ((c + 1 - c_lo) & 1) * CH * DK, K + (size_t)(b0 + CH) * DK, min(CH, B - b0 - CH), wave, lane);
 #endif
-        f32x4 scv[MODE == 1 ? 2 : 1][MODE == 1 ? 4 : 1];
-        if constexpr (MODE == 1) {
+        f32x4 scv[MODE >= 1 ? 2 : 1][MODE >= 1 ? 4 : 1];
+        float rs_lane = 1.f;
+        if constexpr (MODE >= 1) {
             const float* rs = p.rowscale + (size_t)obj * p.stride_rs;
 #pragma unroll
             for (int i = 0; i < 2; ++i)
 #pragma unroll
                 for (int g = 0; g < 4; ++g) scv[i][g] = *reinterpret_cast<const f32x4*>(rs + b0 + 32 * i + 4 * lh + 8 * g);
+            if constexpr (MODE == 2) rs_lane = rs[b0 + lane];
         }
         f32x16 acc[2];
 #pragma unroll
@@ -318,16 +343,18 @@
 #pragma unroll
                 for (int g = 0; g < 4; ++g) {
                     const int row0 = b0 + 32 * i + 4 * lh + 8 * g;
-                    const f32x4 sc = scv[MODE == 1 ? i : 0][MODE == 1 ? g : 0];
+                    const f32x4 sc = scv[MODE >= 1 ? i : 0][MODE >= 1 ? g : 0];
 #pragma unroll
                     for (int j = 0; j < 4; ++j) {
                         const int row = row0 + j;
                         if (row < B) {
                             const float s_ = acc[i][4 * g + j] * sc[j];
+                            if constexpr (MODE == 2) run_2 = __builtin_amdgcn_fmed3f(s_, run_m, run_2);
                             if (s_ > run_m) { run_m = s_; run_i = row; }
                         }
                     }
                 }
+            if constexpr (MODE == 2) sick |= (b0 + lane < B) && !(rs_lane > 0.f && rs_lane < 1e12f);
         }
         __syncthreads();
     }
@@ -342,8 +369,16 @@
             run_m = mn; run_l = l;
         } else {
             const int oi = __shfl_xor(run_i, 32, 64);
+            if constexpr (MODE == 2) {
+                const float o2 = __shfl_xor(run_2, 32, 64);
+                if (om > run_m || (om == run_m && oi < run_i)) run_2 = fmaxf(run_m, o2);
+                else run_2 = fmaxf(run_2, om);
+            }
             if (om > run_m || (om == run_m && oi < run_i)) { run_m = om; run_i = oi; }
         }
+    }
+    if constexpr (MODE == 2) {
+        if (__ballot(sick) != 0) run_2 = INFINITY;
     }
 #ifdef VFN_CENSUS
     if (threadIdx.x == 0) {
@@ -358,10 +393,15 @@
     }
 #endif
     const int q = q0 + li;
-    if (lh == 0 && q < p.HW) {
-        float* dst = p.part + (((size_t)obj * p.nsplit + split) * p.HW + q) * 2;
-        dst[0] = run_m;
-        dst[1] = (MODE == 0) ? run_l : __int_as_float(run_i);
+    if (lh == 0 && q < ncol) {
+        if constexpr (MODE == 2) {
+            float* dst = p.part + (((size_t)obj * p.nsplit + split) * p.HW + q) * 4;
+            *reinterpret_cast<f32x4*>(dst) = f32x4{run_m, __int_as_float(run_i), run_2, 0.f};
+        } else {
+            float* dst = p.part + (((size_t)obj * p.nsplit + split) * p.HW + q) * 2;
+            dst[0] = run_m;
+            dst[1] = (MODE == 0) ? run_l : __int_as_float(run_i);
+        }
     }
   }
 }
@@ -582,6 +622,92 @@
     if (j != 0 || !live) return;
     if (MODE == 0) { ml[(size_t)i * 2] = m; ml[(size_t)i * 2 + 1] = x; }
     else { idx[i] = __float_as_int(x); corr[i] = m * colscale[i]; }
+}
+
+constexpr float MATCH_EPS_REL = 1.25e-4f;
+constexpr float MATCH_EPS_ABS = 5.421010862427522e-20f;
+constexpr float MATCH_QNORM_MAX = 1.152921504606846976e18f;
+
+__global__ __launch_bounds__(64)
+void bank_match_certify_kernel(const vfn_bankmatch_desc p) {
+    const int lane = threadIdx.x, li = lane & 31, lh = lane >> 5;
+    const int obj = blockIdx.y, q0 = blockIdx.x * 32;
+    const int q = q0 + li, qc = min(q, p.HW - 1);
+    float m = -INFINITY, m2 = -INFINITY;
+    int bi = 0x7fffffff;
+    auto fold = [&](float om, int oi, float o2) {
+        if (om > m || (om == m && oi < bi)) { m2 = fmaxf(fmaxf(m, m2), o2); m = om; bi = oi; }
+        else m2 = fmaxf(fmaxf(m2, om), o2);
+    };
+    const float* part = p.part_x3 + ((size_t)obj * p.nsplit * p.HW + qc) * 4;
+#pragma unroll 4
+    for (int s = lh; s < p.nsplit; s += 2) {
+        const f32x4 v = *reinterpret_cast<const f32x4*>(part + (size_t)s * p.HW * 4);
+        fold(v[0], __float_as_int(v[1]), v[2]);
+    }
+    fold(__shfl_xor(m, 32, 64), __shfl_xor(bi, 32, 64), __shfl_xor(m2, 32, 64));
+
+    const size_t col = (size_t)obj * p.HW + qc;
+    const float qn = p.qnorm[col];
+    const float margin = 4.f * (MATCH_EPS_REL * qn + MATCH_EPS_ABS);
+    const bool cert = q < p.HW && qn > 0.f && qn <= MATCH_QNORM_MAX && m > -INFINITY && m < INFINITY && (m - m2) > margin;
+
+    const float* krow = p.bank_k + (size_t)obj * p.stride_k + (size_t)(cert ? bi : 0) * DK + 4 * lh;
+    const float* qrow = p.q + (size_t)obj * p.stride_q + (size_t)qc * p.ldq + 4 * lh;
+    f32x16 acc;
+#pragma unroll
+    for (int r = 0; r < 16; ++r) acc[r] = 0.f;
+#pragma unroll
+    for (int kk = 0; kk < 16; ++kk) {
+        f32x4 a = *reinterpret_cast<const f32x4*>(krow + 8 * kk);
+        const f32x4 b = *reinterpret_cast<const f32x4*>(qrow + 8 * kk);
+        if (!cert) a = f32x4{0.f, 0.f, 0.f, 0.f};
+#pragma unroll
+        for (int t = 0; t < 4; ++t) acc = __builtin_amdgcn_mfma_f32_32x32x2f32(a[t], b[t], acc, 0, 0, 0);
+    }
+    const int rsel = (li & 3) + 4 * (li >> 3);
+    float dot = 0.f;
+#pragma unroll
+    for (int r = 0; r < 16; ++r) dot = (r == rsel) ? acc[r] : dot;
+    if (lh != ((li >> 2) & 1)) return;
+    if (cert) {
+        const float s_ = dot * p.rowscale[(size_t)obj * p.stride_rs + bi];
+        p.match_idx[col] = bi;
+        p.match_corr[col] = s_ * p.colscale[col];
+    } else if (q < p.HW) {
+        const int pos = atomicAdd(p.ucount + obj, 1);
+        p.ulist[(size_t)obj * p.HW + pos] = q;
+        if (p.utotal) atomicAdd(p.utotal + obj, 1);
+    }
+}
+
+__global__ void bank_match_finish_listed_kernel(const float* __restrict__ part, int nsplit, int HW, int obj_n,
+                                                const int* __restrict__ ulist, const int* __restrict__ ucount,
+                                                int* __restrict__ idx, float* __restrict__ corr, const float* __restrict__ colscale) {
+    const int t = blockIdx.x * blockDim.x + threadIdx.x;
+    const int i = min(t >> 3, obj_n * HW - 1), j = t & 7;
+    const int obj = i / HW, pos = i - obj * HW;
+    const bool live = (t >> 3) < obj_n * HW && pos < ucount[obj];
+    float m = -INFINITY, x = __int_as_float(0x7fffffff);
+    auto fold = [&](float om, float ox) {
+        const int i0 = __float_as_int(x), i1 = __float_as_int(ox);
+        if (om > m || (om == m && i1 < i0)) { m = om; x = ox; }
+    };
+    if (live)
+        for (int s = j; s < nsplit; s += 8) {
+            const float* src = part + (((size_t)obj * nsplit + s) * HW + pos) * 2;
+            fold(src[0], src[1]);
+        }
+    const int base = (threadIdx.x & 63) & ~7;
+#pragma unroll
+    for (int o = 1; o < 8; ++o) {
+        const float om = __shfl(m, base + o, 64), ox = __shfl(x, base + o, 64);
+        if (j == 0) fold(om, ox);
+    }
+    if (j != 0 || !live) return;
+    const size_t c = (size_t)obj * HW + ulist[(size_t)obj * HW + pos];
+    idx[c] = __float_as_int(x);
+    corr[c] = m * colscale[c];
 }
 
 __device__ __forceinline__ int softmax_hits(f32x16& acc, float scale, float qm, float qinv, float thres, int nvalid, int rloc) {
@@ -1550,12 +1676,12 @@
         }
     }
     switch (d->mode * 3 + d->precision) {
-        case 0: hipLaunchKernelGGL((bank_scan_kernel<0, 0>), grid, dim3(256), SCAN_LDS, s, *d); break;
-        case 1: hipLaunchKernelGGL((bank_scan_kernel<0, 1>), grid, dim3(256), SCAN_LDS, s, *d); break;
-        case 2: hipLaunchKernelGGL((bank_scan_kernel<0, 2>), grid, dim3(256), SCAN_LDS, s, *d); break;
-        case 3: hipLaunchKernelGGL((bank_scan_kernel<1, 0>), grid, dim3(256), SCAN_LDS, s, *d); break;
-        case 4: hipLaunchKernelGGL((bank_scan_kernel<1, 1>), grid, dim3(256), SCAN_LDS, s, *d); break;
-        case 5: hipLaunchKernelGGL((bank_scan_kernel<1, 2>), grid, dim3(256), SCAN_LDS, s, *d); break;
+        case 0: hipLaunchKernelGGL((bank_scan_kernel<0, 0>), grid, dim3(256), SCAN_LDS, s, *d, scan_gather{}); break;
+        case 1: hipLaunchKernelGGL((bank_scan_kernel<0, 1>), grid, dim3(256), SCAN_LDS, s, *d, scan_gather{}); break;
+        case 2: hipLaunchKernelGGL((bank_scan_kernel<0, 2>), grid, dim3(256), SCAN_LDS, s, *d, scan_gather{}); break;
+        case 3: hipLaunchKernelGGL((bank_scan_kernel<1, 0>), grid, dim3(256), SCAN_LDS, s, *d, scan_gather{}); break;
+        case 4: hipLaunchKernelGGL((bank_scan_kernel<1, 1>), grid, dim3(256), SCAN_LDS, s, *d, scan_gather{}); break;
+        case 5: hipLaunchKernelGGL((bank_scan_kernel<1, 2>), grid, dim3(256), SCAN_LDS, s, *d, scan_gather{}); break;
         default: return VFN_ERR_ARG;
     }
     return vfn_check_launch();
@@ -1574,6 +1700,36 @@
         hipLaunchKernelGGL(bank_scan_finish_kernel<1>, dim3(cdiv(total * 8, 256)), dim3(256), 0, (hipStream_t)stream,
                            part, nsplit, HW, obj_n, ml, idx, corr, colscale);
     }
+    return vfn_check_launch();
+}
+
+extern "C" int vfn_bank_match_certified(const vfn_bankmatch_desc* d, void* stream) {
+    if (!d || !d->q || !d->bank_k || !d->bank_k_lp || !d->bank_len || !d->rowscale || !d->qnorm || !d->colscale) return VFN_ERR_ARG;
+    if (!d->part_x3 || !d->part_f32 || !d->ulist || !d->ucount || !d->work_counter || !d->match_idx || !d->match_corr) return VFN_ERR_ARG;
+    if (d->nsplit < 1 || d->nsplit_fb < 1 || d->HW < 1 || d->obj_n < 1 || d->ldq % 4 || d->stride_rs % 4) return VFN_ERR_ARG;
+    static bool once = false;
+    if (!once) {
+        allow_lds(bank_scan_kernel<2, 2>, SCAN_LDS); allow_lds(bank_scan_kernel<1, 0, true>, SCAN_LDS);
+        once = true;
+    }
+    hipStream_t s = (hipStream_t)stream;
+    vfn_bankscan_desc sd = {};
+    sd.q = d->q; sd.bank_k = d->bank_k; sd.bank_len = d->bank_len; sd.rowscale = d->rowscale;
+    sd.stride_q = d->stride_q; sd.stride_k = d->stride_k; sd.stride_rs = d->stride_rs;
+    sd.scale = 1.f; sd.ldq = d->ldq; sd.q_per_obj = 1; sd.HW = d->HW; sd.obj_n = d->obj_n;
+    sd.work_counter = d->work_counter; sd.bank_k_lp = d->bank_k_lp;
+    sd.part = d->part_x3; sd.nsplit = d->nsplit; sd.mode = 2; sd.precision = 2;
+    const int items = cdiv(d->HW, QTS) * d->nsplit * d->obj_n;
+    if (hipMemsetAsync(d->work_counter, 0, sizeof(int), s) != hipSuccess) return VFN_ERR_LAUNCH;
+    if (hipMemsetAsync(d->ucount, 0, sizeof(int) * d->obj_n, s) != hipSuccess) return VFN_ERR_LAUNCH;
+    hipLaunchKernelGGL((bank_scan_kernel<2, 2>), dim3(items < 512 ? items : 512), dim3(256), SCAN_LDS, s, sd, scan_gather{});
+    hipLaunchKernelGGL(bank_match_certify_kernel, dim3(cdiv(d->HW, 32), d->obj_n), dim3(64), 0, s, *d);
+    sd.part = d->part_f32; sd.nsplit = d->nsplit_fb; sd.mode = 1; sd.precision = 0; sd.bank_k_lp = nullptr;
+    if (hipMemsetAsync(d->work_counter, 0, sizeof(int), s) != hipSuccess) return VFN_ERR_LAUNCH;
+    hipLaunchKernelGGL((bank_scan_kernel<1, 0, true>), dim3(512), dim3(256), SCAN_LDS, s, sd, scan_gather{d->ulist, d->ucount});
+    hipLaunchKernelGGL(bank_match_finish_listed_kernel, dim3(cdiv(d->obj_n * d->HW * 8, 256)), dim3(256), 0, s,
+                       (const float*)d->part_f32, d->nsplit_fb, d->HW, d->obj_n, (const int*)d->ulist, (const int*)d->ucount,
+                       d->match_idx, d->match_corr, d->colscale);
     return vfn_check_launch();
 }
 
diff --git a/v-floodnet_amd/feature_bank.py b/v-floodnet_amd/feature_bank.py
--- a/v-floodnet_amd/feature_bank.py
+++ b/v-floodnet_amd/feature_bank.py
@@ -2,7 +2,7 @@
 import torch
 
 from . import _lib, ops
-from ._lib import ptr, stream, check, BankDesc, BankScanDesc
+from ._lib import ptr, stream, check, BankDesc, BankScanDesc, BankMatchDesc
 
 DK, DV = 128, 512
 MAX_SPLIT = 20
@@ -19,6 +19,11 @@
         return max(1, min(int(os.environ['VFN_NSPLIT_SCAN']), nchunks, MAX_SPLIT_SCAN))
     want = max(1, target_items // (qtiles * obj_n))
     return max(1, min(want, nchunks // min_chunks if nchunks >= min_chunks else 1, MAX_SPLIT_SCAN))
+
+
+def pick_fallback_slices(obj_n, b_upper, target_items=512, min_chunks=4):
+    nchunks = max(1, (b_upper + CH - 1) // CH)
+    return max(1, min(target_items // obj_n, nchunks // min_chunks, MAX_SPLIT_SCAN))
 
 
 def pick_nsplit(hw, obj_n, b_upper, qt=QT, max_split=MAX_SPLIT):
@@ -67,6 +72,9 @@
         self._scratch = None
         self._norms_valid = self._lp_valid = False
         self._klp = self._vlp = None
+        self._kimg_valid = False
+        self._mbuf = None
+        self._match_updates = 0
 
     def _require_gpu(self):
         if self.device.type != 'cuda':
@@ -103,7 +111,9 @@
         self._stats_pinned = torch.zeros(o, 4, dtype=torch.int32).pin_memory()
         self._scratch = None
         self._klp = self._vlp = None
-        self._norms_valid = self._lp_valid = False
+        self._mbuf = None
+        self._match_updates = 0
+        self._norms_valid = self._lp_valid = self._kimg_valid = False
 
     def _ensure_scratch(self):
         if self._scratch is None:
@@ -123,17 +133,46 @@
         import os
         if os.environ.get('VFN_LP_IMAGE', '1') == '0' or self._kbuf is None:
             return None, None
+        o, cap = self.obj_n, self._cap
         if self._klp is None:
-            o, cap = self.obj_n, self._cap
             self._klp = torch.zeros(o * cap * DK * 2 + CH * DK * 2, dtype=torch.int16, device=self.device)
+            self._lp_valid = self._kimg_valid = False
+        if self._vlp is None:
             self._vlp = torch.zeros(o * cap * DV * 2 + CH * DV * 2, dtype=torch.int16, device=self.device)
             self._lp_valid = False
         if not self._lp_valid:
             bd = self._bank_desc()
             check(_lib.lib().vfn_bank_refresh_lp(_lib.C.byref(bd), ptr(self._klp), ptr(self._vlp), 1, stream()),
                   'vfn_bank_refresh_lp')
-            self._lp_valid = True
+            self._lp_valid = self._kimg_valid = True
         return self._klp, self._vlp
+
+    def key_image(self):
+        if self._klp is None:
+            self._klp = torch.zeros(self.obj_n * self._cap * DK * 2 + CH * DK * 2, dtype=torch.int16, device=self.device)
+            self._lp_valid = self._kimg_valid = False
+        if not self._kimg_valid:
+            bd = self._bank_desc()
+            check(_lib.lib().vfn_bank_refresh_lp_keys(_lib.C.byref(bd), ptr(self._klp), 1, stream()), 'vfn_bank_refresh_lp_keys')
+            self._kimg_valid = True
+        return self._klp
+
+    def _match_buffers(self):
+        if self._mbuf is None:
+            o, hw, dev = self.obj_n, self._hw, self.device
+            self._mbuf = dict(part_x3=torch.empty(o, MAX_SPLIT_SCAN, hw, 4, device=dev),
+                              ulist=torch.empty(o, hw, dtype=torch.int32, device=dev),
+                              ucount=torch.zeros(o, dtype=torch.int32, device=dev),
+                              utotal=torch.zeros(o, dtype=torch.int32, device=dev))
+        return self._mbuf
+
+    def certified_match(self):
+        import os
+        return self.precision == 'fp32' and os.environ.get('VFN_CERTIFIED_MATCH', '1') != '0'
+
+    def match_stats(self):
+        unc = [0] * self.obj_n if self._mbuf is None else [int(x) for x in self._mbuf['utotal'].cpu()]
+        return dict(updates=self._match_updates, columns=self._match_updates * self._hw, uncertain=unc)
 
     def _sync_len(self):
         if self._dirty:
@@ -179,7 +218,7 @@
         if self._kbuf is None:
             return None
         n = self._sync_len()
-        self._norms_valid = self._lp_valid = False
+        self._norms_valid = self._lp_valid = self._kimg_valid = False
         return [self._kbuf[i, :n[i]].t() for i in range(self.obj_n)]
 
     @keys.setter
@@ -194,7 +233,7 @@
         if self._vbuf is None:
             return None
         n = self._sync_len()
-        self._norms_valid = self._lp_valid = False
+        self._norms_valid = self._lp_valid = self._kimg_valid = False
         return [self._vbuf[i, :n[i]].t() for i in range(self.obj_n)]
 
     @values.setter
@@ -259,7 +298,7 @@
             self._grow(need)
         self._write_columns(keys, values, lens, frame_idx, 20.0)
         self._graph_kv = None
-        self._norms_valid = self._lp_valid = False
+        self._norms_valid = self._lp_valid = self._kimg_valid = False
         self._set_lengths([lens[i] + int(keys[i].shape[1]) for i in range(self.obj_n)])
 
     def _grow(self, need):
@@ -273,7 +312,7 @@
         self._cap = cap
         self._scratch = None
         self._klp = self._vlp = None
-        self._lp_valid = False
+        self._lp_valid = self._kimg_valid = False
         del lens
 
     def _stage_new(self, prev_key, prev_value):
@@ -320,19 +359,33 @@
 
         b_up = self.len_upper()
         nsplit = pick_scan_slices(hw, o, b_up)
-        d = BankScanDesc()
-        d.q, d.bank_k, d.bank_len, d.rowscale, d.part = ptr(new), ptr(self._kbuf), ptr(self._len_dev), ptr(self._kinv), ptr(self._part)
-        d.stride_q, d.stride_k, d.stride_rs = hw * ld, cap * DK, cap
-        d.scale = 1.0
-        d.ldq, d.q_per_obj, d.HW, d.obj_n, d.nsplit, d.mode = ld, 1, hw, o, nsplit, 1
-        d.precision = ops.MODES[self.precision]
-        d.work_counter = ptr(self._work)
-        if d.precision:
-            klp, _ = self.lp_image()
-            d.bank_k_lp = ptr(klp) if klp is not None else None
-        check(L.vfn_bank_scan(_lib.C.byref(d), s), 'vfn_bank_scan')
-        check(L.vfn_bank_scan_finish(ptr(self._part), nsplit, hw, o, 1, None, ptr(self._midx), ptr(self._mcorr),
-                                     ptr(self._nkinv), s), 'vfn_bank_scan_finish')
+        if self.certified_match():
+            mb = self._match_buffers()
+            md = BankMatchDesc()
+            md.q, md.bank_k, md.bank_k_lp, md.bank_len = ptr(new), ptr(self._kbuf), ptr(self.key_image()), ptr(self._len_dev)
+            md.rowscale, md.qnorm, md.colscale = ptr(self._kinv), ptr(self._nknorm), ptr(self._nkinv)
+            md.part_x3, md.part_f32, md.ulist = ptr(mb['part_x3']), ptr(self._part), ptr(mb['ulist'])
+            md.ucount, md.utotal, md.work_counter = ptr(mb['ucount']), ptr(mb['utotal']), ptr(self._work)
+            md.match_idx, md.match_corr = ptr(self._midx), ptr(self._mcorr)
+            md.stride_q, md.stride_k, md.stride_rs = hw * ld, cap * DK, cap
+            md.ldq, md.HW, md.obj_n, md.nsplit = ld, hw, o, nsplit
+            md.nsplit_fb = pick_fallback_slices(o, b_up)
+            check(L.vfn_bank_match_certified(_lib.C.byref(md), s), 'vfn_bank_match_certified')
+            self._match_updates += 1
+        else:
+            d = BankScanDesc()
+            d.q, d.bank_k, d.bank_len, d.rowscale, d.part = ptr(new), ptr(self._kbuf), ptr(self._len_dev), ptr(self._kinv), ptr(self._part)
+            d.stride_q, d.stride_k, d.stride_rs = hw * ld, cap * DK, cap
+            d.scale = 1.0
+            d.ldq, d.q_per_obj, d.HW, d.obj_n, d.nsplit, d.mode = ld, 1, hw, o, nsplit, 1
+            d.precision = ops.MODES[self.precision]
+            d.work_counter = ptr(self._work)
+            if d.precision:
+                klp, _ = self.lp_image()
+                d.bank_k_lp = ptr(klp) if klp is not None else None
+            check(L.vfn_bank_scan(_lib.C.byref(d), s), 'vfn_bank_scan')
+            check(L.vfn_bank_scan_finish(ptr(self._part), nsplit, hw, o, 1, None, ptr(self._midx), ptr(self._mcorr),
+                                         ptr(self._nkinv), s), 'vfn_bank_scan_finish')
 
         may_evict = self.class_budget < b_up + hw
         if may_evict:
@@ -359,6 +412,8 @@
         self._norms_valid = True
         if self._klp is not None and self._lp_valid:
             check(L.vfn_bank_refresh_lp(_lib.C.byref(bd), ptr(self._klp), ptr(self._vlp), 0, s), 'vfn_bank_refresh_lp')
+        elif self._klp is not None and self._kimg_valid:
+            check(L.vfn_bank_refresh_lp_keys(_lib.C.byref(bd), ptr(self._klp), 0, s), 'vfn_bank_refresh_lp_keys')
 
         self._dirty = True
         self._len_upper = [min(n + hw, cap) for n in self._len_upper]
@@ -383,7 +438,7 @@
         bd.frame_idx, bd.ld_new, bd.voff, bd.HW, bd.obj_n, bd.cap = int(frame_idx), DK + DV, DK, hw, o, cap
         bd.rm_class, bd.rm_request = int(class_idx), int(request_n)
         check(L.vfn_bank_remove(_lib.C.byref(bd), stream()), 'vfn_bank_remove')
-        self._norms_valid = self._lp_valid = False
+        self._norms_valid = self._lp_valid = self._kimg_valid = False
         self._dirty = True
         n = self._sync_len()
         return (self.class_budget - n[class_idx]) - request_n
```

After: 158.4, median of 6. +3.9%, better.
